# SilentView/EMCID

Measured on AMD Instinct MI355X. Metric: concept-edits/sec (1 000-concept batch, SD-v1.4), higher is better.
Workload: dtype f32 forward (2 x fp16 split MFMA, fp32 accumulate) + f64 solve

## Files before the change

emcid_amd/csrc/clip_layers.hip:

```cpp
#include "common.h"

#include <algorithm>

namespace emcid {

__global__ __launch_bounds__(256) void gather_rows16_kernel(const unsigned char* __restrict__ src, int64_t src_stride,
                                                             const int* __restrict__ idx, unsigned char* __restrict__ dst,
                                                             int64_t dst_stride, int row_bytes) {
    typedef unsigned int v4u __attribute__((ext_vector_type(4)));
    const int64_t r = blockIdx.x;
    const v4u* s = reinterpret_cast<const v4u*>(src + (int64_t)idx[r] * src_stride);
    v4u* d = reinterpret_cast<v4u*>(dst + r * dst_stride);
    for (int i = threadIdx.x; i < row_bytes / 16; i += 256) d[i] = s[i];
}

__global__ __launch_bounds__(256) void gather_f32_kernel(const float* __restrict__ src, const int* __restrict__ idx,
                                                          float* __restrict__ dst, int n) {
    const int i = blockIdx.x * 256 + threadIdx.x;
    if (i < n) dst[i] = src[idx[i]];
}

__device__ __forceinline__ unsigned long long fp_mix(unsigned long long x) {
    x ^= x >> 30; x *= 0xBF58476D1CE4E5B9ull; x ^= x >> 27; x *= 0x94D049BB133111EBull; x ^= x >> 31;
    return x;
}

__device__ __forceinline__ unsigned long long fingerprint_of(const unsigned char* data, long long bytes, unsigned long long* lds) {
    typedef unsigned long long v2u64 __attribute__((ext_vector_type(2)));
    const long long nvec = bytes / 16, ns = nvec < 4096 ? nvec : 4096;
    unsigned long long h = 0;
    v2u64 x[16];
#pragma unroll
    for (int u = 0; u < 16; ++u) {
        const long long i = threadIdx.x + 256 * u;
        const long long v = ns == nvec ? i : i * nvec / ns;
        x[u] = i < ns ? *reinterpret_cast<const v2u64*>(data + 16 * v) : (v2u64){0ull, 0ull};
    }
#pragma unroll
    for (int u = 0; u < 16; ++u) {
        const long long i = threadIdx.x + 256 * u;
        if (i < ns)
            h ^= fp_mix(x[u][0] + 0x9E3779B97F4A7C15ull * (unsigned long long)(2 * i + 1)) ^ fp_mix(x[u][1] + 0x9E3779B97F4A7C15ull * (unsigned long long)(2 * i + 2));
    }
#pragma unroll
    for (int o = 32; o > 0; o >>= 1) {
        const unsigned lo = __shfl_xor((unsigned)(h & 0xffffffffu), o, 64), hi = __shfl_xor((unsigned)(h >> 32), o, 64);
        h ^= ((unsigned long long)hi << 32) | lo;
    }
    if ((threadIdx.x & 63) == 0) lds[threadIdx.x >> 6] = h;
    __syncthreads();
    return lds[0] ^ lds[1] ^ lds[2] ^ lds[3];
}

struct FpBatch { const unsigned char* data[32]; long long bytes[32]; long long slot[32]; };

__global__ __launch_bounds__(256) void fingerprint_store_kernel(FpBatch b, long long* table) {
    __shared__ unsigned long long lds[4];
    const unsigned char* data = b.data[blockIdx.x];
    const long long bytes = b.bytes[blockIdx.x];
    const unsigned long long h = fingerprint_of(data, bytes, lds);
    if (threadIdx.x == 0) {
        long long* e = table + 4 * b.slot[blockIdx.x];
        e[0] = (long long)reinterpret_cast<uintptr_t>(data); e[1] = bytes; e[2] = (long long)h; e[3] = 0;
    }
}

__global__ __launch_bounds__(256) void fingerprint_content_kernel(FpBatch b, unsigned long long* out) {
    __shared__ unsigned long long lds[4];
    const unsigned long long h = fingerprint_of(b.data[blockIdx.x], b.bytes[blockIdx.x], lds);
    if (threadIdx.x == 0) out[b.slot[blockIdx.x]] = h;
}

struct FpSkip { unsigned long long m[4]; };

__global__ __launch_bounds__(256) void fingerprint_check_kernel(const long long* table, long long first_slot, FpSkip skip, int* flag) {
    __shared__ unsigned long long lds[4];
    if ((skip.m[blockIdx.x >> 6] >> (blockIdx.x & 63)) & 1ull) return;
    const long long* e = table + 4 * (first_slot + blockIdx.x);
    const long long bytes = e[1];
    if (bytes <= 0) return;
    const unsigned long long h = fingerprint_of(reinterpret_cast<const unsigned char*>((uintptr_t)e[0]), bytes, lds);
    if (threadIdx.x == 0 && h != (unsigned long long)e[2]) atomicOr(flag, 1);
}

struct ClipWs {
    float* qkv;
    float* mid;
    uint32_t* ctx_p;
    float* ctx_s;
    uint32_t* z_p;
    float* z_s;
    float* f_scale;
    uint32_t* f_p;
    uint32_t* xq_p;
    float* xq_s;
    float* hs_q;
};

inline int64_t clip_ws_bytes(int64_t rows, int64_t h, int64_t d) {
    const int64_t r = round_up(rows, 64);
    return 4 * (r * 3 * h + r * h + r * h + r + r * h + r + 2 * r + r * d + r * h + r + r * h) + 16 * 16;
}

inline bool clip_ws_carve(void* base, int64_t bytes, int64_t rows, int64_t h, int64_t d, ClipWs& w) {
    if (base == nullptr || !aligned16(base) || bytes < clip_ws_bytes(rows, h, d)) return false;
    const int64_t r = round_up(rows, 64);
    char* p = (char*)base;
    auto take = [&](int64_t n4) { char* q = p; p += round_up(4 * n4, 16); return q; };
    w.qkv = (float*)take(r * 3 * h);
    w.mid = (float*)take(r * h);
    w.ctx_p = (uint32_t*)take(r * h);
    w.ctx_s = (float*)take(r);
    w.z_p = (uint32_t*)take(r * h);
    w.z_s = (float*)take(r);
    w.f_scale = (float*)take(2 * r);
    w.f_p = (uint32_t*)take(r * d);
    w.xq_p = (uint32_t*)take(r * h);
    w.xq_s = (float*)take(r);
    w.hs_q = (float*)take(r * h);
    return true;
}

}

using namespace emcid;

extern "C" {

int emcid_fingerprint_store(int64_t n, const void* const* data, const int64_t* bytes, const int64_t* slots, void* table,
                            int64_t table_slots, void* stream) {
    EMCID_CHECK_ARG(n >= 0 && table && (n == 0 || (data && bytes && slots)));
    for (int64_t i0 = 0; i0 < n; i0 += 32) {
        FpBatch b{};
        const int cnt = (int)std::min<int64_t>(32, n - i0);
        for (int i = 0; i < cnt; ++i) {
            EMCID_CHECK_ARG(data[i0 + i] && bytes[i0 + i] > 0 && bytes[i0 + i] % 16 == 0 && aligned16(data[i0 + i]) &&
                            slots[i0 + i] >= 0 && slots[i0 + i] < table_slots);
            b.data[i] = (const unsigned char*)data[i0 + i]; b.bytes[i] = bytes[i0 + i]; b.slot[i] = slots[i0 + i];
        }
        hipLaunchKernelGGL(fingerprint_store_kernel, dim3((unsigned)cnt), dim3(256), 0, (hipStream_t)stream, b, (long long*)table);
    }
    EMCID_CHECK_LAUNCH();
    return EMCID_OK;
}

int emcid_fingerprint_check(const void* table, int64_t table_slots, int64_t first_slot, int64_t n_slots, const uint64_t* skip_mask,
                            int* flag, void* stream) {
    EMCID_CHECK_ARG(table && flag && first_slot >= 0 && n_slots >= 0 && first_slot + n_slots <= table_slots && n_slots <= 256);
    if (n_slots == 0) return EMCID_OK;
    FpSkip skip{};
    if (skip_mask != nullptr)
        for (int w = 0; w < 4; ++w) skip.m[w] = skip_mask[w];
    hipLaunchKernelGGL(fingerprint_check_kernel, dim3((unsigned)n_slots), dim3(256), 0, (hipStream_t)stream, (const long long*)table,
                       (long long)first_slot, skip, flag);
    EMCID_CHECK_LAUNCH();
    return EMCID_OK;
}

int emcid_fingerprint_content(int64_t n, const void* const* data, const int64_t* bytes, uint64_t* out_dev, void* stream) {
    EMCID_CHECK_ARG(n >= 0 && (n == 0 || (data && bytes && out_dev)));
    if (n == 0) return EMCID_OK;
    for (int64_t i = 0; i < n; ++i)
        EMCID_CHECK_ARG(data[i] && bytes[i] > 0 && bytes[i] % 16 == 0 && aligned16(data[i]));
    for (int64_t i0 = 0; i0 < n; i0 += 32) {
        FpBatch b{};
        const int cnt = (int)std::min<int64_t>(32, n - i0);
        for (int i = 0; i < cnt; ++i) {
            b.data[i] = (const unsigned char*)data[i0 + i]; b.bytes[i] = bytes[i0 + i]; b.slot[i] = i0 + i;
        }
        hipLaunchKernelGGL(fingerprint_content_kernel, dim3((unsigned)cnt), dim3(256), 0, (hipStream_t)stream, b,
                           (unsigned long long*)out_dev);
    }
    EMCID_CHECK_LAUNCH();
    return EMCID_OK;
}

int64_t emcid_clip_workspace_bytes(int64_t rows, int64_t h, int64_t d) { return clip_ws_bytes(rows, h, d); }

int emcid_clip_layer_head_sp16(const emcid_clip_layer_sp16* L, int64_t rows, int64_t h, int64_t d, int64_t heads, float attn_scale,
                               const int* anc, int64_t anc_ld, const int* depth, const int* rows_sel, int64_t n_sel,
                               const float* hs, const void* x_planes, const float* x_inv_scale, float* mid, void* f_planes,
                               float* f_scale, float* f_f32, void* workspace, int64_t workspace_bytes, void* stream) {
    EMCID_CHECK_ARG(L && rows > 0 && h > 0 && d > 0 && heads > 0 && h % heads == 0 && anc && depth && hs && x_planes && x_inv_scale);
    EMCID_CHECK_ARG(mid && f_planes && f_scale && n_sel > 0 && n_sel <= rows && (rows_sel != nullptr || n_sel == rows) && h % 32 == 0 && d % 32 == 0);
    ClipWs w;
    if (!clip_ws_carve(workspace, workspace_bytes, rows, h, d, w)) return fail(EMCID_ERR_BAD_ARG, __func__, "workspace too small or misaligned");
    hipStream_t st = (hipStream_t)stream;
    const int64_t D = h / heads;
    const float* q;
    int64_t ldq;
    const float* res;
    if (rows_sel == nullptr) {
        EMCID_TRY(emcid_linear_sp16_f32(x_planes, h, x_inv_scale, L->qkv_planes, h, L->qkv_inv_scale, L->qkv_bias, nullptr, 0, w.qkv,
                                        3 * h, nullptr, 0, nullptr, rows, 3 * h, h, 0, -1, stream));
        q = w.qkv, ldq = 3 * h, res = hs;
    } else {
        EMCID_TRY(emcid_linear_sp16_f32(x_planes, h, x_inv_scale, (const uint32_t*)L->qkv_planes + h * h, h, L->qkv_inv_scale + h,
                                        L->qkv_bias ? L->qkv_bias + h : nullptr, nullptr, 0, w.qkv + h, 3 * h, nullptr, 0, nullptr,
                                        rows, 2 * h, h, 0, -1, stream));
        {
            ScopedProf sp(KC_MISC, st);
            hipLaunchKernelGGL(gather_rows16_kernel, dim3((unsigned)n_sel), dim3(256), 0, st, (const unsigned char*)x_planes, 4 * h,
                               rows_sel, (unsigned char*)w.xq_p, 4 * h, (int)(4 * h));
            hipLaunchKernelGGL(gather_f32_kernel, dim3((unsigned)((n_sel + 255) / 256)), dim3(256), 0, st, x_inv_scale, rows_sel,
                               w.xq_s, (int)n_sel);
            hipLaunchKernelGGL(gather_rows16_kernel, dim3((unsigned)n_sel), dim3(256), 0, st, (const unsigned char*)hs, 4 * h,
                               rows_sel, (unsigned char*)w.hs_q, 4 * h, (int)(4 * h));
            EMCID_CHECK_LAUNCH();
        }
        EMCID_TRY(emcid_linear_sp16_f32(w.xq_p, h, w.xq_s, L->qkv_planes, h, L->qkv_inv_scale, L->qkv_bias, nullptr, 0, w.mid, h,
                                        nullptr, 0, nullptr, n_sel, h, h, 0, -1, stream));
        q = w.mid, ldq = h, res = w.hs_q;
    }
    EMCID_TRY(emcid_tree_attention_sp16(q, ldq, w.qkv + h, w.qkv + 2 * h, 3 * h, anc, anc_ld, depth, rows_sel, n_sel, heads, D,
                                        attn_scale, w.ctx_p, h, w.ctx_s, stream));
    EMCID_TRY(emcid_linear_sp16_f32(w.ctx_p, h, w.ctx_s, L->out_planes, h, L->out_inv_scale, L->out_bias, res, h, mid, h, nullptr,
                                    0, nullptr, n_sel, h, h, 0, -1, stream));
    EMCID_TRY(emcid_add_layernorm_sp16(mid, h, nullptr, 0, L->ln2_gamma, L->ln2_beta, L->ln2_eps, n_sel, h, nullptr, nullptr, w.z_p,
                                       h, w.z_s, L->fc1_bound, f_scale, stream));
    EMCID_TRY(emcid_linear_sp16_f32(w.z_p, h, w.z_s, L->fc1_planes, h, L->fc1_inv_scale, L->fc1_bias, nullptr, 0, f_f32, d,
                                    f_planes, d, f_scale, n_sel, d, h, L->act, -1, stream));
    return EMCID_OK;
}

int emcid_clip_layer_tail_sp16(const emcid_clip_layer_sp16* L, int64_t n, int64_t h, int64_t d, const void* f_planes,
                               const float* f_inv_scale, const float* mid, float* hs_out, const float* next_ln_gamma,
                               const float* next_ln_beta, float next_ln_eps, void* x_planes, float* x_inv_scale, void* stream) {
    EMCID_CHECK_ARG(L && n > 0 && h % 32 == 0 && d % 32 == 0 && f_planes && f_inv_scale && mid && hs_out);
    EMCID_TRY(emcid_linear_sp16_f32(f_planes, d, f_inv_scale, L->fc2_planes, d, L->fc2_inv_scale, L->fc2_bias, mid, h, hs_out, h,
                                    nullptr, 0, nullptr, n, h, d, 0, -1, stream));
    if (next_ln_gamma != nullptr) {
        EMCID_CHECK_ARG(next_ln_beta && x_planes && x_inv_scale);
        EMCID_TRY(emcid_add_layernorm_sp16(hs_out, h, nullptr, 0, next_ln_gamma, next_ln_beta, next_ln_eps, n, h, nullptr, nullptr,
                                           x_planes, h, x_inv_scale, nullptr, nullptr, stream));
    }
    return EMCID_OK;
}

int emcid_clip_edit_layer_tail_sp16(const emcid_clip_layer_sp16* L, int64_t n_rows, int64_t h, int64_t d, const float* f_f32,
                                    const void* f_planes, const float* f_inv_scale, const float* mid, const int64_t* lookup,
                                    const int64_t* seg, int64_t B, int64_t N, const float* zs_t, double edit_weight,
                                    int layers_left, double lam_ratio, const void* cov_factor_ws, int64_t n_layers,
                                    int64_t layer_index, int use_inverse, const float* W0, float* W, float* dW, float* K_out,
                                    float* Zc_out, void* k_planes, float* k_inv_scale, void* dual_ws, int64_t dual_ws_bytes,
                                    int* info_dev, void* linear_ws, int64_t linear_ws_bytes, float* hs_out,
                                    const float* next_ln_gamma, const float* next_ln_beta, float next_ln_eps, void* x_planes,
                                    float* x_inv_scale, void* stream) {
    EMCID_CHECK_ARG(L && n_rows > 0 && h % 32 == 0 && d % 32 == 0 && f_f32 && lookup && seg && B > 0 && N > 0 && zs_t);
    EMCID_CHECK_ARG(cov_factor_ws && W0 && W && K_out && Zc_out && dual_ws && info_dev && (hs_out == nullptr || (f_planes && f_inv_scale && mid)));
    EMCID_TRY(emcid_gather_mean_f32(f_f32, B, n_rows, d, 0, d, lookup, seg, N, K_out, d, stream));
    EMCID_CHECK_ARG((k_planes == nullptr) == (k_inv_scale == nullptr));
    if (k_planes != nullptr) {
        EMCID_TRY(emcid_split_rows_f16(K_out, d, N, d, k_planes, d, k_inv_scale, nullptr, stream));
        EMCID_TRY(emcid_linear_sp16_f32(k_planes, d, k_inv_scale, L->fc2_planes, d, L->fc2_inv_scale, L->fc2_bias, nullptr, 0, Zc_out, h,
                                        nullptr, 0, nullptr, N, h, d, 0, -1, stream));
    } else {
        EMCID_TRY(emcid_linear_ws_f32(K_out, d, W, d, L->fc2_bias, nullptr, 0, Zc_out, h, N, h, d, 0, -1, linear_ws, linear_ws_bytes, stream));
    }
    EMCID_TRY(emcid_edit_dual_apply_stage1_f64(K_out, Zc_out, zs_t, N, d, h, edit_weight, layers_left, lam_ratio, cov_factor_ws,
                                               n_layers, layer_index, 0, N, use_inverse, dual_ws, dual_ws_bytes, stream));
    EMCID_TRY(emcid_edit_dual_apply_stage2_f64(N, d, h, cov_factor_ws, n_layers, layer_index, use_inverse, 0, W0, W, dW, dual_ws,
                                               dual_ws_bytes, info_dev, stream));
    if (hs_out != nullptr) {
        EMCID_TRY(emcid_split_rows_f16(W, d, h, d, const_cast<void*>(L->fc2_planes), d, const_cast<float*>(L->fc2_inv_scale), nullptr,
                                       stream));
        EMCID_TRY(emcid_clip_layer_tail_sp16(L, n_rows, h, d, f_planes, f_inv_scale, mid, hs_out, next_ln_gamma, next_ln_beta,
                                             next_ln_eps, x_planes, x_inv_scale, stream));
    }
    return EMCID_OK;
}

int emcid_clip_layers_sp16(const emcid_clip_layer_sp16* layers, int64_t n_layers, int64_t rows, int64_t h, int64_t d, int64_t heads,
                           float attn_scale, const int* anc, int64_t anc_ld, const int* depth, float* hs, void* x_planes,
                           float* x_inv_scale, const float* next_ln_gamma, const float* next_ln_beta, float next_ln_eps,
                           void* workspace, int64_t workspace_bytes, void* stream) {
    EMCID_CHECK_ARG(layers && n_layers > 0 && hs && x_planes && x_inv_scale);
    ClipWs w;
    if (!clip_ws_carve(workspace, workspace_bytes, rows, h, d, w)) return fail(EMCID_ERR_BAD_ARG, __func__, "workspace too small or misaligned");
    for (int64_t i = 0; i < n_layers; ++i) {
        const emcid_clip_layer_sp16* L = layers + i;
        EMCID_TRY(emcid_clip_layer_head_sp16(L, rows, h, d, heads, attn_scale, anc, anc_ld, depth, nullptr, rows, hs, x_planes,
                                             x_inv_scale, w.mid, w.f_p, w.f_scale, nullptr, workspace, workspace_bytes, stream));
        const bool last = i + 1 == n_layers;
        const float* g = last ? next_ln_gamma : layers[i + 1].ln1_gamma;
        const float* b = last ? next_ln_beta : layers[i + 1].ln1_beta;
        const float eps = last ? next_ln_eps : layers[i + 1].ln1_eps;
        EMCID_TRY(emcid_clip_layer_tail_sp16(L, rows, h, d, w.f_p, w.f_scale + rows, w.mid, hs, g, b, eps, x_planes, x_inv_scale, stream));
    }
    return EMCID_OK;
}

}
```

emcid_amd/csrc/edit_solve.hip:

```cpp
#include "spd_solve.h"

namespace emcid {


__global__ __launch_bounds__(256) void prep_kr_kernel(const float* __restrict__ K, const float* __restrict__ Zc,
                                                       const float* __restrict__ zs_t, int N, int d, int h, double s,
                                                       double layers_left, double* __restrict__ Kt64, int Np, int dp,
                                                       double* __restrict__ Rt, int hp, double g = 1.0) {
    const int n = blockIdx.x;
    for (int j = threadIdx.x; j < dp; j += 256) {
        double v = 0.0;
        if (n < N && j < d) v = (double)K[(int64_t)n * d + j] * s * g;
        Kt64[(int64_t)n * dp + j] = v;
    }
    if (Rt) {
        for (int i = threadIdx.x; i < hp; i += 256) {
            double v = 0.0;
            if (n < N && i < h) {
                const float src = zs_t[(int64_t)n * h + i] - Zc[(int64_t)n * h + i];
                v = ((double)src * s) / layers_left * g;
            }
            Rt[(int64_t)n * hp + i] = v;
        }
    }
}

static void launch_prep_kr(const float* K, const float* Zc, const float* zs_t, int64_t N, int64_t d, int64_t h, double edit_weight,
                           int layers_left, double gain, double* Kt, int64_t Np, int64_t dp, double* R, int64_t hp, hipStream_t st) {
    ScopedProf sp(KC_PREP, st);
    hipLaunchKernelGGL(prep_kr_kernel, dim3((unsigned)Np), dim3(256), 0, st, K, Zc, zs_t, (int)N, (int)d, (int)h, sqrt(edit_weight / 0.5),
                       (double)layers_left, Kt, (int)Np, (int)dp, R, (int)hp, gain);
}

__global__ __launch_bounds__(256) void axpy_f32_kernel(float* __restrict__ W, const float* __restrict__ dW, int64_t n) {
    int64_t i = (int64_t)blockIdx.x * 256 + threadIdx.x;
    const int64_t stride = (int64_t)gridDim.x * 256;
    for (; i < n; i += stride) W[i] += dW[i];
}

__global__ __launch_bounds__(256) void apply_u_kernel(const double* __restrict__ U, const float* __restrict__ W0,
                                                       float* __restrict__ W, float* __restrict__ dW, int64_t n) {
    int64_t i = (int64_t)blockIdx.x * 256 + threadIdx.x;
    const int64_t stride = (int64_t)gridDim.x * 256;
    for (; i < n; i += stride) {
        const float f = (float)U[i];
        if (dW) dW[i] = f;
        if (W) W[i] = W0[i] + f;
    }
}

static int factor_and_solve(double* A, double* L, int64_t dp, int64_t lda, double* invw, int* info, double* B, double* Y,
                            int64_t rows, int64_t ldb, hipStream_t st) {
    return with_graph(make_key(GRAPH_FACTOR_SOLVE, {A, L, invw, info, B, Y}, {dp, lda, rows, ldb}), st, [&](hipStream_t s) {
        EMCID_TRY(cholesky_impl(A, L, dp, lda, invw, info, s));
        return cholesky_solve_impl(L, dp, lda, invw, B, Y, rows, ldb, s);
    });
}


struct CovPtrs { const float* c[32]; };
__global__ __launch_bounds__(256) void scale_cov_kernel(CovPtrs cov, int d, int dp, double lam, float cw, double* __restrict__ M,
                                                         int64_t s_mat) {
    const int l = blockIdx.y;
    const int i = blockIdx.x;
    const float* C = cov.c[l];
    double* row = M + l * s_mat + (int64_t)i * dp;
    for (int j = threadIdx.x; j <= i; j += 256) {
        double v;
        if (i < d) {
            const float c1 = C[(int64_t)i * d + j] * cw;
            v = lam * (double)(c1 / 0.5f);
        } else {
            v = (i == j) ? 1.0 : 0.0;
        }
        row[j] = v;
    }
}

static void assemble_dual_system(const double* P, const double* Q, int64_t dp, double* S, int Np, hipStream_t st,
                                 double* sk_work = nullptr) {
    ScopedProf sp(KC_ASSEMBLE, st);
    GemmShape g{P, dp, Q, dp, Np, Np, (int)dp, 1};
    if (Np >= 512 && sk_work && launch_gemm_f64_streamk2<true, true>(g, EpiAxpby{S, Np, 1.0, 0.0}, st, kStreamKWgs, sk_work, 1.0))
        return;
    hipLaunchKernelGGL(eye_f64_kernel, dim3((unsigned)Np), dim3(256), 0, st, S, Np);
    const int kt = (int)(dp / 16);
    g.ksplit = kt >= 64 ? 4 : kt >= 32 ? 2 : 1;
    launch_gemm_f64<true, true>(g, EpiAxpby{S, Np, 1.0, 1.0}, st, Np >= 512 ? 1 : 2);
}

__global__ __launch_bounds__(256) void transpose_f64_kernel(const double* __restrict__ src, int64_t lds_, double* __restrict__ dst,
                                                             int64_t ldd, int rows, int cols) {
    __shared__ double tile[32][33];
    const int bx = blockIdx.x * 32, by = blockIdx.y * 32;
    const int tx = threadIdx.x & 31, ty = threadIdx.x >> 5;
    for (int r = ty; r < 32; r += 8)
        tile[r][tx] = (by + r < rows && bx + tx < cols) ? src[(int64_t)(by + r) * lds_ + bx + tx] : 0.0;
    __syncthreads();
    for (int r = ty; r < 32; r += 8)
        if (bx + r < cols && by + tx < rows) dst[(int64_t)(bx + r) * ldd + by + tx] = tile[tx][r];
}

struct EditWorkspace {
    int64_t Np, dp, hp;
    int64_t off_A, off_L, off_inv, off_B, off_Y, off_R, total;
    EditWorkspace(int64_t N, int64_t d, int64_t h) {
        Np = round_up(N, NPAD);
        dp = round_up(d, NB);
        hp = round_up(h, 2);
        int64_t o = 0;
        off_A = o; o += dp * dp;
        off_L = o; o += dp * dp;
        off_inv = o; o += inv_doubles(dp);
        off_B = o; o += Np * dp;
        off_Y = o; o += Np * dp;
        off_R = o; o += Np * hp;
        total = o;
    }
};

int solve_schur_rhs(const double* R, int64_t hp, int64_t h, int64_t Np, const double* LS, const double* invS, const double* XT,
                    double* full_inv, double* RT, double* Y2, int64_t y2_doubles, hipStream_t st) {
    if (y2_doubles < hp * Np) return fail(EMCID_ERR_WORKSPACE, __func__, "RT / Y2 hold fewer than h rows of Np (h > d rounded up to 128)");
    const int form = schur_rhs_form(Np, XT != nullptr, full_inv != nullptr, y2_doubles);
    hipLaunchKernelGGL(transpose_f64_kernel, dim3((unsigned)((hp + 31) / 32), (unsigned)(Np / 32)), dim3(256), 0, st, R, hp, RT, Np,
                       (int)Np, (int)hp);
    if (form == EMCID_SCHUR_XROW) {
        ScopedProf sp(KC_TRSM_DIAG, st);
        GemmShape f{RT, Np, XT, Np, (int)h, (int)Np, (int)Np, 0};
        f.tri = 1; f.pair = 1;
        launch_gemm_f64<true, false>(f, EpiAxpby{Y2, Np, 1.0, 0.0}, st);
        GemmShape b{Y2, Np, XT, Np, (int)h, (int)Np, (int)Np, 0};
        b.tri = 2; b.pair = 1;
        launch_gemm_f64<true, true>(b, EpiAxpby{RT, Np, 1.0, 0.0}, st);
    } else if (form == EMCID_SCHUR_FULL_INVERSE) {
        EMCID_TRY(build_full_inverse(LS, Np, Np, invS, full_inv, Y2, y2_doubles, 1, 0, 0, st));
        ScopedProf sp(KC_TRSM_DIAG, st);
        GemmShape f{RT, Np, full_inv, Np, (int)h, (int)Np, (int)Np, 0};
        f.tri = 1; f.pair = 1;
        launch_gemm_f64<true, true>(f, EpiAxpby{Y2, Np, 1.0, 0.0}, st);
        GemmShape b{Y2, Np, full_inv, Np, (int)h, (int)Np, (int)Np, 0};
        b.tri = 2; b.pair = 1;
        launch_gemm_f64<true, false>(b, EpiAxpby{RT, Np, 1.0, 0.0}, st);
    } else {
        EMCID_TRY(cholesky_solve_impl(LS, Np, Np, invS, RT, Y2, h, Np, st));
    }
    return EMCID_OK;
}

}

using namespace emcid;

extern "C" {

int emcid_assemble_spd_f64(const float* C, int64_t ldc, const double* Kt64, int64_t Np, int64_t d, int64_t ldk, double lam,
                           float cw, double* A, int64_t lda, void* stream) {
    EMCID_CHECK_ARG(C && Kt64 && A && Np > 0 && d > 0);
    const int64_t dp = round_up(d, NB);
    EMCID_CHECK_ARG(lda >= dp && ldk >= dp && ldc >= d && (ldk % 2 == 0) && aligned16(Kt64));
    GemmShape p{Kt64, ldk, Kt64, ldk, (int)dp, (int)dp, (int)Np, 1};
    {
        ScopedProf sp(KC_ASSEMBLE, (hipStream_t)stream);
        launch_gemm_f64<false, false>(p, EpiAssemble{C, ldc, lam, cw, A, lda, (int)d}, (hipStream_t)stream);
    }
    EMCID_CHECK_LAUNCH();
    return EMCID_OK;
}

int emcid_delta_w_f64(const double* Rt, int64_t ldr, const double* Xt, int64_t ldx, int64_t Np, int64_t h, int64_t d,
                      const float* W0, float* W, int64_t ldw, float* dW, double* U, void* stream) {
    EMCID_CHECK_ARG(Rt && Xt && Np > 0 && h > 0 && d > 0 && ldr % 2 == 0 && ldx % 2 == 0 && aligned16(Rt) && aligned16(Xt));
    EMCID_CHECK_ARG((W == nullptr) || (W0 != nullptr));
    GemmShape p{Rt, ldr, Xt, ldx, (int)h, (int)d, (int)Np, 0};
    {
        ScopedProf sp(KC_DELTA_W, (hipStream_t)stream);
        launch_gemm_f64<false, false>(p, EpiDeltaW{W0, W, ldw, dW, d, U, d}, (hipStream_t)stream);
    }
    EMCID_CHECK_LAUNCH();
    return EMCID_OK;
}

int emcid_axpy_f32(float* W, const float* dW, int64_t n, void* stream) {
    EMCID_CHECK_ARG(W && dW && n > 0);
    int64_t blocks = (n + 255) / 256;
    if (blocks > 2048) blocks = 2048;
    hipLaunchKernelGGL(axpy_f32_kernel, dim3((unsigned)blocks), dim3(256), 0, (hipStream_t)stream, W, dW, n);
    EMCID_CHECK_LAUNCH();
    return EMCID_OK;
}

int64_t emcid_edit_workspace_bytes(int64_t N, int64_t d, int64_t h) {
    if (N <= 0 || d <= 0 || h <= 0) return 0;
    return EditWorkspace(N, d, h).total * (int64_t)sizeof(double);
}

static int edit_layer_impl(const float* K, const float* Zc, const float* zs_t, const float* C, int64_t N, int64_t d, int64_t h,
                           double lam, double edit_weight, int layers_left, int64_t n_lo, int64_t n_hi, const float* W0,
                           float* W, double* Xt_out, double* Rt_out, float* dW_out, double* U_out, void* workspace,
                           int64_t workspace_bytes, int* info_dev, void* stream) {
    EMCID_CHECK_ARG(K && Zc && zs_t && C && N > 0 && d > 0 && h > 0 && layers_left > 0 && workspace && info_dev);
    EMCID_CHECK_ARG(N < (1 << 24) && d <= 32768 && h <= 32768);
    EMCID_CHECK_ARG(0 <= n_lo && n_lo < n_hi && n_hi <= N);
    EMCID_CHECK_ARG((W == nullptr) || (W0 != nullptr));
    EMCID_CHECK_ARG(aligned16(workspace));
    EditWorkspace ws(N, d, h);
    EMCID_CHECK_WORKSPACE(workspace_bytes, ws.total * (int64_t)sizeof(double), " (see emcid_edit_workspace_bytes)");
    hipStream_t st = (hipStream_t)stream;
    double* base = (double*)workspace;
    double *A = base + ws.off_A, *L = base + ws.off_L, *inv = base + ws.off_inv;
    double *B = base + ws.off_B, *Y = base + ws.off_Y, *R = base + ws.off_R;
    const float cw = (float)(1.0 - edit_weight);
    const int64_t rows = n_hi - n_lo;

    launch_prep_kr(K, Zc, zs_t, N, d, h, edit_weight, layers_left, 1.0, B, ws.Np, ws.dp, R, ws.hp, st);
    EMCID_CHECK_LAUNCH();
    EMCID_TRY(emcid_assemble_spd_f64(C, d, B, ws.Np, d, ws.dp, lam, cw, A, ws.dp, stream));
    double* Bs = B + n_lo * ws.dp;
    EMCID_TRY(factor_and_solve(A, L, ws.dp, ws.dp, inv, info_dev, Bs, Y + n_lo * ws.dp, rows, ws.dp, st));
    if (W || dW_out || U_out)
        EMCID_TRY(emcid_delta_w_f64(R + n_lo * ws.hp, ws.hp, Bs, ws.dp, rows, h, d, W0, W, d, dW_out, U_out, stream));
    if (Xt_out)
        hipLaunchKernelGGL(copy2d_f64_kernel, dim3((unsigned)rows), dim3(256), 0, st, Bs, ws.dp, Xt_out, d, (int)rows, (int)d);
    if (Rt_out)
        hipLaunchKernelGGL(copy2d_f64_kernel, dim3((unsigned)rows), dim3(256), 0, st, R + n_lo * ws.hp, ws.hp, Rt_out, h,
                           (int)rows, (int)h);
    EMCID_CHECK_LAUNCH();
    return EMCID_OK;
}

int emcid_edit_layer_f64(const float* K, const float* Zc, const float* zs_t, const float* C, int64_t N, int64_t d, int64_t h,
                         double lam, double edit_weight, int layers_left, const float* W0, float* W, double* Xt_out,
                         double* Rt_out, float* dW_out, void* workspace, int64_t workspace_bytes, int* info_dev,
                         void* stream) {
    return edit_layer_impl(K, Zc, zs_t, C, N, d, h, lam, edit_weight, layers_left, 0, N, W0, W, Xt_out, Rt_out, dW_out,
                           nullptr, workspace, workspace_bytes, info_dev, stream);
}

int emcid_edit_layer_shard_f64(const float* K, const float* Zc, const float* zs_t, const float* C, int64_t N, int64_t d,
                               int64_t h, double lam, double edit_weight, int layers_left, int64_t n_lo, int64_t n_hi,
                               double* U_partial, double* Xt_out, double* Rt_out, void* workspace, int64_t workspace_bytes,
                               int* info_dev, void* stream) {
    EMCID_CHECK_ARG(U_partial != nullptr);
    return edit_layer_impl(K, Zc, zs_t, C, N, d, h, lam, edit_weight, layers_left, n_lo, n_hi, nullptr, nullptr, Xt_out,
                           Rt_out, nullptr, U_partial, workspace, workspace_bytes, info_dev, stream);
}

int emcid_apply_update_f32(const double* U, const float* W0, float* W, float* dW, int64_t n, void* stream) {
    EMCID_CHECK_ARG(U && n > 0 && (W || dW) && ((W == nullptr) || (W0 != nullptr)));
    int64_t blocks = (n + 255) / 256;
    if (blocks > 2048) blocks = 2048;
    hipLaunchKernelGGL(apply_u_kernel, dim3((unsigned)blocks), dim3(256), 0, (hipStream_t)stream, U, W0, W, dW, n);
    EMCID_CHECK_LAUNCH();
    return EMCID_OK;
}


int64_t emcid_cov_factor_workspace_bytes(int64_t n_layers, int64_t d) {
    if (n_layers <= 0 || d <= 0) return 0;
    return CovFactorLayout(n_layers, d).total * (int64_t)sizeof(double);
}

int emcid_factor_cov_f64(const float* const* C_host_list, int64_t n_layers, int64_t d, double lam, double edit_weight,
                         void* workspace, int64_t workspace_bytes, int* info_dev, void* stream) {
    EMCID_CHECK_ARG(C_host_list && n_layers > 0 && n_layers <= 32 && d > 0 && d <= 32768 && workspace && info_dev);
    EMCID_CHECK_ARG(aligned16(workspace));
    const CovFactorLayout cov(n_layers, d);
    EMCID_CHECK_WORKSPACE(workspace_bytes, cov.total * (int64_t)sizeof(double), " (see emcid_cov_factor_workspace_bytes)");
    const int64_t dp = cov.dp, s_mat = cov.s_mat, s_inv = cov.s_inv;
    double *Mb = cov.M(workspace, 0), *Lb = cov.L(workspace, 0), *Ib = cov.I(workspace, 0);
    CovPtrs cp;
    for (int i = 0; i < 32; ++i) cp.c[i] = i < n_layers ? C_host_list[i] : nullptr;
    for (int i = 0; i < n_layers; ++i) EMCID_CHECK_ARG(cp.c[i] != nullptr);
    const float cw = (float)(1.0 - edit_weight);
    hipStream_t st = (hipStream_t)stream;
    GraphKey key = make_key(GRAPH_FACTOR_COV, {Mb, info_dev}, {n_layers, d, 0, 0, 0});
    memcpy(&key.num[2], &lam, sizeof(double));
    memcpy(&key.num[3], &cw, sizeof(float));
    for (int i = 0; i < n_layers; ++i)
        if (i < 6) key.ptr[2 + i] = cp.c[i]; else key.num[4] = key.num[4] * 1000003 + (int64_t)(uintptr_t)cp.c[i];
    return with_graph(key, st, [&](hipStream_t s) {
        hipLaunchKernelGGL(scale_cov_kernel, dim3((unsigned)dp, (unsigned)n_layers), dim3(256), 0, s, cp, (int)d, (int)dp, lam, cw,
                           Mb, s_mat);
        return cholesky_serial(Mb, Lb, dp, dp, Ib, info_dev, s, (int)n_layers, s_mat, s_inv);
    });
}

int emcid_cov_inverse_f64(void* cov_factor_ws, int64_t n_layers, int64_t d, int64_t first_layer, int64_t count, void* stream) {
    EMCID_CHECK_ARG(cov_factor_ws && n_layers > 0 && n_layers <= 32 && d > 0 && d <= 32768 && aligned16(cov_factor_ws));
    EMCID_CHECK_ARG(0 <= first_layer && count > 0 && first_layer + count <= n_layers);
    const CovFactorLayout cov(n_layers, d);
    const int64_t dp = cov.dp;
    double* Mb = cov.M(cov_factor_ws, first_layer);
    const double *Lb = cov.L(cov_factor_ws, first_layer), *Ib = cov.I(cov_factor_ws, first_layer);
    double* Xb = cov.X(cov_factor_ws, first_layer);
    return with_graph(make_key(GRAPH_COV_INVERSE, {Mb, Lb, Ib, Xb}, {dp, count}), (hipStream_t)stream, [&](hipStream_t s) {
        return build_full_inverse(Lb, dp, dp, Ib, Xb, Mb, cov.s_mat, (int)count, cov.s_mat, cov.s_inv, s);
    });
}

__global__ __launch_bounds__(256) void cov_factor_rescale_kernel(const double* src, double* dst, int64_t off_L, int64_t off_I,
                                                                 int64_t off_X, int64_t s_mat, int64_t s_inv, int dp, int n_tri,
                                                                 double gain_L, double gain_inv, int with_inverse) {
    const int64_t layer = blockIdx.y;
    const int region = blockIdx.z;
    if (region == 1) {
        const double2* s = reinterpret_cast<const double2*>(src + off_I + layer * s_inv);
        double2* o = reinterpret_cast<double2*>(dst + off_I + layer * s_inv);
        for (int64_t i = (int64_t)blockIdx.x * 256 + threadIdx.x; i < s_inv / 2; i += (int64_t)gridDim.x * 256) {
            double2 v = s[i];
            v.x *= gain_inv;
            v.y *= gain_inv;
            o[i] = v;
        }
        return;
    }
    if (region == 2 && !with_inverse) return;
    const int t = blockIdx.x;
    if (t >= n_tri) return;
    int I = (int)((sqrtf(8.0f * (float)t + 1.0f) - 1.0f) * 0.5f);
    while ((I + 1) * (I + 2) / 2 <= t) ++I;
    while (I * (I + 1) / 2 > t) --I;
    const int J = t - I * (I + 1) / 2;
    const int64_t base = (region == 0 ? off_L : off_X) + layer * s_mat + (int64_t)I * NB * dp + (int64_t)J * NB;
    const double g = region == 0 ? gain_L : gain_inv;
    for (int e = threadIdx.x; e < NB * (NB / 2); e += 256) {
        const int r = e / (NB / 2), c2 = e % (NB / 2);
        const int64_t at = base + (int64_t)r * dp + 2 * c2;
        double2 v = *reinterpret_cast<const double2*>(src + at);
        v.x *= g;
        v.y *= g;
        *reinterpret_cast<double2*>(dst + at) = v;
    }
}

int emcid_cov_factor_rescale_f64(const void* src_ws, void* dst_ws, int64_t workspace_bytes, int64_t n_layers, int64_t d, double a,
                                 int with_inverse, void* stream) {
    EMCID_CHECK_ARG(src_ws && dst_ws && n_layers > 0 && n_layers <= 32 && d > 0 && d <= 32768);
    EMCID_CHECK_ARG(aligned16(src_ws) && aligned16(dst_ws) && a > 0.0 && a < 1e300);
    const CovFactorLayout cov(n_layers, d);
    EMCID_CHECK_WORKSPACE(workspace_bytes, cov.total * (int64_t)sizeof(double), " (see emcid_cov_factor_workspace_bytes)");
    const int64_t dp = cov.dp, s_inv = cov.s_inv, nt = dp / NB;
    EMCID_CHECK_ARG(s_inv % 2 == 0);
    const double* src = (const double*)src_ws;
    const int n_tri = (int)(nt * (nt + 1) / 2);
    const double root = sqrt(a);
    hipLaunchKernelGGL(cov_factor_rescale_kernel, dim3((unsigned)n_tri, (unsigned)n_layers, 3), dim3(256), 0, (hipStream_t)stream,
                       src, (double*)dst_ws, (int64_t)(cov.L(src, 0) - src), (int64_t)(cov.I(src, 0) - src), (int64_t)(cov.X(src, 0) - src),
                       cov.s_mat, s_inv, (int)dp, n_tri, root, 1.0 / root, with_inverse);
    EMCID_CHECK_LAUNCH();
    return EMCID_OK;
}

static double* dual_block(void* workspace, int64_t N, int64_t d, int64_t h, int64_t DualWorkspace::*off) {
    if (!workspace || N <= 0 || d <= 0 || h <= 0) return nullptr;
    return (double*)workspace + DualWorkspace(N, d, h).*off;
}

int64_t emcid_edit_dual_workspace_bytes(int64_t N, int64_t d, int64_t h) {
    if (N <= 0 || d <= 0 || h <= 0) return 0;
    return DualWorkspace(N, d, h).total * (int64_t)sizeof(double);
}

double* emcid_edit_dual_block(void* workspace, int64_t N, int64_t d, int64_t h, int which, int64_t* doubles_out) {
    if (doubles_out) *doubles_out = -1;
    int64_t off = 0, n = 0;
    if (!workspace || N <= 0 || d <= 0 || h <= 0 || !DualWorkspace(N, d, h).block(which, &off, &n)) return nullptr;
    if (doubles_out) *doubles_out = n;
    return (double*)workspace + off;
}

int emcid_edit_dual_schur_form(int64_t N, int64_t d, int64_t h) {
    if (N <= 0 || d <= 0 || h <= 0) return -1;
    const DualWorkspace ws(N, d, h);
    return schur_rhs_form(ws.Np, cholesky_takes_shadow(ws.Np), true, ws.y2_doubles());
}

#define EMCID_CHECK_DUAL_STAGE1_ARGS()                                                                            \
    EMCID_CHECK_ARG(K && Zc && zs_t && N > 0 && d > 0 && h > 0 && layers_left > 0 && cov_factor_ws && workspace); \
    EMCID_CHECK_ARG(0 <= layer_index && layer_index < n_layers && 0 <= n_lo && n_lo < n_hi && n_hi <= N);         \
    EMCID_CHECK_ARG(lam_ratio > 0.0 && lam_ratio < 1e300)

int emcid_edit_dual_stage1_f64(const float* K, const float* Zc, const float* zs_t, int64_t N, int64_t d, int64_t h,
                               double edit_weight, int layers_left, double lam_ratio, const void* cov_factor_ws, int64_t n_layers,
                               int64_t layer_index, int64_t n_lo, int64_t n_hi, int use_inverse, void* workspace,
                               int64_t workspace_bytes, void* stream) {
    EMCID_CHECK_DUAL_STAGE1_ARGS();
    DualWorkspace ws(N, d, h);
    EMCID_CHECK_WORKSPACE(workspace_bytes, ws.total * (int64_t)sizeof(double), "");
    hipStream_t st = (hipStream_t)stream;
    double* base = (double*)workspace;
    double *Kt = base + ws.off_K, *Pt = base + ws.off_P, *Y = base + ws.off_Y, *R = base + ws.off_R;
    const int64_t dp = ws.dp;
    const CovFactorLayout cov(n_layers, d);
    const double *Lb = cov.L(cov_factor_ws, layer_index), *Ib = cov.I(cov_factor_ws, layer_index);
    launch_prep_kr(K, Zc, zs_t, N, d, h, edit_weight, layers_left, 1.0 / sqrt(lam_ratio), Kt, ws.Np, dp, R, ws.hp, st);
    const int64_t rows = n_hi - n_lo;
    if (use_inverse) {
        const double* Xb = cov.X(cov_factor_ws, layer_index);
        apply_inverse_forward(Xb, dp, Kt + n_lo * dp, Y + n_lo * dp, (int)rows, st, base + ws.off_SK);
        apply_inverse_backward(Xb, dp, Y + n_lo * dp, (int)rows, (int)dp, Pt + n_lo * dp, dp, st, base + ws.off_SK);
        EMCID_CHECK_LAUNCH();
        return EMCID_OK;
    }
    if (hipMemcpyAsync(Pt + n_lo * dp, Kt + n_lo * dp, rows * dp * sizeof(double), hipMemcpyDeviceToDevice, st) != hipSuccess)
        return fail(EMCID_ERR_HIP, __func__, "hipMemcpyAsync");
    return with_graph(make_key(GRAPH_DUAL_STAGE1, {Lb, Ib, Pt + n_lo * dp, Y + n_lo * dp}, {dp, rows}), st, [&](hipStream_t q) {
        return cholesky_solve_impl(Lb, dp, dp, Ib, Pt + n_lo * dp, Y + n_lo * dp, rows, dp, q);
    });
}

double* emcid_edit_dual_pt(void* workspace, int64_t N, int64_t d, int64_t h) { return dual_block(workspace, N, d, h, &DualWorkspace::off_P); }

int emcid_edit_dual_stage2_f64(int64_t N, int64_t d, int64_t h, double lam_ratio, const float* W0, float* W, double* adjk_out, double* Rt_out,
                               float* dW_out, void* workspace, int64_t workspace_bytes, int* info_dev, void* stream) {
    EMCID_CHECK_ARG(N > 0 && d > 0 && h > 0 && workspace && info_dev && ((W == nullptr) || (W0 != nullptr)));
    EMCID_CHECK_ARG(lam_ratio > 0.0 && lam_ratio < 1e300);
    DualWorkspace ws(N, d, h);
    EMCID_CHECK_WORKSPACE(workspace_bytes, ws.total * (int64_t)sizeof(double), "");
    hipStream_t st = (hipStream_t)stream;
    double* base = (double*)workspace;
    double *Kt = base + ws.off_K, *Pt = base + ws.off_P, *R = base + ws.off_R, *S = base + ws.off_S, *LS = base + ws.off_LS;
    double *invS = base + ws.off_invS, *PT = base + ws.off_PT, *Y2 = base + ws.off_Y2;
    const int64_t dp = ws.dp, Np = ws.Np;
    EMCID_TRY(with_graph(make_key(GRAPH_DUAL_STAGE2,{Kt, Pt, S, LS, invS, PT, Y2, info_dev}, {dp, Np, N}), st, [&](hipStream_t q) {
        if (Np > N)
            hipLaunchKernelGGL(zero_f64_kernel, dim3(256), dim3(256), 0, q, Pt + N * dp, (Np - N) * dp);
        assemble_dual_system(Pt, Kt, dp, S, (int)Np, q, base + ws.off_SK);
        EMCID_TRY(cholesky_impl(S, LS, Np, Np, invS, info_dev, q));
        hipLaunchKernelGGL(transpose_f64_kernel, dim3((unsigned)(dp / 32), (unsigned)(Np / 32)), dim3(256), 0, q, Pt, dp, PT, Np,
                           (int)Np, (int)dp);
        return cholesky_solve_impl(LS, Np, Np, invS, PT, Y2, dp, Np, q);
    }));
    if (W || dW_out) {
        ScopedProf sp(KC_DELTA_W, st);
        GemmShape g{R, ws.hp, PT, Np, (int)h, (int)d, (int)Np, 0};
        launch_gemm_f64<false, true>(g, EpiDeltaW{W0, W, d, dW_out, d, nullptr, d}, st);
    }
    const double root = sqrt(lam_ratio);
    if (adjk_out)
        hipLaunchKernelGGL(copy2d_f64_kernel, dim3((unsigned)d), dim3(256), 0, st, PT, Np, adjk_out, N, (int)d, (int)N, 1.0 / root);
    if (Rt_out) hipLaunchKernelGGL(copy2d_f64_kernel, dim3((unsigned)N), dim3(256), 0, st, R, ws.hp, Rt_out, h, (int)N, (int)h, root);
    EMCID_CHECK_LAUNCH();
    return EMCID_OK;
}

int emcid_edit_dual_apply_stage1_f64(const float* K, const float* Zc, const float* zs_t, int64_t N, int64_t d, int64_t h,
                                     double edit_weight, int layers_left, double lam_ratio, const void* cov_factor_ws, int64_t n_layers,
                                     int64_t layer_index, int64_t n_lo, int64_t n_hi, int use_inverse, void* workspace,
                                     int64_t workspace_bytes, void* stream) {
    EMCID_CHECK_DUAL_STAGE1_ARGS();
    DualWorkspace ws(N, d, h);
    EMCID_CHECK_WORKSPACE(workspace_bytes, ws.total * (int64_t)sizeof(double), "");
    hipStream_t st = (hipStream_t)stream;
    double* base = (double*)workspace;
    double *Kt = base + ws.off_K, *Bs = base + ws.off_P, *Yt = base + ws.off_Y, *R = base + ws.off_R;
    const int64_t dp = ws.dp;
    const CovFactorLayout cov(n_layers, d);
    const double *Lb = cov.L(cov_factor_ws, layer_index), *Ib = cov.I(cov_factor_ws, layer_index);
    launch_prep_kr(K, Zc, zs_t, N, d, h, edit_weight, layers_left, 1.0 / sqrt(lam_ratio), Kt, ws.Np, dp, R, ws.hp, st);
    const int64_t rows = n_hi - n_lo;
    if (use_inverse) {
        const int64_t gemm_rows = (n_lo == 0 && n_hi == N) ? ws.Np : rows;
        apply_inverse_forward(cov.X(cov_factor_ws, layer_index), dp, Kt + n_lo * dp, Yt + n_lo * dp, (int)gemm_rows, st,
                              base + ws.off_SK);
        if (gemm_rows != ws.Np && ws.Np > N)
            hipLaunchKernelGGL(zero_f64_kernel, dim3(256), dim3(256), 0, st, Yt + N * dp, (ws.Np - N) * dp);
        EMCID_CHECK_LAUNCH();
        return EMCID_OK;
    }
    if (ws.Np > N) hipLaunchKernelGGL(zero_f64_kernel, dim3(256), dim3(256), 0, st, Yt + N * dp, (ws.Np - N) * dp);
    if (hipMemcpyAsync(Bs + n_lo * dp, Kt + n_lo * dp, rows * dp * sizeof(double), hipMemcpyDeviceToDevice, st) != hipSuccess)
        return fail(EMCID_ERR_HIP, __func__, "hipMemcpyAsync");
    return with_graph(make_key(GRAPH_APPLY_STAGE1,{Lb, Ib, Bs + n_lo * dp, Yt + n_lo * dp}, {dp, rows}), st, [&](hipStream_t q) {
        trsm_forward(Lb, dp, dp, OB, Ib, Bs + n_lo * dp, dp, Yt + n_lo * dp, dp, (int)rows, q);
        return check_launch("emcid_edit_dual_apply_stage1_f64");
    });
}

double* emcid_edit_dual_yt(void* workspace, int64_t N, int64_t d, int64_t h) { return dual_block(workspace, N, d, h, &DualWorkspace::off_Y); }

int emcid_edit_dual_apply_assemble_f64(int64_t N, int64_t d, int64_t h, void* workspace, int64_t workspace_bytes, void* stream) {
    EMCID_CHECK_ARG(N > 0 && d > 0 && h > 0 && workspace);
    DualWorkspace ws(N, d, h);
    EMCID_CHECK_WORKSPACE(workspace_bytes, ws.total * (int64_t)sizeof(double), "");
    hipStream_t st = (hipStream_t)stream;
    double* base = (double*)workspace;
    double *Yt = base + ws.off_Y, *S = base + ws.off_S;
    const int64_t dp = ws.dp, Np = ws.Np;
    assemble_dual_system(Yt, Yt, dp, S, (int)Np, st, base + ws.off_SK);
    EMCID_CHECK_LAUNCH();
    return EMCID_OK;
}

int emcid_edit_dual_apply_stage2_f64(int64_t N, int64_t d, int64_t h, const void* cov_factor_ws, int64_t n_layers,
                                     int64_t layer_index, int use_inverse, int assembled, const float* W0, float* W,
                                     float* dW_out, void* workspace, int64_t workspace_bytes, int* info_dev, void* stream) {
    EMCID_CHECK_ARG(N > 0 && d > 0 && h > 0 && workspace && info_dev && cov_factor_ws && ((W == nullptr) || (W0 != nullptr)));
    EMCID_CHECK_ARG(0 <= layer_index && layer_index < n_layers && (W || dW_out));
    DualWorkspace ws(N, d, h);
    EMCID_CHECK_WORKSPACE(workspace_bytes, ws.total * (int64_t)sizeof(double), "");
    hipStream_t st = (hipStream_t)stream;
    double* base = (double*)workspace;
    double *Yt = base + ws.off_Y, *R = base + ws.off_R, *S = base + ws.off_S, *LS = base + ws.off_LS, *invS = base + ws.off_invS;
    double *RT = base + ws.off_PT, *Y2 = base + ws.off_Y2, *V = base + ws.off_V, *U = base + ws.off_U;
    const int64_t dp = ws.dp, Np = ws.Np, hp = ws.hp;
    const CovFactorLayout cov(n_layers, d);
    const double *Lb = cov.L(cov_factor_ws, layer_index), *Ib = cov.I(cov_factor_ws, layer_index);
    static const int shadow_env = env_flag("EMCID_SHADOW_P", 1);
    bool shadow = shadow_env && use_inverse && cholesky_takes_shadow(Np);
    if (shadow && shadow_env == 1) {
        const int64_t ntl = (dp + SH_BN - 1) / SH_BN, nb = Np / NB;
        const int64_t steps = ((ntl + 1) * (SH_BN / 16) + nb - 1) / nb;
        const int64_t wgs = ((Np + SH_BM - 1) / SH_BM) * ((ntl + 1) / 2), rounds = (wgs + 239) / 240;
        shadow = rounds * (9.0 + 1.5 * (double)steps) <= 50.0;
    }
    double* P = base + ws.off_P;
    const double* X = use_inverse ? cov.X(cov_factor_ws, layer_index) : nullptr;
    const bool p_first = !shadow && use_inverse && Np < h;
    const bool xrow = cholesky_takes_shadow(Np);
    double *XT = base + ws.off_XT, *TT = base + ws.off_TT;
    EMCID_TRY(with_graph(make_key(GRAPH_APPLY_STAGE2, {Yt, R, S, LS, RT, V, U, info_dev},
                                  {dp, Np, N, hp, (int64_t)(uintptr_t)Lb,
                                   use_inverse + 2 * (assembled != 0) + 4 * (int)shadow + 8 * h + ((int64_t)p_first << 31) + ((int64_t)xrow << 30) + (d << 32)}),
                         st,
                         [&](hipStream_t q) {
        if (!assembled) {
            assemble_dual_system(Yt, Yt, dp, S, (int)Np, q, base + ws.off_SK);
        }
        if (p_first) apply_inverse_backward(X, dp, Yt, (int)Np, (int)dp, P, dp, q, base + ws.off_SK);
        ShadowJob job{Yt, dp, X, dp, P, dp, (int)Np, (int)dp, (int)dp, 0, nullptr, 0, 0, 0};
        job.wgs = (int)((Np + SH_BM - 1) / SH_BM) * (int)(((dp + SH_BN - 1) / SH_BN + 1) / 2);
        const XrowJob xj{XT, Np, TT};
        EMCID_TRY(cholesky_impl(S, LS, Np, Np, invS, info_dev, q, shadow ? &job : nullptr, xrow ? &xj : nullptr));
        EMCID_TRY(solve_schur_rhs(R, hp, h, Np, LS, invS, xrow ? XT : nullptr, S, RT, Y2, ws.y2_doubles(), q));
        if (!shadow && !p_first) {
            ScopedProf sp(KC_DELTA_W, q);
            GemmShape g{RT, Np, Yt, dp, (int)h, (int)dp, (int)Np, 0};
            launch_gemm_f64<true, false>(g, EpiAxpby{V, dp, 1.0, 0.0}, q);
        }
        if (!use_inverse) trsm_backward(Lb, dp, dp, OB, Ib, V, dp, U, dp, (int)h, q);
        return check_launch("emcid_edit_dual_apply_stage2_f64");
    }));
    if (shadow || p_first) {
        ScopedProf sp(KC_DELTA_W, st);
        GemmShape g{RT, Np, P, dp, (int)h, (int)d, (int)Np, 0};
        launch_gemm_f64<true, false>(g, EpiDeltaW{W0, W, d, dW_out, d, nullptr, 0}, st, -1);
        EMCID_CHECK_LAUNCH();
        return EMCID_OK;
    }
    if (use_inverse)
        apply_inverse_backward(X, dp, V, (int)h, (int)dp, U, dp, st, base + ws.off_SK);
    hipLaunchKernelGGL(apply_u2d_kernel, dim3((unsigned)h), dim3(256), 0, st, U, dp, W0, W, dW_out, (int)d);
    EMCID_CHECK_LAUNCH();
    return EMCID_OK;
}

__global__ __launch_bounds__(256) void add_identity_f64_kernel(double* __restrict__ S, int n) {
    const int i = blockIdx.x * 256 + threadIdx.x;
    if (i < n) S[(int64_t)i * n + i] += 1.0;
}

static int check_tiles(const int* tiles, int n_tiles, int64_t dp) {
    if (!tiles || n_tiles <= 0 || n_tiles > 256) return 0;
    for (int i = 0; i < n_tiles; ++i)
        if (tiles[i] < 0 || (int64_t)tiles[i] * NB >= dp || (i > 0 && tiles[i] <= tiles[i - 1])) return 0;
    return 1;
}

int emcid_edit_dual_cols_stage1_f64(const float* K, const float* Zc, const float* zs_t, int64_t N, int64_t d, int64_t h,
                                    double edit_weight, int layers_left, double lam_ratio, const void* cov_factor_ws, int64_t n_layers,
                                    int64_t layer_index, const int* tiles_host, int n_tiles, void* workspace,
                                    int64_t workspace_bytes, void* stream) {
    EMCID_CHECK_ARG(K && Zc && zs_t && N > 0 && d > 0 && h > 0 && layers_left > 0 && cov_factor_ws && workspace);
    EMCID_CHECK_ARG(0 <= layer_index && layer_index < n_layers && lam_ratio > 0.0 && lam_ratio < 1e300);
    DualWorkspace ws(N, d, h);
    EMCID_CHECK_ARG(check_tiles(tiles_host, n_tiles, ws.dp));
    EMCID_CHECK_WORKSPACE(workspace_bytes, ws.total * (int64_t)sizeof(double), "");
    hipStream_t st = (hipStream_t)stream;
    double* base = (double*)workspace;
    double *Kt = base + ws.off_K, *Yc = base + ws.off_Y, *R = base + ws.off_R, *S = base + ws.off_S, *sk = base + ws.off_SK;
    const int64_t dp = ws.dp, Np = ws.Np;
    const double* X = CovFactorLayout(n_layers, d).X(cov_factor_ws, layer_index);
    launch_prep_kr(K, Zc, zs_t, N, d, h, edit_weight, layers_left, 1.0 / sqrt(lam_ratio), Kt, Np, dp, R, ws.hp, st);
    for (int i = 0; i < n_tiles; ++i) {
        const int64_t t = tiles_host[i], kd = (t + 1) * NB;
        ScopedProf sp(KC_INV_APPLY, st);
        GemmShape g{Kt, dp, X + t * NB * dp, dp, (int)Np, NB, (int)kd, 0};
        if (!launch_gemm_f64_streamk2<true, true>(g, EpiAxpby{Yc + (int64_t)i * NB, dp, 1.0, 0.0}, st, kStreamKWgs, sk))
            return fail(EMCID_ERR_BAD_ARG, __func__, "more output tiles than stream-K ticket counters");
    }
    {
        ScopedProf sp(KC_ASSEMBLE, st);
        GemmShape g{Yc, dp, Yc, dp, (int)Np, (int)Np, n_tiles * NB, 1};
        if (!launch_gemm_f64_streamk2<true, true>(g, EpiAxpby{S, Np, 1.0, 0.0}, st, kStreamKWgs, sk, 0.0))
            return fail(EMCID_ERR_BAD_ARG, __func__, "more output tiles than stream-K ticket counters");
    }
    EMCID_CHECK_LAUNCH();
    return EMCID_OK;
}

double* emcid_edit_dual_s(void* workspace, int64_t N, int64_t d, int64_t h) { return dual_block(workspace, N, d, h, &DualWorkspace::off_S); }

double* emcid_edit_dual_u(void* workspace, int64_t N, int64_t d, int64_t h) { return dual_block(workspace, N, d, h, &DualWorkspace::off_U); }

int emcid_edit_dual_cols_stage2_f64(int64_t N, int64_t d, int64_t h, const void* cov_factor_ws, int64_t n_layers,
                                    int64_t layer_index, const int* tiles_host, int n_tiles, void* workspace,
                                    int64_t workspace_bytes, int* info_dev, void* stream) {
    EMCID_CHECK_ARG(N > 0 && d > 0 && h > 0 && workspace && info_dev && cov_factor_ws);
    EMCID_CHECK_ARG(0 <= layer_index && layer_index < n_layers);
    DualWorkspace ws(N, d, h);
    EMCID_CHECK_ARG(check_tiles(tiles_host, n_tiles, ws.dp));
    EMCID_CHECK_WORKSPACE(workspace_bytes, ws.total * (int64_t)sizeof(double), "");
    hipStream_t st = (hipStream_t)stream;
    double* base = (double*)workspace;
    double *Yc = base + ws.off_Y, *R = base + ws.off_R, *S = base + ws.off_S, *LS = base + ws.off_LS, *invS = base + ws.off_invS;
    double *RT = base + ws.off_PT, *Y2 = base + ws.off_Y2, *V = base + ws.off_V, *U = base + ws.off_U;
    const int64_t dp = ws.dp, Np = ws.Np, hp = ws.hp;
    if (ws.y2_doubles() < hp * Np) return fail(EMCID_ERR_WORKSPACE, __func__, "RT / Y2 hold fewer than h rows of Np (h > d rounded up to 128)");
    const double* X = CovFactorLayout(n_layers, d).X(cov_factor_ws, layer_index);
    const int w = n_tiles * NB;
    const bool xrow = cholesky_takes_shadow(Np);
    EMCID_TRY(with_graph(make_key(GRAPH_COLS_STAGE2,{Yc, R, S, LS, RT, V, U, info_dev}, {dp, Np, N, hp, (int64_t)w + ((int64_t)xrow << 40)}), st, [&](hipStream_t q) {
        hipLaunchKernelGGL(add_identity_f64_kernel, dim3((unsigned)((Np + 255) / 256)), dim3(256), 0, q, S, (int)Np);
        const XrowJob xj{base + ws.off_XT, Np, base + ws.off_TT};
        EMCID_TRY(cholesky_impl(S, LS, Np, Np, invS, info_dev, q, nullptr, xrow ? &xj : nullptr));
        EMCID_TRY(solve_schur_rhs(R, hp, h, Np, LS, invS, xrow ? xj.Xt : nullptr, nullptr, RT, Y2, ws.y2_doubles(), q));
        {
            ScopedProf sp(KC_DELTA_W, q);
            GemmShape g{RT, Np, Yc, dp, (int)h, w, (int)Np, 0};
            launch_gemm_f64<true, false>(g, EpiAxpby{V, dp, 1.0, 0.0}, q);
        }
        hipLaunchKernelGGL(zero2d_f64_kernel, dim3((unsigned)h, 1u), dim3(256), 0, q, U, dp, (int64_t)0, (int)dp);
        return check_launch("emcid_edit_dual_cols_stage2_f64");
    }));
    for (int i = 0; i < n_tiles; ++i) {
        const int64_t t = tiles_host[i], kd = (t + 1) * NB;
        ScopedProf sp(KC_INV_APPLY, st);
        GemmShape g{V + (int64_t)i * NB, dp, X + t * NB * dp, dp, (int)h, (int)kd, NB, 0};
        launch_gemm_f64<true, false>(g, EpiAxpby{U, dp, 1.0, 1.0}, st);
    }
    EMCID_CHECK_LAUNCH();
    return EMCID_OK;
}

int emcid_apply_update2d_f32(const double* U, int64_t ldu, const float* W0, float* W, float* dW, int64_t h, int64_t d, void* stream) {
    EMCID_CHECK_ARG(U && h > 0 && d > 0 && ldu >= d && (W || dW) && ((W == nullptr) || (W0 != nullptr)));
    hipLaunchKernelGGL(apply_u2d_kernel, dim3((unsigned)h), dim3(256), 0, (hipStream_t)stream, U, ldu, W0, W, dW, (int)d);
    EMCID_CHECK_LAUNCH();
    return EMCID_OK;
}

}
```

emcid_amd/csrc/spd_solve.h:

```cpp
#pragma once
#include "common.h"
#include "gemm_f64.h"

namespace emcid {


#define EMCID_GEMM_F64_INSTANCES(X)                                                                        \
    X void launch_gemm_f64<true, false, EpiAxpby>(GemmShape, EpiAxpby, hipStream_t, int);                     \
    X void launch_gemm_f64<true, true, EpiAxpby>(GemmShape, EpiAxpby, hipStream_t, int);                      \
    X bool launch_gemm_f64_streamk2<true, true>(GemmShape, EpiAxpby, hipStream_t, int, double*, double);      \
    X bool launch_gemm_f64_streamk2<true, false>(GemmShape, EpiAxpby, hipStream_t, int, double*, double);     \
    X void launch_gemm_f64<false, true, EpiAxpby>(GemmShape, EpiAxpby, hipStream_t, int);                     \
    X void launch_gemm_f64<false, false, EpiAxpby>(GemmShape, EpiAxpby, hipStream_t, int);                    \
    X void launch_gemm_f64<false, false, EpiAssemble>(GemmShape, EpiAssemble, hipStream_t, int);              \
    X void launch_gemm_f64<false, false, EpiDeltaW>(GemmShape, EpiDeltaW, hipStream_t, int);                  \
    X void launch_gemm_f64<false, true, EpiDeltaW>(GemmShape, EpiDeltaW, hipStream_t, int);                   \
    X void launch_gemm_f64<true, false, EpiDeltaW>(GemmShape, EpiDeltaW, hipStream_t, int);
EMCID_GEMM_F64_INSTANCES(extern template)

struct ShadowJob {
    const double* A; int64_t lda;
    const double* B; int64_t ldb;
    double* C; int64_t ldc;
    int M, N, K;
    int wgs;
    long long* stamps;
    int xcd_gx;
    int nofast;
    int fuse_pair;
};

struct XrowJob {
    double* Xt; int64_t ldx;
    double* Tt;
};
constexpr int SH_BM = 64, SH_BN = 128;

inline bool cholesky_takes_shadow(int64_t dp) {
    return dp <= 2048 && dp >= 2 * NB;
}
int cholesky_serial(double* A, double* L, int64_t dp, int64_t lda, double* invw, int* info, hipStream_t st, int nbatch = 1,
                    int64_t s_mat = 0, int64_t s_inv = 0);
int cholesky_impl(double* A, double* L, int64_t dp, int64_t lda, double* invw, int* info, hipStream_t st,
                  const ShadowJob* shadow = nullptr, const XrowJob* xrow = nullptr);
void trsm_forward(const double* L, int64_t ldl, int64_t n, int blk, const double* inv, double* B, int64_t ldb, double* Out,
                  int64_t ldo, int rows, hipStream_t st);
void trsm_backward(const double* L, int64_t ldl, int64_t n, int blk, const double* inv, double* B, int64_t ldb, double* Out,
                   int64_t ldo, int rows, hipStream_t st);
int cholesky_solve_impl(const double* L, int64_t dp, int64_t lda, const double* invw, double* Bt, double* Yt, int64_t Mrows,
                        int64_t ldb, hipStream_t st);
int64_t full_inverse_scratch_doubles(int64_t dp, int64_t lda);
int build_full_inverse(const double* L, int64_t dp, int64_t lda, const double* invw, double* X, double* T, int64_t t_doubles,
                       int nbatch, int64_t s_mat, int64_t s_inv, hipStream_t st);
constexpr int kStreamKWgs = 256;
void apply_inverse_forward(const double* X, int64_t dp, const double* Kt, double* Yt, int rows, hipStream_t st,
                           double* sk_work = nullptr);
void apply_inverse_backward(const double* X, int64_t dp, const double* V, int rows, int ncols, double* C, int64_t ldc,
                            hipStream_t st, double* sk_work = nullptr);
void assemble_schur_system(const double* Yk, int64_t ldy, int64_t dp, const double* Lkp, int64_t ldl, int64_t M, double* S, int N,
                           int Np, hipStream_t st);


struct CovFactorLayout {
    int64_t n_layers, dp, s_mat, s_inv, total;
    CovFactorLayout(int64_t n_layers_, int64_t d)
        : n_layers(n_layers_), dp(round_up(d, NB)), s_mat(dp * dp), s_inv(inv_doubles(dp)), total(n_layers * (3 * s_mat + s_inv)) {}
    double* M(const void* ws, int64_t l) const { return (double*)ws + l * s_mat; }
    double* L(const void* ws, int64_t l) const { return (double*)ws + n_layers * s_mat + l * s_mat; }
    double* I(const void* ws, int64_t l) const { return (double*)ws + 2 * n_layers * s_mat + l * s_inv; }
    double* X(const void* ws, int64_t l) const { return (double*)ws + n_layers * (2 * s_mat + s_inv) + l * s_mat; }
};

struct DualWorkspace {
    int64_t Np, dp, hp;
    int64_t off_K, off_P, off_Y, off_R, off_S, off_LS, off_invS, off_PT, off_Y2, off_V, off_U, off_SK, off_XT, off_TT, total;
    DualWorkspace(int64_t N, int64_t d, int64_t h) {
        Np = round_up(N, NB);
        dp = round_up(d, NB);
        hp = round_up(h, 2);
        int64_t o = 0;
        off_K = o; o += Np * dp;
        off_P = o; o += Np * dp;
        off_Y = o; o += Np * dp;
        off_R = o; o += Np * hp;
        off_S = o; o += Np * Np;
        off_LS = o; o += Np * Np;
        off_invS = o; o += inv_doubles(Np);
        off_PT = o; o += dp * Np;
        off_Y2 = o; o += dp * Np;
        off_V = o; o += hp * dp;
        off_U = o; o += hp * dp;
        off_SK = o; o += streamk_workspace_doubles(kStreamKWgs);
        off_XT = o; o += Np * Np;
        off_TT = o; o += Np * NB;
        total = o;
    }
    int64_t y2_doubles() const { return dp * Np; }
    bool block(int which, int64_t* off, int64_t* doubles) const {
        const int64_t offs[] = {off_K, off_P, off_Y, off_R, off_S, off_LS, off_invS, off_PT, off_Y2, off_V, off_U, off_SK, off_XT, off_TT, total};
        if (which == EMCID_DUAL_SK_COUNTERS) {
            *off = off_XT - 8192;
            *doubles = 8192;
            return true;
        }
        if (which < 0 || which > EMCID_DUAL_TT) return false;
        *off = offs[which];
        *doubles = offs[which + 1] - offs[which];
        return true;
    }
};

inline int schur_rhs_form(int64_t Np, bool have_xt, bool have_full_inv, int64_t scratch_doubles) {
    if (have_xt) return EMCID_SCHUR_XROW;
    if (have_full_inv && Np <= 4096 && full_inverse_scratch_doubles(Np, Np) <= scratch_doubles) return EMCID_SCHUR_FULL_INVERSE;
    return EMCID_SCHUR_SUBSTITUTION;
}

int solve_schur_rhs(const double* R, int64_t hp, int64_t h, int64_t Np, const double* LS, const double* invS, const double* XT,
                    double* full_inv, double* RT, double* Y2, int64_t y2_doubles, hipStream_t st);


static __global__ __launch_bounds__(256) void copy2d_f64_kernel(const double* __restrict__ src, int64_t lds_, double* __restrict__ dst,
                                                                 int64_t ldd, int rows, int cols, double scale = 1.0) {
    const int r = blockIdx.x;
    for (int c = threadIdx.x; c < cols; c += 256) dst[(int64_t)r * ldd + c] = src[(int64_t)r * lds_ + c] * scale;
}

static __global__ __launch_bounds__(256) void zero_f64_kernel(double* __restrict__ p, int64_t n) {
    int64_t i = (int64_t)blockIdx.x * 256 + threadIdx.x;
    const int64_t stride = (int64_t)gridDim.x * 256;
    for (; i < n; i += stride) p[i] = 0.0;
}

static __global__ __launch_bounds__(256) void zero2d_f64_kernel(double* __restrict__ p, int64_t ld, int64_t s_batch, int cols) {
    double* row = p + blockIdx.y * s_batch + (int64_t)blockIdx.x * ld;
    for (int j = threadIdx.x; j < cols; j += 256) row[j] = 0.0;
}

static __global__ __launch_bounds__(256) void eye_f64_kernel(double* __restrict__ S, int n) {
    const int i = blockIdx.x;
    for (int j = threadIdx.x; j < n; j += 256) S[(int64_t)i * n + j] = (i == j) ? 1.0 : 0.0;
}

static __global__ __launch_bounds__(256) void apply_u2d_kernel(const double* __restrict__ U, int64_t ldu, const float* __restrict__ W0,
                                                                float* __restrict__ W, float* __restrict__ dW, int d) {
    const int i = blockIdx.x;
    for (int j = threadIdx.x; j < d; j += 256) {
        const float f = (float)U[(int64_t)i * ldu + j];
        if (dW) dW[(int64_t)i * d + j] = f;
        if (W) W[(int64_t)i * d + j] = W0[(int64_t)i * d + j] + f;
    }
}

}
```

emcid_amd/hip.py:

```python
from __future__ import annotations

import ctypes as C
import math
import os
import threading
from pathlib import Path
from typing import Optional

import torch

_LIB_PATH = Path(__file__).resolve().parent / "csrc" / "libemcid_hip.so"
_lib = None

EXPORTS = [
    "emcid_abi_version", "emcid_last_error", "emcid_gram_accumulate_f32", "emcid_symmetrize_lower_f32",
    "emcid_gather_mean_f32", "emcid_edit_workspace_bytes", "emcid_edit_layer_f64", "emcid_assemble_spd_f64",
    "emcid_cholesky_f64", "emcid_cholesky_solve_f64", "emcid_delta_w_f64", "emcid_dgemm_f64", "emcid_dgemm_ex_f64", "emcid_dgemm_batched_f64", "emcid_streamk_workspace_bytes", "emcid_dgemm_streamk_f64", "emcid_debug_streamk_stamps", "emcid_debug_step_stamps", "emcid_debug_linear_sp16_stamps", "emcid_fingerprint_store", "emcid_fingerprint_check", "emcid_fingerprint_content", "emcid_axpy_f32",
    "emcid_profile_enable", "emcid_profile_collect", "emcid_attention_f32", "emcid_edit_layer_shard_f64",
    "emcid_apply_update_f32", "emcid_inverse_workspace_doubles", "emcid_quick_gelu_f32", "emcid_add_layernorm_f32", "emcid_embed_layernorm_f32", "emcid_tree_attention_f32", "emcid_debug_leaf_stamps",
    "emcid_cov_factor_workspace_bytes", "emcid_factor_cov_f64", "emcid_cov_inverse_f64", "emcid_cov_factor_rescale_f64",
    "emcid_edit_dual_workspace_bytes",
    "emcid_edit_dual_stage1_f64", "emcid_edit_dual_pt", "emcid_edit_dual_stage2_f64",
    "emcid_edit_dual_apply_stage1_f64", "emcid_edit_dual_yt", "emcid_edit_dual_apply_stage2_f64",
    "emcid_edit_dual_apply_assemble_f64",
    "emcid_edit_dual_preserve_workspace_bytes", "emcid_edit_layer_dual_preserve_f64",
    "emcid_session_retain_workspace_bytes", "emcid_session_retain_f64", "emcid_session_step_norms_f64",
    "emcid_session_release_workspace_bytes", "emcid_session_release_f64", "emcid_session_rescale_f64",
    "emcid_cov_factor_fold_workspace_bytes", "emcid_cov_factor_fold_f64",
    "emcid_session_refold_update_f64", "emcid_cov_factor_refactor_f64",
    "emcid_score_rows_f32", "emcid_score_chains_f64", "emcid_score_chains_pair_f64", "emcid_score_pooled_f32",
    "emcid_score_chains_pair_grid_f64",
    "emcid_edit_lu_workspace_bytes", "emcid_edit_layer_lu_f64", "emcid_lu_solve_f64",
    "emcid_edit_dual_cols_stage1_f64", "emcid_edit_dual_s", "emcid_edit_dual_u", "emcid_edit_dual_cols_stage2_f64",
    "emcid_apply_update2d_f32", "emcid_linear_f32", "emcid_linear_ws_f32", "emcid_linear_workspace_bytes",
    "emcid_split_rows_f16", "emcid_linear_sp16_f32", "emcid_gram_sp16_workspace_bytes", "emcid_gram_sp16_workspace_bytes_for", "emcid_gram_accumulate_sp16_f32", "emcid_add_layernorm_sp16", "emcid_embed_layernorm_sp16",
    "emcid_tree_attention_sp16", "emcid_tree_attention_sp16_supported", "emcid_clip_workspace_bytes",
    "emcid_clip_layer_head_sp16", "emcid_clip_layer_tail_sp16", "emcid_clip_layers_sp16", "emcid_clip_edit_layer_tail_sp16",
    "emcid_edit_dual_block", "emcid_edit_dual_schur_form", "emcid_full_inverse_scratch_doubles", "emcid_full_inverse_f64",
]
DUAL_BLOCKS = ["K", "P", "Y", "R", "S", "LS", "INVS", "PT", "Y2", "V", "U", "SK", "XT", "TT", "SK_COUNTERS"]
SCHUR_FORMS = ["xrow", "full_inverse", "substitution"]
PROF_CLASSES = ["prep", "assemble", "chol_leaf", "chol_panel", "chol_trail", "trsm_diag", "trsm_update", "delta_w",
                "gram", "gather", "dgemm", "misc", "inv_build", "chol_inner", "inv_apply", "inv_block", "linear"]

ABI_VERSION = 16
NB = 128
NPAD = 64


class EmcidHipError(RuntimeError):
    pass


def lib_path() -> Path:
    return _LIB_PATH


def load():
    global _lib
    if _lib is not None:
        return _lib
    if not _LIB_PATH.exists():
        raise EmcidHipError(
            f"{_LIB_PATH} is missing: build it with `python -c 'import __graft_entry__ as g; g.build()'` "
            f"or `make -C {_LIB_PATH.parent}`. The MI355X path has no CPU fallback.")
    lib = C.CDLL(str(_LIB_PATH))
    p, i64, i32, f64, f32 = C.c_void_p, C.c_int64, C.c_int, C.c_double, C.c_float
    sig = {
        "emcid_abi_version": (i32, []),
        "emcid_last_error": (C.c_char_p, []),
        "emcid_gram_accumulate_f32": (i32, [p, i64, i64, i64, p, i64, i32, p]),
        "emcid_symmetrize_lower_f32": (i32, [p, i64, i64, p]),
        "emcid_gather_mean_f32": (i32, [p, i64, i64, i64, i64, i64, p, p, i64, p, i64, p]),
        "emcid_edit_workspace_bytes": (i64, [i64, i64, i64]),
        "emcid_edit_layer_f64": (i32, [p, p, p, p, i64, i64, i64, f64, f64, i32, p, p, p, p, p, p, i64, p, p]),
        "emcid_edit_layer_shard_f64": (i32, [p, p, p, p, i64, i64, i64, f64, f64, i32, i64, i64, p, p, p, p, i64, p, p]),
        "emcid_apply_update_f32": (i32, [p, p, p, p, i64, p]),
        "emcid_assemble_spd_f64": (i32, [p, i64, p, i64, i64, i64, f64, f32, p, i64, p]),
        "emcid_cholesky_f64": (i32, [p, p, i64, i64, p, p, p]),
        "emcid_inverse_workspace_doubles": (i64, [i64]),
        "emcid_debug_leaf_stamps": (i32, [p, p, p, p, p, p]),
        "emcid_cov_factor_workspace_bytes": (i64, [i64, i64]),
        "emcid_factor_cov_f64": (i32, [p, i64, i64, f64, f64, p, i64, p, p]),
        "emcid_cov_inverse_f64": (i32, [p, i64, i64, i64, i64, p]),
        "emcid_cov_factor_rescale_f64": (i32, [p, p, i64, i64, i64, f64, i32, p]),
        "emcid_edit_dual_workspace_bytes": (i64, [i64, i64, i64]),
        "emcid_edit_dual_stage1_f64": (i32, [p, p, p, i64, i64, i64, f64, i32, f64, p, i64, i64, i64, i64, i32, p, i64, p]),
        "emcid_edit_dual_pt": (p, [p, i64, i64, i64]),
        "emcid_edit_dual_block": (p, [p, i64, i64, i64, i32, C.POINTER(i64)]),
        "emcid_edit_dual_schur_form": (i32, [i64, i64, i64]),
        "emcid_full_inverse_scratch_doubles": (i64, [i64, i64]),
        "emcid_full_inverse_f64": (i32, [p, i64, i64, p, p, p, i64, p]),
        "emcid_edit_dual_stage2_f64": (i32, [i64, i64, i64, f64, p, p, p, p, p, p, i64, p, p]),
        "emcid_edit_dual_apply_stage1_f64": (i32, [p, p, p, i64, i64, i64, f64, i32, f64, p, i64, i64, i64, i64, i32, p, i64, p]),
        "emcid_edit_dual_yt": (p, [p, i64, i64, i64]),
        "emcid_edit_dual_apply_stage2_f64": (i32, [i64, i64, i64, p, i64, i64, i32, i32, p, p, p, p, i64, p, p]),
        "emcid_edit_dual_apply_assemble_f64": (i32, [i64, i64, i64, p, i64, p]),
        "emcid_edit_dual_preserve_workspace_bytes": (i64, [i64, i64, i64, i64]),
        "emcid_edit_layer_dual_preserve_f64": (i32, [p, p, p, i64, i64, i64, f64, i32, f64, p, i64, i64, p, i64, p, i64, p, i64, i64,
                                                     p, p, p, p, p, i64, p, p]),
        "emcid_session_retain_workspace_bytes": (i64, [i64, i64, i64]),
        "emcid_session_retain_f64": (i32, [p, i64, i64, f64, f64, p, i64, i64, p, i64, p, i64, p, i64, i64, p, i64, p, p]),
        "emcid_session_step_norms_f64": (i32, [p, i64, i64, i64, i64, i64, i64, p, p, p, p]),
        "emcid_session_release_workspace_bytes": (i64, [i64, i64, i64]),
        "emcid_session_release_f64": (i32, [p, i64, i64, i64, p, i64, p, i64, p, i64, i64, p, i64, p, p]),
        "emcid_session_rescale_f64": (i32, [p, p, i64, i64, i64, p, i64, p, i64, p, i64, i64, p, i64, p, p]),
        "emcid_cov_factor_fold_workspace_bytes": (i64, [i64, i64]),
        "emcid_cov_factor_fold_f64": (i32, [p, f64, p, i64, i64, i64, p, f64, f64, i32, p, i64, i64, i64, p, p, i64, p, p]),
        "emcid_session_refold_update_f64": (i32, [p, i64, i64, i64, p, i64, i64, i64, p, i64, i64, p, i64, p, p]),
        "emcid_cov_factor_refactor_f64": (i32, [p, i64, i64, i64, p, p]),
        "emcid_score_rows_f32": (i32, [p, i64, p, i64, p, i64, p, p, f32, i64, i64, p, p]),
        "emcid_score_chains_f64": (i32, [p, i64, p, i64, p, p, i64, p, p]),
        "emcid_score_chains_pair_f64": (i32, [p, i64, p, i64, p, p, p, i64, p, i64, p, p, i64, p, p]),
        "emcid_score_chains_pair_grid_f64": (i32, [p, i64, i64, p, i64, p, p, p, i64, i64, p, i64, p, p, i64, p, i64, p, p]),
        "emcid_score_pooled_f32": (i32, [p, i64, p, i64, p, p, f32, p, i64, i64, i64, i64, p, p]),
        "emcid_cholesky_solve_f64": (i32, [p, i64, i64, p, p, p, i64, i64, p]),
        "emcid_edit_dual_cols_stage1_f64": (i32, [p, p, p, i64, i64, i64, f64, i32, f64, p, i64, i64, p, i32, p, i64, p]),
        "emcid_edit_dual_s": (p, [p, i64, i64, i64]),
        "emcid_edit_dual_u": (p, [p, i64, i64, i64]),
        "emcid_edit_dual_cols_stage2_f64": (i32, [i64, i64, i64, p, i64, i64, p, i32, p, i64, p, p]),
        "emcid_apply_update2d_f32": (i32, [p, i64, p, p, p, i64, i64, p]),
        "emcid_edit_lu_workspace_bytes": (i64, [i64, i64, i64]),
        "emcid_edit_layer_lu_f64": (i32, [p, p, p, p, i64, i64, i64, f64, f64, i32, p, p, p, p, p, p, i64, p, p]),
        "emcid_lu_solve_f64": (i32, [p, i64, i64, p, i64, i64, p, p, p]),
        "emcid_delta_w_f64": (i32, [p, i64, p, i64, i64, i64, i64, p, p, i64, p, p, p]),
        "emcid_dgemm_f64": (i32, [i32, i32, i64, i64, i64, f64, p, i64, p, i64, f64, p, i64, p]),
        "emcid_dgemm_ex_f64": (i32, [i32, i32, i64, i64, i64, f64, p, i64, p, i64, f64, p, i64, i32, i32, i32, p]),
        "emcid_dgemm_batched_f64": (i32, [i32, i32, i64, i64, i64, f64, p, i64, i64, p, i64, i64, f64, p, i64, i64, i64, p]),
        "emcid_streamk_workspace_bytes": (i64, [i32]),
        "emcid_debug_streamk_stamps": (i32, [p]),
        "emcid_debug_linear_sp16_stamps": (i32, [p]),
        "emcid_fingerprint_store": (i32, [i64, p, p, p, p, i64, p]),
        "emcid_fingerprint_check": (i32, [p, i64, i64, i64, p, p, p]),
        "emcid_fingerprint_content": (i32, [i64, p, p, p, p]),
        "emcid_debug_step_stamps": (i32, [p]),
        "emcid_dgemm_streamk_f64": (i32, [i32, i64, i64, i64, f64, p, i64, p, i64, p, i64, i32, i32, f64, p, i64, p]),
        "emcid_axpy_f32": (i32, [p, p, i64, p]),
        "emcid_quick_gelu_f32": (i32, [p, p, i64, p]),
        "emcid_linear_f32": (i32, [p, i64, p, i64, p, p, i64, p, i64, i64, i64, i64, i32, i32, p]),
        "emcid_linear_ws_f32": (i32, [p, i64, p, i64, p, p, i64, p, i64, i64, i64, i64, i32, i32, p, i64, p]),
        "emcid_linear_workspace_bytes": (i64, []),
        "emcid_split_rows_f16": (i32, [p, i64, i64, i64, p, i64, p, p, p]),
        "emcid_gram_sp16_workspace_bytes": (i64, [i64]),
        "emcid_gram_sp16_workspace_bytes_for": (i64, [i64, i64]),
        "emcid_gram_accumulate_sp16_f32": (i32, [p, p, i64, i64, i64, p, i64, p, i64, p]),
        "emcid_add_layernorm_sp16": (i32, [p, i64, p, i64, p, p, C.c_float, i64, i64, p, p, p, i64, p, p, p, p]),
        "emcid_embed_layernorm_sp16": (i32, [p, i64, i64, p, i64, i64, p, p, p, p, C.c_float, i64, i64, p, p, p, i64, p, p]),
        "emcid_tree_attention_sp16_supported": (i32, [i64, i64, i64]),
        "emcid_clip_workspace_bytes": (i64, [i64, i64, i64]),
        "emcid_clip_layer_head_sp16": (i32, [p, i64, i64, i64, i64, f32, p, i64, p, p, i64, p, p, p, p, p, p, p, p, i64, p]),
        "emcid_clip_layer_tail_sp16": (i32, [p, i64, i64, i64, p, p, p, p, p, p, f32, p, p, p]),
        "emcid_clip_layers_sp16": (i32, [p, i64, i64, i64, i64, i64, f32, p, i64, p, p, p, p, p, p, f32, p, i64, p]),
        "emcid_clip_edit_layer_tail_sp16": (i32, [p, i64, i64, i64, p, p, p, p, p, p, i64, i64, p, f64, i32, f64, p, i64, i64, i32,
                                                 p, p, p, p, p, p, p, p, i64, p, p, i64, p, p, p, f32, p, p, p]),
        "emcid_tree_attention_sp16": (i32, [p, i64, p, p, i64, p, i64, p, p, i64, i64, i64, f32, p, i64, p, p]),
        "emcid_linear_sp16_f32": (i32, [p, i64, p, p, i64, p, p, p, i64, p, i64, p, i64, p, i64, i64, i64, i32, i32, p]),
        "emcid_add_layernorm_f32": (i32, [p, i64, p, i64, p, p, C.c_float, i64, i64, p, p, p]),
        "emcid_embed_layernorm_f32": (i32, [p, i64, i64, p, i64, i64, p, p, p, p, C.c_float, i64, i64, p, p, p]),
        "emcid_tree_attention_f32": (i32, [p, i64, p, p, i64, p, i64, p, p, i64, i64, i64, f32, p, i64, p]),
        "emcid_profile_enable": (i32, [C.c_uint]),
        "emcid_profile_collect": (i32, [p, p, i32]),
        "emcid_attention_f32": (i32, [p, p, p, i64, i64, i64, p, i32, i64, i64, i32, f32, i64, i64, i64, i64, p, p]),
    }
    for name, (res, args) in sig.items():
        fn = getattr(lib, name)
        fn.restype, fn.argtypes = res, args
    if lib.emcid_abi_version() != ABI_VERSION:
        raise EmcidHipError(f"ABI mismatch: library {lib.emcid_abi_version()} vs binding {ABI_VERSION}; rebuild csrc/")
    _lib = lib
    return lib


_tls = threading.local()


def _check(rc: int, what: str):
    restore = getattr(_tls, "restore", None)
    if restore:
        torch.cuda.set_device(restore.pop())
    if rc != 0:
        raise EmcidHipError(f"{what} failed (rc={rc}): {load().emcid_last_error().decode()}")


def _ptr(t: Optional[torch.Tensor], dtype=None, what="tensor"):
    if t is None:
        return None
    if not t.is_cuda:
        raise EmcidHipError(f"{what} must live in HBM (got device {t.device}); there is no CPU path")
    if dtype is not None and t.dtype != dtype:
        raise EmcidHipError(f"{what} must be {dtype}, got {t.dtype}")
    return C.c_void_p(t.data_ptr())


def _stream(t: torch.Tensor):
    idx = t.device.index
    cur = torch.cuda.current_device()
    if idx is not None and idx != cur:
        if getattr(_tls, "restore", None) is None:
            _tls.restore = []
        _tls.restore.append(cur)
        torch.cuda.set_device(idx)
    return C.c_void_p(torch.cuda.current_stream(t.device).cuda_stream)


def pinned_copy(t: torch.Tensor) -> torch.Tensor:
    out = torch.empty(t.shape, dtype=t.dtype, pin_memory=True)
    out.copy_(t.detach(), non_blocking=True)
    return out



GRAM_SPLIT = os.environ.get("EMCID_GRAM_SPLIT", "1") != "0"
_GRAM_WS = {}


def gram_takes_row_weight(X: torch.Tensor, ksplit: int = 0) -> bool:
    d = X.shape[1]
    return bool(GRAM_SPLIT and ksplit != 1 and X.shape[0] >= 2048 and d % 4 == 0 and d >= 256 and X.stride(0) % 4 == 0
                and X.stride(1) == 1 and X.data_ptr() % 16 == 0 and X.dtype == torch.float32)


def gram_accumulate_(G: torch.Tensor, X: torch.Tensor, ksplit: int = 0, row_weight: Optional[torch.Tensor] = None):
    assert X.dim() == 2 and G.dim() == 2 and G.shape[0] == G.shape[1] == X.shape[1]
    assert X.stride(1) == 1 and G.stride(1) == 1
    if X.shape[0] == 0:
        return G
    d = X.shape[1]
    if row_weight is not None:
        assert row_weight.shape == (X.shape[0],) and row_weight.dtype == torch.float32 and row_weight.is_contiguous()
        if not (gram_takes_row_weight(X, ksplit) and G.dtype == torch.float32):
            X, row_weight = X * row_weight.unsqueeze(1), None
    if GRAM_SPLIT and ksplit != 1 and X.shape[0] >= 2048 and d % 4 == 0 and d >= 256 and X.stride(0) % 4 == 0 \
            and X.data_ptr() % 16 == 0 and X.dtype == torch.float32 and G.dtype == torch.float32:
        key = (X.device.index if X.device.index is not None else torch.cuda.current_device(),
               torch.cuda.current_stream(X.device).cuda_stream, d)
        need = int(load().emcid_gram_sp16_workspace_bytes_for(d, X.shape[0]))
        ws = _GRAM_WS.get(key)
        if ws is None or ws.numel() < need:
            if ws is None and len(_GRAM_WS) >= 8:
                _GRAM_WS.clear()
            ws = _GRAM_WS[key] = torch.empty(need, dtype=torch.uint8, device=X.device)
        _check(load().emcid_gram_accumulate_sp16_f32(_ptr(X, torch.float32, "X"),
                                                     _ptr(row_weight, torch.float32, "row_weight") if row_weight is not None else None,
                                                     X.shape[0], d, X.stride(0),
                                                     _ptr(G, torch.float32, "G"), G.stride(0), C.c_void_p(ws.data_ptr()),
                                                     ws.numel(), _stream(G)), "emcid_gram_accumulate_sp16_f32")
        return G
    _check(load().emcid_gram_accumulate_f32(_ptr(X, torch.float32, "X"), X.shape[0], X.shape[1], X.stride(0),
                                            _ptr(G, torch.float32, "G"), G.stride(0), ksplit, _stream(G)),
           "emcid_gram_accumulate_f32")
    return G


def symmetrize_lower_(G: torch.Tensor):
    _check(load().emcid_symmetrize_lower_f32(_ptr(G, torch.float32, "G"), G.shape[0], G.stride(0), _stream(G)),
           "emcid_symmetrize_lower_f32")
    return G



def gather_mean(act: torch.Tensor, idx: torch.Tensor, seg: torch.Tensor, out: Optional[torch.Tensor] = None):
    assert act.dim() == 3 and act.stride(2) == 1
    B, S, c = act.shape
    N = seg.numel() - 1
    assert idx.numel() == B
    if out is None:
        out = torch.empty(N, c, dtype=torch.float32, device=act.device)
    _check(load().emcid_gather_mean_f32(_ptr(act, torch.float32, "act"), B, S, c, act.stride(0), act.stride(1),
                                        _ptr(idx, torch.int64, "idx"), _ptr(seg, torch.int64, "seg"), N,
                                        _ptr(out, torch.float32, "out"), out.stride(0), _stream(act)),
           "emcid_gather_mean_f32")
    return out



def edit_workspace_bytes(N: int, d: int, h: int) -> int:
    return int(load().emcid_edit_workspace_bytes(N, d, h))


class EditWorkspace:

    def __init__(self, N: int, d: int, h: int, device, lu: bool = False):
        self.key = (N, d, h)
        self.lu = lu
        self.nbytes = int(load().emcid_edit_lu_workspace_bytes(N, d, h)) if lu else edit_workspace_bytes(N, d, h)
        self.buf = torch.zeros(self.nbytes // 8, dtype=torch.float64, device=device)
        self.info = torch.zeros(1, dtype=torch.int32, device=device)


def edit_layer(K, Zc, zs_t, Cov, lam: float, edit_weight: float, layers_left: int, W0=None, W=None,
               want_factors: bool = False, want_dw: bool = True, ws: Optional[EditWorkspace] = None):
    N, d = K.shape
    h = Zc.shape[1]
    assert Cov.shape == (d, d) and zs_t.shape == (N, h) and Zc.shape == (N, h)
    for t, nm in ((K, "K"), (Zc, "Zc"), (zs_t, "zs_t"), (Cov, "C")):
        assert t.is_contiguous(), nm
    if ws is None or ws.key != (N, d, h) or ws.lu:
        ws = EditWorkspace(N, d, h, K.device)
    dev = K.device
    Xt = torch.empty(N, d, dtype=torch.float64, device=dev) if want_factors else None
    Rt = torch.empty(N, h, dtype=torch.float64, device=dev) if want_factors else None
    dW = torch.empty(h, d, dtype=torch.float32, device=dev) if want_dw else None
    if W is not None:
        assert W.is_contiguous() and W.shape == (h, d) and W0 is not None and W0.is_contiguous()
    _check(load().emcid_edit_layer_f64(
        _ptr(K, torch.float32, "K"), _ptr(Zc, torch.float32, "Zc"), _ptr(zs_t, torch.float32, "zs_t"),
        _ptr(Cov, torch.float32, "C"), N, d, h, float(lam), float(edit_weight), int(layers_left),
        _ptr(W0, torch.float32, "W0"), _ptr(W, torch.float32, "W"), _ptr(Xt), _ptr(Rt), _ptr(dW),
        _ptr(ws.buf), ws.nbytes, _ptr(ws.info, torch.int32, "info"), _stream(K)), "emcid_edit_layer_f64")
    return {"Xt": Xt, "Rt": Rt, "dW": dW, "ws": ws}


def edit_layer_lu(K, Zc, zs_t, Cov, lam: float, edit_weight: float, layers_left: int, W0=None, W=None,
                  want_factors: bool = False, want_dw: bool = True, ws: Optional[EditWorkspace] = None):
    N, d = K.shape
    h = Zc.shape[1]
    assert Cov.shape == (d, d) and zs_t.shape == (N, h) and Zc.shape == (N, h)
    for t, nm in ((K, "K"), (Zc, "Zc"), (zs_t, "zs_t"), (Cov, "C")):
        assert t.is_contiguous(), nm
    if ws is None or ws.key != (N, d, h) or not ws.lu:
        ws = EditWorkspace(N, d, h, K.device, lu=True)
    dev = K.device
    adj_k = torch.empty(d, N, dtype=torch.float64, device=dev) if want_factors else None
    Rt = torch.empty(N, h, dtype=torch.float64, device=dev) if want_factors else None
    dW = torch.empty(h, d, dtype=torch.float32, device=dev) if want_dw else None
    if W is not None:
        assert W.is_contiguous() and W.shape == (h, d) and W0 is not None and W0.is_contiguous()
    _check(load().emcid_edit_layer_lu_f64(
        _ptr(K, torch.float32, "K"), _ptr(Zc, torch.float32, "Zc"), _ptr(zs_t, torch.float32, "zs_t"),
        _ptr(Cov, torch.float32, "C"), N, d, h, float(lam), float(edit_weight), int(layers_left),
        _ptr(W0, torch.float32, "W0"), _ptr(W, torch.float32, "W"), _ptr(adj_k), _ptr(Rt), _ptr(dW),
        _ptr(ws.buf), ws.nbytes, _ptr(ws.info, torch.int32, "info"), _stream(K)), "emcid_edit_layer_lu_f64")
    return {"adj_k": adj_k, "Rt": Rt, "dW": dW, "ws": ws}


def lu_solve_(A: torch.Tensor, B: torch.Tensor):
    n = A.shape[0]
    piv = torch.zeros(n, dtype=torch.int32, device=A.device)
    info = torch.zeros(1, dtype=torch.int32, device=A.device)
    _check(load().emcid_lu_solve_f64(_ptr(A, torch.float64, "A"), A.stride(0), n, _ptr(B, torch.float64, "B"), B.stride(0),
                                     B.shape[1], _ptr(piv), _ptr(info), _stream(A)), "emcid_lu_solve_f64")
    return piv, info


def edit_layer_shard(K, Zc, zs_t, Cov, lam: float, edit_weight: float, layers_left: int, rows, want_factors=False,
                     ws: Optional[EditWorkspace] = None):
    N, d = K.shape
    h = Zc.shape[1]
    lo, hi = rows
    assert Cov.shape == (d, d) and zs_t.shape == (N, h) and Zc.shape == (N, h) and 0 <= lo < hi <= N
    for t, nm in ((K, "K"), (Zc, "Zc"), (zs_t, "zs_t"), (Cov, "C")):
        assert t.is_contiguous(), nm
    if ws is None or ws.key != (N, d, h) or ws.lu:
        ws = EditWorkspace(N, d, h, K.device)
    dev = K.device
    U = torch.empty(h, d, dtype=torch.float64, device=dev)
    Xt = torch.empty(hi - lo, d, dtype=torch.float64, device=dev) if want_factors else None
    Rt = torch.empty(hi - lo, h, dtype=torch.float64, device=dev) if want_factors else None
    _check(load().emcid_edit_layer_shard_f64(
        _ptr(K, torch.float32, "K"), _ptr(Zc, torch.float32, "Zc"), _ptr(zs_t, torch.float32, "zs_t"),
        _ptr(Cov, torch.float32, "C"), N, d, h, float(lam), float(edit_weight), int(layers_left), lo, hi,
        _ptr(U), _ptr(Xt), _ptr(Rt), _ptr(ws.buf), ws.nbytes, _ptr(ws.info, torch.int32, "info"), _stream(K)),
        "emcid_edit_layer_shard_f64")
    return {"U": U, "Xt": Xt, "Rt": Rt, "ws": ws}


def apply_update_(U, W0, W, want_dw=True):
    assert U.is_contiguous() and W.is_contiguous() and W0.is_contiguous() and U.shape == W.shape
    dW = torch.empty_like(W) if want_dw else None
    _check(load().emcid_apply_update_f32(_ptr(U, torch.float64, "U"), _ptr(W0, torch.float32, "W0"),
                                         _ptr(W, torch.float32, "W"), _ptr(dW), W.numel(), _stream(W)),
           "emcid_apply_update_f32")
    return dW


def dgemm(ta: int, tb: int, A, B, Cm, alpha=1.0, beta=0.0, M=None, N=None, K=None):
    M = M if M is not None else (A.shape[0] if ta == 0 else A.shape[1])
    K = K if K is not None else (A.shape[1] if ta == 0 else A.shape[0])
    N = N if N is not None else (B.shape[0] if tb == 0 else B.shape[1])
    _check(load().emcid_dgemm_f64(ta, tb, M, N, K, float(alpha), _ptr(A, torch.float64), A.stride(0),
                                  _ptr(B, torch.float64), B.stride(0), float(beta), _ptr(Cm, torch.float64),
                                  Cm.stride(0), _stream(Cm)), "emcid_dgemm_f64")
    return Cm


def dgemm_ex(ta: int, tb: int, A, B, Cm, alpha=1.0, beta=0.0, flags=0, cfg=-1, ksplit=0):
    M = A.shape[0] if ta == 0 else A.shape[1]
    K = A.shape[1] if ta == 0 else A.shape[0]
    N = B.shape[0] if tb == 0 else B.shape[1]
    _check(load().emcid_dgemm_ex_f64(ta, tb, M, N, K, float(alpha), _ptr(A, torch.float64), A.stride(0),
                                     _ptr(B, torch.float64), B.stride(0), float(beta), _ptr(Cm, torch.float64),
                                     Cm.stride(0), int(flags), int(cfg), int(ksplit), _stream(Cm)), "emcid_dgemm_ex_f64")
    return Cm


_streamk_ws = {}


def dgemm_streamk(tb: int, A, B, Cm, alpha=1.0, flags=1, wgs=256, diag_add=0.0):
    M, K = A.shape
# ... 246 lines not shown
        h = self.planes.contiguous().view(torch.float16).view(r, k // 8, 2, 8).float()
        return ((h[:, :, 0] + h[:, :, 1]).reshape(r, k)) * self.inv_scale[:, None]


def split_supported(x: torch.Tensor) -> bool:
    return (x.is_cuda and x.dtype == torch.float32 and x.dim() == 2 and x.shape[1] % 32 == 0 and x.stride(1) == 1
            and x.stride(0) % 4 == 0 and x.data_ptr() % 16 == 0 and x.shape[0] > 0)


def split_rows(x: torch.Tensor, bias: Optional[torch.Tensor] = None, want_bound: bool = False) -> SplitRows:
    if not split_supported(x):
        raise EmcidHipError("split_rows: fp32 HBM rows with K contiguous, K % 32 == 0 and 16-byte aligned rows")
    rows, K = x.shape
    planes = torch.empty(rows, K, dtype=torch.int32, device=x.device)
    inv = torch.empty(rows, dtype=torch.float32, device=x.device)
    bound = None
    if want_bound:
        bound = torch.zeros(2, dtype=torch.float32, device=x.device)
        if bias is not None:
            bound[1:2] = bias.detach().abs().max()
    _check(load().emcid_split_rows_f16(_ptr(x, torch.float32, "x"), x.stride(0), rows, K, _ptr(planes), planes.stride(0), _ptr(inv),
                                       _ptr(bound), _stream(x)), "emcid_split_rows_f16")
    return SplitRows(planes, inv, None, bound)


def linear_sp(x: SplitRows, w: SplitRows, bias: Optional[torch.Tensor] = None, act: int = ACT_NONE,
              residual: Optional[torch.Tensor] = None, out: Optional[torch.Tensor] = None, want_f32: bool = True,
              planes_scale: Optional[torch.Tensor] = None, cfg: int = -1):
    M, K = x.planes.shape
    N = w.planes.shape[0]
    if w.planes.shape[1] != K or K % 32:
        raise EmcidHipError("linear_sp: operands (M, K) and (N, K) with K % 32 == 0")
    for t in (x.planes, w.planes):
        if t.stride(1) != 1 or t.stride(0) % 4 or t.data_ptr() % 16 or t.dtype != torch.int32:
            raise EmcidHipError("linear_sp: planes must be int32 row views with 16-byte aligned rows")
    dev = x.planes.device
    y = None
    if want_f32 or planes_scale is None:
        y = out if out is not None else torch.empty(M, N, dtype=torch.float32, device=dev)
        if y.shape != (M, N) or y.stride(1) != 1 or y.dtype != torch.float32:
            raise EmcidHipError("linear_sp: out must be an (M, N) fp32 row view")
    yp = None
    if planes_scale is not None:
        if N % 32 or planes_scale.shape != (2, M) or not planes_scale.is_contiguous():
            raise EmcidHipError("linear_sp: planes output needs N % 32 == 0 and a contiguous (2, M) scale / inverse scale")
        yp = torch.empty(M, N, dtype=torch.int32, device=dev)
    if bias is not None and (bias.shape != (N,) or not bias.is_contiguous()):
        raise EmcidHipError("linear_sp: bias must be a contiguous (N,) vector")
    if residual is not None and (residual.shape != (M, N) or residual.stride(1) != 1):
        raise EmcidHipError("linear_sp: residual must be an (M, N) row view")
    if LINEAR_FLOPS["count"]:
        LINEAR_FLOPS["flops"] += 2.0 * M * N * K
        LINEAR_FLOPS["launches"] += 1
    _check(load().emcid_linear_sp16_f32(
        _ptr(x.planes), x.planes.stride(0), _ptr(x.inv_scale, torch.float32, "x scale"), _ptr(w.planes), w.planes.stride(0),
        _ptr(w.inv_scale, torch.float32, "w scale"), _ptr(bias, torch.float32, "bias"), _ptr(residual, torch.float32, "residual"),
        residual.stride(0) if residual is not None else 0, _ptr(y), y.stride(0) if y is not None else 0, _ptr(yp),
        yp.stride(0) if yp is not None else 0, _ptr(planes_scale, torch.float32, "planes scale"), M, N, K, int(act), int(cfg),
        _stream(x.planes)), "emcid_linear_sp16_f32")
    if planes_scale is None:
        return y
    return SplitRows(yp, planes_scale[1], y)


def add_layernorm(a: torch.Tensor, b: Optional[torch.Tensor], ln: torch.nn.LayerNorm, want_sum: bool = True):
    rows, cols = a.shape
    if a.stride(1) != 1 or (b is not None and (b.stride(1) != 1 or b.shape != a.shape)):
        raise EmcidHipError("add_layernorm: (rows, cols) operands with unit column stride")
    if ln.weight is None or ln.bias is None or tuple(ln.normalized_shape) != (cols,):
        raise EmcidHipError("add_layernorm: LayerNorm over the last dimension with affine parameters")
    y = torch.empty(rows, cols, dtype=torch.float32, device=a.device) if (b is not None and want_sum) else None
    z = torch.empty(rows, cols, dtype=torch.float32, device=a.device)
    _check(load().emcid_add_layernorm_f32(_ptr(a, torch.float32, "a"), a.stride(0), _ptr(b, torch.float32, "b"),
                                          b.stride(0) if b is not None else 0,
                                          _ptr(ln.weight, torch.float32, "gamma"), _ptr(ln.bias, torch.float32, "beta"),
                                          float(ln.eps), rows, cols, _ptr(y), _ptr(z), _stream(a)), "emcid_add_layernorm_f32")
    return (a if b is None else y), z


def add_layernorm_sp(a: torch.Tensor, b: Optional[torch.Tensor], ln: torch.nn.LayerNorm, want_sum: bool = True,
                     want_f32: bool = False, bound: Optional[torch.Tensor] = None):
    rows, cols = a.shape
    if a.stride(1) != 1 or (b is not None and (b.stride(1) != 1 or b.shape != a.shape)):
        raise EmcidHipError("add_layernorm_sp: (rows, cols) operands with unit column stride")
    if ln.weight is None or ln.bias is None or tuple(ln.normalized_shape) != (cols,) or cols % 32 or cols > 2048:
        raise EmcidHipError("add_layernorm_sp: LayerNorm over the last dimension with affine parameters, cols % 32 == 0, <= 2048")
    dev = a.device
    y = torch.empty(rows, cols, dtype=torch.float32, device=dev) if (b is not None and want_sum) else None
    z = torch.empty(rows, cols, dtype=torch.float32, device=dev) if want_f32 else None
    planes = torch.empty(rows, cols, dtype=torch.int32, device=dev)
    inv = torch.empty(rows, dtype=torch.float32, device=dev)
    out_scale = torch.empty(2, rows, dtype=torch.float32, device=dev) if bound is not None else None
    _check(load().emcid_add_layernorm_sp16(_ptr(a, torch.float32, "a"), a.stride(0), _ptr(b, torch.float32, "b"),
                                           b.stride(0) if b is not None else 0,
                                           _ptr(ln.weight, torch.float32, "gamma"), _ptr(ln.bias, torch.float32, "beta"),
                                           float(ln.eps), rows, cols, _ptr(y), _ptr(z), _ptr(planes), planes.stride(0), _ptr(inv),
                                           _ptr(bound, torch.float32, "bound"), _ptr(out_scale), _stream(a)),
           "emcid_add_layernorm_sp16")
    return (a if b is None else y), SplitRows(planes, inv, z, None, out_scale)


def embed_layernorm_sp(tok_emb: torch.Tensor, pos_emb: torch.Tensor, token: torch.Tensor, position: torch.Tensor,
                       ln: torch.nn.LayerNorm):
    rows, cols = token.numel(), tok_emb.shape[1]
    if tok_emb.stride(1) != 1 or pos_emb.stride(1) != 1 or pos_emb.shape[1] != cols or position.numel() != rows:
        raise EmcidHipError("embed_layernorm_sp: embedding tables with unit column stride and one index pair per row")
    if ln.weight is None or ln.bias is None or tuple(ln.normalized_shape) != (cols,) or cols % 32 or cols > 2048:
        raise EmcidHipError("embed_layernorm_sp: LayerNorm over the last dimension with affine parameters, cols % 32 == 0, <= 2048")
    y = torch.empty(rows, cols, dtype=torch.float32, device=tok_emb.device)
    planes = torch.empty(rows, cols, dtype=torch.int32, device=tok_emb.device)
    inv = torch.empty(rows, dtype=torch.float32, device=tok_emb.device)
    _check(load().emcid_embed_layernorm_sp16(_ptr(tok_emb, torch.float32, "tok_emb"), tok_emb.stride(0), tok_emb.shape[0],
                                             _ptr(pos_emb, torch.float32, "pos_emb"), pos_emb.stride(0), pos_emb.shape[0],
                                             _ptr(token, torch.int64, "token"), _ptr(position, torch.int32, "position"),
                                             _ptr(ln.weight, torch.float32, "gamma"), _ptr(ln.bias, torch.float32, "beta"),
                                             float(ln.eps), rows, cols, _ptr(y), None, _ptr(planes), planes.stride(0), _ptr(inv),
                                             _stream(tok_emb)), "emcid_embed_layernorm_sp16")
    return y, SplitRows(planes, inv)


def tree_attention_sp_supported(anc: torch.Tensor, H: int, D: int) -> bool:
    return bool(load().emcid_tree_attention_sp16_supported(anc.shape[1], H, D)) and (H * D) % 32 == 0


def tree_attention_sp(q, k, v, anc, depth, H: int, scale=None, rows=None) -> SplitRows:
    U, HD = k.shape
    D = HD // H
    for t in (q, k, v):
        if t.stride(1) != 1 or t.shape[1] != HD:
            raise EmcidHipError("tree_attention_sp: q/k/v must be row-major")
    if k.stride(0) != v.stride(0):
        raise EmcidHipError("tree_attention_sp: k and v must share a leading dimension")
    n = U if rows is None else rows.numel()
    if q.shape[0] != n:
        raise EmcidHipError(f"tree_attention_sp: {q.shape[0]} query rows for {n} query nodes")
    planes = torch.empty(n, HD, dtype=torch.int32, device=q.device)
    inv = torch.empty(n, dtype=torch.float32, device=q.device)
    scale = float(D ** -0.5 if scale is None else scale)
    _check(load().emcid_tree_attention_sp16(
        _ptr(q, torch.float32, "q"), q.stride(0), _ptr(k, torch.float32, "k"), _ptr(v, torch.float32, "v"), k.stride(0),
        _ptr(anc, torch.int32, "anc"), anc.stride(0), _ptr(depth, torch.int32, "depth"),
        _ptr(rows, torch.int32, "rows") if rows is not None else None, n, H, D, scale, _ptr(planes), planes.stride(0), _ptr(inv),
        _stream(q)), "emcid_tree_attention_sp16")
    return SplitRows(planes, inv)


def embed_layernorm(tok_emb: torch.Tensor, pos_emb: torch.Tensor, token: torch.Tensor, position: torch.Tensor,
                    ln: torch.nn.LayerNorm):
    rows, cols = token.numel(), tok_emb.shape[1]
    if tok_emb.stride(1) != 1 or pos_emb.stride(1) != 1 or pos_emb.shape[1] != cols or position.numel() != rows:
        raise EmcidHipError("embed_layernorm: embedding tables with unit column stride and one index pair per row")
    if ln.weight is None or ln.bias is None or tuple(ln.normalized_shape) != (cols,):
        raise EmcidHipError("embed_layernorm: LayerNorm over the last dimension with affine parameters")
    y = torch.empty(rows, cols, dtype=torch.float32, device=tok_emb.device)
    z = torch.empty_like(y)
    _check(load().emcid_embed_layernorm_f32(_ptr(tok_emb, torch.float32, "tok_emb"), tok_emb.stride(0), tok_emb.shape[0],
                                            _ptr(pos_emb, torch.float32, "pos_emb"), pos_emb.stride(0), pos_emb.shape[0],
                                            _ptr(token, torch.int64, "token"), _ptr(position, torch.int32, "position"),
                                            _ptr(ln.weight, torch.float32, "gamma"), _ptr(ln.bias, torch.float32, "beta"),
                                            float(ln.eps), rows, cols, _ptr(y), _ptr(z), _stream(tok_emb)),
           "emcid_embed_layernorm_f32")
    return y, z


def tree_attention(q, k, v, anc, depth, H: int, scale=None, rows=None):
    U, HD = k.shape
    D = HD // H
    for t in (q, k, v):
        if t.stride(1) != 1 or t.shape[1] != HD:
            raise EmcidHipError("tree_attention: q/k/v must be row-major")
    if k.stride(0) != v.stride(0):
        raise EmcidHipError("tree_attention: k and v must share a leading dimension")
    n = U if rows is None else rows.numel()
    if q.shape[0] != n:
        raise EmcidHipError(f"tree_attention: {q.shape[0]} query rows for {n} query nodes")
    out = torch.empty(n, HD, dtype=torch.float32, device=q.device)
    scale = float(D ** -0.5 if scale is None else scale)
    _check(load().emcid_tree_attention_f32(
        _ptr(q, torch.float32, "q"), q.stride(0), _ptr(k, torch.float32, "k"), _ptr(v, torch.float32, "v"), k.stride(0),
        _ptr(anc, torch.int32, "anc"), anc.stride(0), _ptr(depth, torch.int32, "depth"),
        _ptr(rows, torch.int32, "rows") if rows is not None else None, n, H, D, scale, _ptr(out), out.stride(0),
        _stream(q)), "emcid_tree_attention_f32")
    return out



class ClipLayerSp16(C.Structure):
    _fields_ = [(n, C.c_void_p) for n in (
        "ln1_gamma", "ln1_beta", "ln2_gamma", "ln2_beta", "qkv_planes", "qkv_inv_scale", "qkv_bias", "out_planes",
        "out_inv_scale", "out_bias", "fc1_planes", "fc1_inv_scale", "fc1_bias", "fc1_bound", "fc2_planes", "fc2_inv_scale",
        "fc2_bias")] + [("ln1_eps", C.c_float), ("ln2_eps", C.c_float), ("act", C.c_int32), ("reserved", C.c_int32)]


_CLIP_WS = {}


def clip_workspace(dev: torch.device, rows: int, h: int, d: int) -> torch.Tensor:
    key = (dev.index if dev.index is not None else torch.cuda.current_device(), torch.cuda.current_stream(dev).cuda_stream,
           rows, h, d)
    ws = _CLIP_WS.get(key)
    if ws is None:
        if len(_CLIP_WS) >= 16:
            _CLIP_WS.clear()
        ws = _CLIP_WS[key] = torch.empty(int(load().emcid_clip_workspace_bytes(rows, h, d)), dtype=torch.uint8, device=dev)
    return ws


def clip_layers(layer_array, first: int, count: int, rows: int, h: int, d: int, heads: int, scale: float, anc: torch.Tensor,
                depth: torch.Tensor, hs: torch.Tensor, x: "SplitRows", next_ln: Optional[torch.nn.LayerNorm]):
    ws = clip_workspace(hs.device, rows, h, d)
    if LINEAR_FLOPS["count"]:
        LINEAR_FLOPS["flops"] += count * 2.0 * rows * h * (4 * h + 2 * d)
        LINEAR_FLOPS["launches"] += 4 * count
    base = C.addressof(layer_array) + first * C.sizeof(ClipLayerSp16)
    g = _ptr(next_ln.weight, torch.float32, "gamma") if next_ln is not None else None
    b = _ptr(next_ln.bias, torch.float32, "beta") if next_ln is not None else None
    _check(load().emcid_clip_layers_sp16(C.c_void_p(base), count, rows, h, d, heads, float(scale), _ptr(anc, torch.int32, "anc"),
                                         anc.stride(0), _ptr(depth, torch.int32, "depth"), _ptr(hs, torch.float32, "hs"),
                                         _ptr(x.planes), _ptr(x.inv_scale), g, b, float(next_ln.eps) if next_ln is not None else 0.0,
                                         C.c_void_p(ws.data_ptr()), ws.numel(), _stream(hs)), "emcid_clip_layers_sp16")


def clip_layer_head(layer_array, index: int, rows: int, h: int, d: int, heads: int, scale: float, anc: torch.Tensor,
                    depth: torch.Tensor, rows_sel: Optional[torch.Tensor], hs: torch.Tensor, x: "SplitRows", want_f32: bool):
    dev = hs.device
    n = rows if rows_sel is None else rows_sel.numel()
    ws = clip_workspace(dev, rows, h, d)
    mid = torch.empty(n, h, dtype=torch.float32, device=dev)
    f_planes = torch.empty(n, d, dtype=torch.int32, device=dev)
    f_scale = torch.empty(2, n, dtype=torch.float32, device=dev)
    f_f32 = torch.empty(n, d, dtype=torch.float32, device=dev) if want_f32 else None
    if LINEAR_FLOPS["count"]:
        LINEAR_FLOPS["flops"] += 2.0 * h * (rows * (3 * h if rows_sel is None else 2 * h) + n * (h if rows_sel is not None else 0)
                                            + n * h + n * d)
        LINEAR_FLOPS["launches"] += 3 if rows_sel is None else 4
    base = C.addressof(layer_array) + index * C.sizeof(ClipLayerSp16)
    _check(load().emcid_clip_layer_head_sp16(
        C.c_void_p(base), rows, h, d, heads, float(scale), _ptr(anc, torch.int32, "anc"), anc.stride(0),
        _ptr(depth, torch.int32, "depth"), _ptr(rows_sel, torch.int32, "rows") if rows_sel is not None else None, n,
        _ptr(hs, torch.float32, "hs"), _ptr(x.planes), _ptr(x.inv_scale), _ptr(mid), _ptr(f_planes), _ptr(f_scale), _ptr(f_f32),
        C.c_void_p(ws.data_ptr()), ws.numel(), _stream(hs)), "emcid_clip_layer_head_sp16")
    return mid, SplitRows(f_planes, f_scale[1], f_f32)


def clip_layer_tail(layer_array, index: int, h: int, d: int, f: "SplitRows", mid: torch.Tensor,
                    next_ln: Optional[torch.nn.LayerNorm]):
    dev = mid.device
    n = mid.shape[0]
    hs = torch.empty(n, h, dtype=torch.float32, device=dev)
    x = None
    if next_ln is not None:
        x = SplitRows(torch.empty(n, h, dtype=torch.int32, device=dev), torch.empty(n, dtype=torch.float32, device=dev))
    if LINEAR_FLOPS["count"]:
        LINEAR_FLOPS["flops"] += 2.0 * n * h * d
        LINEAR_FLOPS["launches"] += 1
    base = C.addressof(layer_array) + index * C.sizeof(ClipLayerSp16)
    _check(load().emcid_clip_layer_tail_sp16(
        C.c_void_p(base), n, h, d, _ptr(f.planes), _ptr(f.inv_scale), _ptr(mid, torch.float32, "mid"), _ptr(hs),
        _ptr(next_ln.weight, torch.float32, "gamma") if next_ln is not None else None,
        _ptr(next_ln.bias, torch.float32, "beta") if next_ln is not None else None,
        float(next_ln.eps) if next_ln is not None else 0.0, _ptr(x.planes) if x is not None else None,
        _ptr(x.inv_scale) if x is not None else None, _stream(mid)), "emcid_clip_layer_tail_sp16")
    return hs, x


def clip_edit_layer_tail(layer_array, index: int, h: int, d: int, f: "SplitRows", mid: torch.Tensor, lookup: torch.Tensor,
                         seg: torch.Tensor, zs_t: torch.Tensor, factors: "CovFactors", layer_index: int, edit_weight: float,
                         layers_left: int, W0: torch.Tensor, W: torch.Tensor, ws: "DualWorkspace", lam: Optional[float],
                         next_ln: Optional[torch.nn.LayerNorm], last: bool, want_dw: bool = True, zc_split: bool = True):
    dev = mid.device
    n = f.f32.shape[0]
    N = seg.numel() - 1
    K = torch.empty(N, d, dtype=torch.float32, device=dev)
    Zc = torch.empty(N, h, dtype=torch.float32, device=dev)
    dW = torch.empty(h, d, dtype=torch.float32, device=dev) if want_dw else None
    kp = torch.empty(N, d, dtype=torch.int32, device=dev) if zc_split else None
    ks = torch.empty(N, dtype=torch.float32, device=dev) if zc_split else None
    hs = x = None
    if not last:
        hs = torch.empty(n, h, dtype=torch.float32, device=dev)
        if next_ln is not None:
            x = SplitRows(torch.empty(n, h, dtype=torch.int32, device=dev), torch.empty(n, dtype=torch.float32, device=dev))
    lws = _linear_workspace(dev) if (d >= 2048 and -(-N // 128) * -(-h // 128) <= 128
                                     and not torch.cuda.is_current_stream_capturing()) else None
    if LINEAR_FLOPS["count"]:
        LINEAR_FLOPS["flops"] += 2.0 * N * h * d + (0.0 if last else 2.0 * n * h * d)
        LINEAR_FLOPS["launches"] += 1 if last else 2
    base = C.addressof(layer_array) + index * C.sizeof(ClipLayerSp16)
    use_inverse = layer_index in factors.have_inverse
    _check(load().emcid_clip_edit_layer_tail_sp16(
        C.c_void_p(base), n, h, d, _ptr(f.f32, torch.float32, "fc2 input"), _ptr(f.planes), _ptr(f.inv_scale),
        _ptr(mid, torch.float32, "mid"), _ptr(lookup, torch.int64, "lookup"), _ptr(seg, torch.int64, "seg"), lookup.numel(), N,
        _ptr(zs_t, torch.float32, "zs_t"), float(edit_weight), int(layers_left), factors.lam_ratio(lam), _ptr(factors.buf),
        factors.n_layers, int(layer_index), int(bool(use_inverse)), _ptr(W0, torch.float32, "W0"), _ptr(W, torch.float32, "W"),
        _ptr(dW), _ptr(K), _ptr(Zc), _ptr(kp), _ptr(ks), _ptr(ws.buf), ws.nbytes, _ptr(ws.info, torch.int32),
        C.c_void_p(lws.data_ptr()) if lws is not None else None, lws.numel() if lws is not None else 0, _ptr(hs),
        _ptr(next_ln.weight, torch.float32, "gamma") if (next_ln is not None and not last) else None,
        _ptr(next_ln.bias, torch.float32, "beta") if (next_ln is not None and not last) else None,
        float(next_ln.eps) if (next_ln is not None and not last) else 0.0, _ptr(x.planes) if x is not None else None,
        _ptr(x.inv_scale) if x is not None else None, _stream(mid)), "emcid_clip_edit_layer_tail_sp16")
    return {"K": K, "Zc": Zc, "dW": dW, "hs": hs, "x": x}



class CovFactors:

    def __init__(self, n_layers: int, d: int, device):
        self.n_layers, self.d = n_layers, d
        self.nbytes = int(load().emcid_cov_factor_workspace_bytes(n_layers, d))
        self.buf = torch.zeros(self.nbytes // 8, dtype=torch.float64, device=device)
        self.info = torch.zeros(1, dtype=torch.int32, device=device)
        self.dp = (d + NB - 1) // NB * NB
        self._inv = ((self.dp + 511) // 512) * (512 * 512 + 256 * 256)
        self.have_inverse = set()
        self.ready = None
        self.cached = False
        self.lam = None
        self.edit_weight = None

    def lam_ratio(self, lam: Optional[float]) -> float:
        if lam is None or self.lam is None or float(lam) == self.lam:
            return 1.0
        if not (lam > 0.0 and self.lam > 0.0):
            raise EmcidHipError(f"mom2_update_weight must be positive for the Cholesky path (got {lam})")
        return float(lam) / float(self.lam)

    def L(self, layer: int) -> torch.Tensor:
        o = (self.n_layers + layer) * self.dp * self.dp
        return self.buf[o:o + self.dp * self.dp].view(self.dp, self.dp)

    def X(self, layer: int) -> torch.Tensor:
        o = self.n_layers * (2 * self.dp * self.dp + self._inv) + layer * self.dp * self.dp
        return self.buf[o:o + self.dp * self.dp].view(self.dp, self.dp)


def cov_inverse(factors: "CovFactors", first: int = 0, count: Optional[int] = None):
    count = factors.n_layers - first if count is None else count
    _check(load().emcid_cov_inverse_f64(_ptr(factors.buf), factors.n_layers, factors.d, int(first), int(count),
                                        _stream(factors.buf)), "emcid_cov_inverse_f64")
    factors.have_inverse.update(range(first, first + count))


def factor_cov(covs, lam: float, edit_weight: float, factors: Optional[CovFactors] = None, inverse: bool = True) -> CovFactors:
    d = covs[0].shape[0]
    for c in covs:
        assert c.shape == (d, d) and c.is_contiguous()
    if factors is None or factors.n_layers != len(covs) or factors.d != d:
        factors = CovFactors(len(covs), d, covs[0].device)
    arr = (C.c_void_p * len(covs))(*[_ptr(c, torch.float32, "C").value for c in covs])
    _check(load().emcid_factor_cov_f64(arr, len(covs), d, float(lam), float(edit_weight), _ptr(factors.buf), factors.nbytes,
                                       _ptr(factors.info, torch.int32), _stream(covs[0])), "emcid_factor_cov_f64")
    factors.have_inverse = set()
    factors.lam, factors.edit_weight = float(lam), float(edit_weight)
    if inverse:
        cov_inverse(factors)
    return factors


def cov_factor_rescale(src: CovFactors, a: float, dst: Optional[CovFactors] = None, lam: Optional[float] = None,
                       edit_weight: Optional[float] = None) -> CovFactors:
    if not (a > 0.0 and a < 1e300):
        raise EmcidHipError(f"the scale of a factored workspace must be positive and finite (got {a})")
    with_inverse = len(src.have_inverse) == src.n_layers
    if dst is None or dst.n_layers != src.n_layers or dst.d != src.d or dst.buf.device != src.buf.device:
        dst = CovFactors(src.n_layers, src.d, src.buf.device)
    if dst is not src:
        dst.info.zero_()
    _check(load().emcid_cov_factor_rescale_f64(_ptr(src.buf), _ptr(dst.buf), dst.nbytes, src.n_layers, src.d, float(a),
                                               int(with_inverse), _stream(src.buf)), "emcid_cov_factor_rescale_f64")
    dst.have_inverse = set(range(src.n_layers)) if with_inverse else set()
    dst.lam = float(lam) if lam is not None else (src.lam * float(a) if src.lam is not None else None)
    dst.edit_weight = float(edit_weight) if edit_weight is not None else src.edit_weight
    return dst


class DualWorkspace:
    def __init__(self, N: int, d: int, h: int, device):
        self.key = (N, d, h)
        self.nbytes = int(load().emcid_edit_dual_workspace_bytes(N, d, h))
        self.buf = torch.zeros(self.nbytes // 8, dtype=torch.float64, device=device)
        self.info = torch.zeros(1, dtype=torch.int32, device=device)
        self.Np, self.dp = (N + NB - 1) // NB * NB, (d + NB - 1) // NB * NB
        pt = load().emcid_edit_dual_pt(_ptr(self.buf), N, d, h)
        off = (pt - self.buf.data_ptr()) // 8
        self.Pt = self.buf[off:off + self.Np * self.dp].view(self.Np, self.dp)
        hp = h + (h % 2)
        off = (load().emcid_edit_dual_s(_ptr(self.buf), N, d, h) - self.buf.data_ptr()) // 8
        self.S = self.buf[off:off + self.Np * self.Np].view(self.Np, self.Np)
        off = (load().emcid_edit_dual_u(_ptr(self.buf), N, d, h) - self.buf.data_ptr()) // 8
        self.U = self.buf[off:off + hp * self.dp].view(hp, self.dp)[:h]
        self.hp = hp
        Np, dp = self.Np, self.dp
        self.Kt, self.Yt = self.block("K").view(Np, dp), self.block("Y").view(Np, dp)
        self.Rt = self.block("R").view(Np, hp)
        self.LS, self.XT = self.block("LS").view(Np, Np), self.block("XT").view(Np, Np)
        self.RT = self.block("PT").view(dp, Np)
        self.V = self.block("V").view(hp, dp)[:h]
        self.sk_counters = self.block("SK_COUNTERS")

    def block(self, name: str) -> torch.Tensor:
        n = C.c_int64(0)
        at = load().emcid_edit_dual_block(_ptr(self.buf), *self.key, DUAL_BLOCKS.index(name), C.byref(n))
        if not at or n.value < 0:
            raise EmcidHipError(f"no block {name!r} in a dual workspace")
        off = (at - self.buf.data_ptr()) // 8
        return self.buf[off:off + n.value]

    def schur_form(self) -> str:
        return SCHUR_FORMS[load().emcid_edit_dual_schur_form(*self.key)]


def full_inverse(L: torch.Tensor, inv: torch.Tensor, scratch: torch.Tensor):
    X = torch.zeros_like(L)
    _check(load().emcid_full_inverse_f64(_ptr(L, torch.float64), L.shape[0], L.stride(0), _ptr(inv), _ptr(X), _ptr(scratch),
                                         scratch.numel(), _stream(L)), "emcid_full_inverse_f64")
    return X


def edit_layer_dual(K, Zc, zs_t, factors: CovFactors, layer_index: int, edit_weight: float, layers_left: int,
                    W0=None, W=None, want_factors: bool = False, want_dw: bool = True, ws: Optional[DualWorkspace] = None,
                    rows=None, gather_pt=None, use_inverse: Optional[bool] = None, lam: Optional[float] = None):
    if use_inverse is None:
        use_inverse = layer_index in factors.have_inverse
    N, d = K.shape
    h = Zc.shape[1]
    for t, nm in ((K, "K"), (Zc, "Zc"), (zs_t, "zs_t")):
        assert t.is_contiguous(), nm
    assert zs_t.shape == (N, h) and factors.d == d
    if ws is None or ws.key != (N, d, h):
        ws = DualWorkspace(N, d, h, K.device)
    lo, hi = rows if rows is not None else (0, N)
    lib = load()
    _check(lib.emcid_edit_dual_stage1_f64(
        _ptr(K, torch.float32, "K"), _ptr(Zc, torch.float32, "Zc"), _ptr(zs_t, torch.float32, "zs_t"), N, d, h,
        float(edit_weight), int(layers_left), factors.lam_ratio(lam), _ptr(factors.buf), factors.n_layers, int(layer_index), lo, hi,
        int(bool(use_inverse)), _ptr(ws.buf), ws.nbytes, _stream(K)), "emcid_edit_dual_stage1_f64")
    if gather_pt is not None:
        ws.Pt[:N].copy_(gather_pt(ws.Pt[lo:hi]))
    dev = K.device
    adj_k = torch.empty(d, N, dtype=torch.float64, device=dev) if want_factors else None
    Rt = torch.empty(N, h, dtype=torch.float64, device=dev) if want_factors else None
    dW = torch.empty(h, d, dtype=torch.float32, device=dev) if want_dw else None
    if W is not None:
        assert W.is_contiguous() and W.shape == (h, d) and W0 is not None and W0.is_contiguous()
    _check(lib.emcid_edit_dual_stage2_f64(N, d, h, factors.lam_ratio(lam), _ptr(W0, torch.float32, "W0"), _ptr(W, torch.float32, "W"), _ptr(adj_k),
                                          _ptr(Rt), _ptr(dW), _ptr(ws.buf), ws.nbytes, _ptr(ws.info, torch.int32),
                                          _stream(K)), "emcid_edit_dual_stage2_f64")
    return {"adj_k": adj_k, "Rt": Rt, "dW": dW, "ws": ws}


def column_tiles(rank: int, world: int, n_tiles: int):
    load_ = [0] * world
    owner = {}
    for t in range(n_tiles - 1, -1, -1):
        r = min(range(world), key=lambda i: (load_[i], i))
        owner[t] = r
        load_[r] += t + 1
    return [t for t in range(n_tiles) if owner[t] == rank]


class _HipColsBackend:

    def __init__(self, K, Zc, zs_t, factors, layer_index, edit_weight, layers_left, ws, lam=None):
        self.a = (K, Zc, zs_t, factors, layer_index, edit_weight, layers_left, ws)
        self.lam_ratio = factors.lam_ratio(lam)

    def stage1(self, tiles):
        K, Zc, zs_t, factors, layer_index, edit_weight, layers_left, ws = self.a
        N, d = K.shape
        arr = (C.c_int * len(tiles))(*tiles)
        _check(load().emcid_edit_dual_cols_stage1_f64(
            _ptr(K, torch.float32, "K"), _ptr(Zc, torch.float32, "Zc"), _ptr(zs_t, torch.float32, "zs_t"), N, d, Zc.shape[1],
            float(edit_weight), int(layers_left), self.lam_ratio, _ptr(factors.buf), factors.n_layers, int(layer_index), arr,
            len(tiles), _ptr(ws.buf), ws.nbytes, _stream(K)), "emcid_edit_dual_cols_stage1_f64")
        return ws.S

    def stage2(self, tiles):
        K, Zc, zs_t, factors, layer_index, edit_weight, layers_left, ws = self.a
        N, d = K.shape
        arr = (C.c_int * len(tiles))(*tiles)
        _check(load().emcid_edit_dual_cols_stage2_f64(N, d, Zc.shape[1], _ptr(factors.buf), factors.n_layers, int(layer_index), arr,
                                                      len(tiles), _ptr(ws.buf), ws.nbytes, _ptr(ws.info, torch.int32), _stream(K)),
               "emcid_edit_dual_cols_stage2_f64")
        return ws.U

    def apply(self, U, W0, W, want_dw):
        K, Zc = self.a[0], self.a[1]
        h, d = Zc.shape[1], K.shape[1]
        dW = torch.empty(h, d, dtype=torch.float32, device=K.device) if want_dw else None
        _check(load().emcid_apply_update2d_f32(_ptr(U), U.stride(0), _ptr(W0, torch.float32, "W0"), _ptr(W, torch.float32, "W"),
                                               _ptr(dW), h, d, _stream(K)), "emcid_apply_update2d_f32")
        return dW


def edit_layer_dual_cols(K, Zc, zs_t, factors, layer_index: int, edit_weight: float, layers_left: int, W0, W,
                         tiles, all_reduce, want_dw: bool = True, ws: Optional["DualWorkspace"] = None, backend=None,
                         lam: Optional[float] = None):
    N, d = K.shape
    h = Zc.shape[1]
    tiles = sorted(int(t) for t in tiles)
    if not tiles:
        raise EmcidHipError("a rank without a column tile: world size exceeds d / 128")
    if backend is None:
        for t, nm in ((K, "K"), (Zc, "Zc"), (zs_t, "zs_t"), (W, "W"), (W0, "W0")):
            assert t.is_contiguous(), nm
        assert zs_t.shape == (N, h) and factors.d == d and W.shape == (h, d)
        if layer_index not in factors.have_inverse:
            raise EmcidHipError("edit_layer_dual_cols needs the explicit inverse factor of the layer (cov_inverse)")
        if ws is None or ws.key != (N, d, h):
            ws = DualWorkspace(N, d, h, K.device)
        backend = _HipColsBackend(K, Zc, zs_t, factors, layer_index, edit_weight, layers_left, ws, lam)
    S = backend.stage1(tiles)
    all_reduce(S)
    U = backend.stage2(tiles)
    all_reduce(U)
    dW = backend.apply(U, W0, W, want_dw)
    return {"dW": dW, "ws": ws}


def edit_layer_dual_apply(K, Zc, zs_t, factors: CovFactors, layer_index: int, edit_weight: float, layers_left: int,
                          W0, W, want_dw: bool = True, ws: Optional[DualWorkspace] = None,
                          use_inverse: Optional[bool] = None, on_factor_start=None, lam: Optional[float] = None):
    if use_inverse is None:
        use_inverse = layer_index in factors.have_inverse
    N, d = K.shape
    h = Zc.shape[1]
    for t, nm in ((K, "K"), (Zc, "Zc"), (zs_t, "zs_t"), (W, "W"), (W0, "W0")):
        assert t.is_contiguous(), nm
    assert zs_t.shape == (N, h) and factors.d == d and W.shape == (h, d)
    if ws is None or ws.key != (N, d, h):
        ws = DualWorkspace(N, d, h, K.device)
    lib = load()
    _check(lib.emcid_edit_dual_apply_stage1_f64(
        _ptr(K, torch.float32, "K"), _ptr(Zc, torch.float32, "Zc"), _ptr(zs_t, torch.float32, "zs_t"), N, d, h,
        float(edit_weight), int(layers_left), factors.lam_ratio(lam), _ptr(factors.buf), factors.n_layers, int(layer_index), 0, N,
        int(bool(use_inverse)), _ptr(ws.buf), ws.nbytes, _stream(K)), "emcid_edit_dual_apply_stage1_f64")
    dW = torch.empty(h, d, dtype=torch.float32, device=K.device) if want_dw else None
    if on_factor_start is not None:
        _check(lib.emcid_edit_dual_apply_assemble_f64(N, d, h, _ptr(ws.buf), ws.nbytes, _stream(K)),
               "emcid_edit_dual_apply_assemble_f64")
        on_factor_start()
    _check(lib.emcid_edit_dual_apply_stage2_f64(N, d, h, _ptr(factors.buf), factors.n_layers, int(layer_index),
                                                int(bool(use_inverse)), int(on_factor_start is not None),
                                                _ptr(W0, torch.float32, "W0"), _ptr(W, torch.float32, "W"), _ptr(dW),
                                                _ptr(ws.buf), ws.nbytes, _ptr(ws.info, torch.int32), _stream(K)),
           "emcid_edit_dual_apply_stage2_f64")
    return {"dW": dW, "ws": ws}


def check_preserved_state(sd, n_layers: int, d: int, capacity: int) -> int:
    def bad(what):
        return EmcidHipError(f"preserved key state: {what}")

    if not isinstance(sd, dict):
        raise bad(f"a dict is expected (got {type(sd).__name__})")
    missing = [k for k in ("M", "d", "n_layers", "Yp", "Lp", "tile_inv", "row_scale") if k not in sd]
    if missing:
        raise bad(f"no entry {missing}")
    M = sd["M"]
    if isinstance(M, bool) or not isinstance(M, int) or M < 0:
        raise bad(f"M must be a non-negative integer (got {M!r})")
    if sd["d"] != d:
        raise bad(f"its rows are of width d = {sd['d']}, this state's of d = {d}")
    if sd["n_layers"] != n_layers:
        raise bad(f"it holds {sd['n_layers']} layers, this state {n_layers}")
    if M > capacity:
        raise bad(f"its M = {M} committed rows exceed this state's capacity {capacity}")
    tiles = (M + NB - 1) // NB
    for name, shape in (("Yp", (M, d)), ("Lp", (M, M)), ("tile_inv", (tiles, NB, NB))):
        ts = sd[name]
        if not isinstance(ts, (list, tuple)) or len(ts) != n_layers:
            raise bad(f"{name} must be a list of {n_layers} tensors")
        for i, t in enumerate(ts):
            if not isinstance(t, torch.Tensor) or t.dtype != torch.float64 or tuple(t.shape) != shape:
                got = (tuple(t.shape), t.dtype) if isinstance(t, torch.Tensor) else type(t).__name__
                raise bad(f"{name}[{i}] must be an f64 tensor of {shape} for M = {M}, d = {d} (got {got})")
    rs = sd["row_scale"]
    if not isinstance(rs, torch.Tensor) or rs.dtype != torch.float64 or tuple(rs.shape) != (M,):
        raise bad(f"row_scale must be an f64 tensor of ({M},)")
    return M


class PreservedKeys:

    def __init__(self, n_layers: int, d: int, capacity: int, device):
        if capacity < 1:
            raise EmcidHipError(f"the capacity of a preserved key set must be positive (got {capacity})")
        self.n_layers, self.d, self.capacity, self.M = int(n_layers), int(d), int(capacity), 0
        self.dp = (d + NB - 1) // NB * NB
        self.ldl = self.capacity + (self.capacity % 2)
        tiles = (self.capacity + NB - 1) // NB
        self.Yp = [torch.zeros(self.capacity, self.dp, dtype=torch.float64, device=device) for _ in range(n_layers)]
        self.Lp = [torch.zeros(self.capacity, self.ldl, dtype=torch.float64, device=device) for _ in range(n_layers)]
        self.tile_inv = [torch.zeros(tiles, NB, NB, dtype=torch.float64, device=device) for _ in range(n_layers)]
        self.row_scale = torch.ones(self.capacity, dtype=torch.float64)

    def commit(self, N: int, scale: float = 1.0):
        assert self.M + N <= self.capacity
        self.row_scale[self.M:self.M + int(N)] = float(scale)
        self.M += int(N)

    def release_commit(self, keep):
        keep = check_keep(keep, self.M)[0]
        self.row_scale[:len(keep)] = self.row_scale[torch.as_tensor(keep, dtype=torch.long)]
        self.M = len(keep)

    def rescale_commit(self, factors):
        f = check_factors(factors, self.M)
        self.row_scale[:self.M] *= f

    def reset(self):
        self.M = 0

    def snapshot(self, first: int, end: int) -> "KeySnapshot":
        return KeySnapshot(self, first, end)

    def state_dict(self, sync: bool = True) -> dict:
        M, d, tiles = self.M, self.d, (self.M + NB - 1) // NB
        w = M - NB * (tiles - 1)

        def host(t: torch.Tensor) -> torch.Tensor:
            return pinned_copy(t) if t.is_cuda else t.clone()

        def tile_part(ti: torch.Tensor) -> torch.Tensor:
            ti = ti[:tiles].clone()
            if tiles and w < NB:
                ti[-1, w:, :] = 0
                ti[-1, :, w:] = 0
            return ti

        sd = {"M": M, "d": d, "n_layers": self.n_layers,
              "Yp": [host(y[:M, :d].contiguous()) for y in self.Yp],
              "Lp": [host(l[:M, :M].contiguous()) for l in self.Lp],
              "tile_inv": [host(tile_part(t)) for t in self.tile_inv],
              "row_scale": self.row_scale[:M].clone()}
        if sync and self.Yp[0].is_cuda:
            torch.cuda.current_stream(self.Yp[0].device).synchronize()
        return sd

    def load_state_dict(self, sd: dict):
        M = check_preserved_state(sd, self.n_layers, self.d, self.capacity)
        tiles = (M + NB - 1) // NB
        for i in range(self.n_layers):
            self.Yp[i][:M, :self.d].copy_(sd["Yp"][i])
            self.Yp[i][:M, self.d:].zero_()
            self.Lp[i][:M, :M].copy_(sd["Lp"][i])
            self.tile_inv[i][:tiles].copy_(sd["tile_inv"][i])
        self.row_scale[:M] = sd["row_scale"]
        self.M = M

    def check_layer(self, layer_index: int):
        if not 0 <= layer_index < self.n_layers:
            raise EmcidHipError(f"layer index {layer_index} outside the session state's {self.n_layers} layers")

    def layer_args(self, layer_index: int):
        self.check_layer(layer_index)
        Yp, Lp, Ti = self.Yp[layer_index], self.Lp[layer_index], self.tile_inv[layer_index]
        for t, nm in ((Yp, "Yp"), (Lp, "Lp"), (Ti, "tile_inv")):
            assert t.stride(-1) == 1 and (t.dim() < 3 or t.is_contiguous()), nm
        return (_ptr(Yp, torch.float64, "Yp"), Yp.stride(0), _ptr(Lp, torch.float64, "Lp"), Lp.stride(0),
                _ptr(Ti, torch.float64, "tile_inv"), self.capacity, self.M)

    @property
    def nbytes(self) -> int:
        return sum(t.numel() * 8 for ts in (self.Yp, self.Lp, self.tile_inv) for t in ts)


class KeySnapshot:

    def __init__(self, state: PreservedKeys, first: int, end: int):
        self.state, self.rows = state, slice(first, end)
        self.tiles = slice(first // NB, (end + NB - 1) // NB if end > first else first // NB)
        self.Yp = [t[self.rows].clone() for t in state.Yp]
        self.Lp = [t[self.rows].clone() for t in state.Lp]
        self.tile_inv = [t[self.tiles].clone() for t in state.tile_inv]
        self.row_scale = state.row_scale[:state.M if end > first else 0].clone()

    def restore(self):
        s = self.state
        for kept, live, part in ((self.Yp, s.Yp, self.rows), (self.Lp, s.Lp, self.rows), (self.tile_inv, s.tile_inv, self.tiles)):
            for k, t in zip(kept, live):
                t[part].copy_(k)
        s.row_scale[:self.row_scale.numel()] = self.row_scale


class _SessionWorkspace:

    @classmethod
    def fitting(cls, ws, device, *dims):
        return ws if ws is not None and ws.key == dims else cls(*dims, device)

    def __init__(self, what: str, size_fn, dims: dict, device):
        self.key = tuple(dims.values())
        self.nbytes = int(size_fn(*self.key))
        if self.nbytes <= 0:
            raise EmcidHipError(f"no {what} workspace for " + ", ".join(f"{k}={v}" for k, v in dims.items()))
        self.buf = torch.zeros(self.nbytes // 8, dtype=torch.float64, device=device)
        self.info = torch.zeros(1, dtype=torch.int32, device=device)


class PreserveWorkspace(_SessionWorkspace):

    def __init__(self, N: int, d: int, h: int, capacity: int, device):
        super().__init__("preserve", load().emcid_edit_dual_preserve_workspace_bytes, dict(N=N, d=d, h=h, capacity=capacity), device)


class RetainWorkspace(_SessionWorkspace):

    def __init__(self, N: int, d: int, capacity: int, device):
        super().__init__("retain", load().emcid_session_retain_workspace_bytes, dict(N=N, d=d, capacity=capacity), device)


class ReleaseWorkspace(_SessionWorkspace):

    def __init__(self, n_rebuilt: int, d: int, capacity: int, device):
        super().__init__("release", load().emcid_session_release_workspace_bytes, dict(n_rebuilt=n_rebuilt, d=d, capacity=capacity),
                         device)


def edit_layer_dual_preserve(K, Zc, zs_t, factors: CovFactors, layer_index: int, edit_weight: float, layers_left: int,
                             W0, W, state: PreservedKeys, want_dw: bool = True, want_u: bool = False,
                             ws: Optional[PreserveWorkspace] = None, lam: Optional[float] = None):
    N, d = K.shape
    h = Zc.shape[1]
    for t, nm in ((K, "K"), (Zc, "Zc"), (zs_t, "zs_t")) + (((W, "W"), (W0, "W0")) if W is not None else ()):
        assert t.is_contiguous(), nm
    assert zs_t.shape == (N, h) and factors.d == d == state.d and (W is None or W.shape == (h, d))
    state.check_layer(layer_index)
    if layer_index not in factors.have_inverse:
        raise EmcidHipError("edit_layer_dual_preserve needs the explicit inverse factor of the layer (cov_inverse)")
    if state.M + N > state.capacity:
        raise EmcidHipError(f"{state.M} preserved + {N} new rows exceed the state's capacity {state.capacity}")
    ws = PreserveWorkspace.fitting(ws, K.device, N, d, h, state.capacity)
    dW = torch.empty(h, d, dtype=torch.float32, device=K.device) if want_dw else None
    U = torch.empty(h, d, dtype=torch.float64, device=K.device) if want_u else None
    _check(load().emcid_edit_layer_dual_preserve_f64(
        _ptr(K, torch.float32, "K"), _ptr(Zc, torch.float32, "Zc"), _ptr(zs_t, torch.float32, "zs_t"), N, d, h,
        float(edit_weight), int(layers_left), factors.lam_ratio(lam), _ptr(factors.buf), factors.n_layers, int(layer_index),
        *state.layer_args(layer_index), _ptr(W0, torch.float32, "W0"), _ptr(W, torch.float32, "W"), _ptr(dW), _ptr(U),
        _ptr(ws.buf), ws.nbytes, _ptr(ws.info, torch.int32), _stream(K)), "emcid_edit_layer_dual_preserve_f64")
    return {"dW": dW, "U": U, "ws": ws}


def row_scale_of(edit_weight: float, factors: CovFactors, lam: Optional[float] = None, weight: float = 1.0) -> float:
    return math.sqrt(float(weight) * float(edit_weight) / 0.5) / math.sqrt(factors.lam_ratio(lam))


def session_retain(K, factors: CovFactors, layer_index: int, row_scale: float, state: PreservedKeys,
                   ws: Optional[RetainWorkspace] = None, lam: Optional[float] = None):
    N, d = K.shape
    assert K.is_contiguous(), "K"
    assert factors.d == d == state.d
    state.check_layer(layer_index)
    if layer_index not in factors.have_inverse:
        raise EmcidHipError("session_retain needs the explicit inverse factor of the layer (cov_inverse)")
    if state.M + N > state.capacity:
        raise EmcidHipError(f"{state.M} preserved + {N} retained rows exceed the state's capacity {state.capacity}")
    row_scale = float(row_scale)
    if not (row_scale > 0.0 and row_scale < float("inf")):
        raise EmcidHipError(f"row_scale must be positive and finite (got {row_scale})")
    ws = RetainWorkspace.fitting(ws, K.device, N, d, state.capacity)
    _check(load().emcid_session_retain_f64(
        _ptr(K, torch.float32, "K"), N, d, row_scale, factors.lam_ratio(lam), _ptr(factors.buf), factors.n_layers, int(layer_index),
        *state.layer_args(layer_index), _ptr(ws.buf), ws.nbytes, _ptr(ws.info, torch.int32), _stream(K)), "emcid_session_retain_f64")
    return {"ws": ws}


def check_keep(keep, M: int):
    keep = [int(i) for i in keep]
    if any(i < 0 or i >= M for i in keep) or any(b <= a for a, b in zip(keep, keep[1:])):
        raise EmcidHipError(f"keep must be strictly ascending row indices inside [0, {M})")
    first = next((j for j, i in enumerate(keep) if i != j), len(keep))
    return keep, first


def session_release(state: PreservedKeys, layer_index: int, keep, first: Optional[int] = None, ws: Optional[ReleaseWorkspace] = None):
    state.check_layer(layer_index)
    Yp = state.Yp[layer_index]
    if isinstance(keep, torch.Tensor) and keep.is_cuda:
        if first is None:
            raise EmcidHipError("session_release: a device tensor of kept rows needs `first`")
        keep_dev, n_keep, first = keep, int(keep.numel()), int(first)
        if keep_dev.dtype != torch.int32 or not keep_dev.is_contiguous() or keep_dev.device != Yp.device:
            raise EmcidHipError(f"session_release: keep must be a contiguous int32 tensor on {Yp.device}")
    else:
        rows, f = check_keep(keep.tolist() if isinstance(keep, torch.Tensor) else keep, state.M)
        if first is not None and int(first) != f:
            raise EmcidHipError(f"session_release: first = {first}, but the smallest released row of keep is {f}")
        keep_dev, n_keep, first = None, len(rows), f
    if not 0 <= first <= n_keep <= state.M:
        raise EmcidHipError(f"session_release: first = {first}, {n_keep} kept rows, {state.M} committed")
    if n_keep == state.M or first == n_keep:
        return {"ws": None, "launched": False, "first": first}
    if keep_dev is None:
        keep_dev = torch.tensor(rows, dtype=torch.int32, device=Yp.device)
    ws = ReleaseWorkspace.fitting(ws, Yp.device, n_keep - first, state.d, state.capacity)
    _check(load().emcid_session_release_f64(
        _ptr(keep_dev, torch.int32, "keep"), n_keep, first, state.d, *state.layer_args(layer_index),
        _ptr(ws.buf), ws.nbytes, _ptr(ws.info, torch.int32), _stream(Yp)), "emcid_session_release_f64")
    return {"ws": ws, "launched": True, "first": first}


def check_factors(factors, M: int) -> torch.Tensor:
    try:
        f = torch.as_tensor(factors, dtype=torch.float64, device="cpu").detach()
    except (TypeError, ValueError, RuntimeError) as e:
        raise EmcidHipError(f"row factors must be numbers: {e}") from e
    if f.dim() == 0:
        f = f.repeat(M)
    if f.dim() != 1 or f.numel() != M:
        raise EmcidHipError(f"{tuple(f.shape)} row factors for {M} committed rows")
    if not bool((torch.isfinite(f) & (f > 0.0)).all()):
        raise EmcidHipError("row factors must be positive and finite")
    return f.contiguous()


class RescaleWorkspace(_SessionWorkspace):

    def __init__(self, n_rebuilt: int, d: int, capacity: int, device):
        super().__init__("rescale", load().emcid_session_retain_workspace_bytes, dict(n_rebuilt=n_rebuilt, d=d, capacity=capacity),
                         device)


def session_rescale(state: PreservedKeys, layer_index: int, factors, first: Optional[int] = None, src: Optional[torch.Tensor] = None,
                    ws: Optional[RescaleWorkspace] = None):
    state.check_layer(layer_index)
    Yp, M = state.Yp[layer_index], state.M
    if isinstance(factors, torch.Tensor) and factors.is_cuda:
        if first is None:
            raise EmcidHipError("session_rescale: a device tensor of factors needs `first`")
        if factors.dtype != torch.float64 or not factors.is_contiguous() or factors.numel() != M or factors.device != Yp.device:
            raise EmcidHipError(f"session_rescale: factors must be a contiguous f64 tensor of {M} elements on {Yp.device}")
        f_dev, first = factors, int(first)
    else:
        f = check_factors(factors, M)
        changed = torch.nonzero(f != 1.0).flatten()
        lowest = int(changed[0]) if changed.numel() else M
        if first is None:
            first = 0 if src is not None else lowest
        first = int(first)
        if not 0 <= first <= M:
            raise EmcidHipError(f"session_rescale: first = {first}, {M} committed")
        if first > lowest:
            raise EmcidHipError(f"session_rescale: first = {first}, but row {lowest} has the factor {float(f[lowest])}")
        f_dev = None
    if not 0 <= first <= M:
        raise EmcidHipError(f"session_rescale: first = {first}, {M} committed")
    if first == M:
        return {"ws": None, "launched": False, "first": first}
    if not Yp.is_cuda:
# ... 246 lines not shown
```

include/emcid_hip.h:

```cpp
#ifndef EMCID_HIP_H
#define EMCID_HIP_H

#include <stdint.h>

#ifdef __cplusplus
extern "C" {
#endif

#define EMCID_OK 0
#define EMCID_ERR_BAD_ARG (-1)
#define EMCID_ERR_HIP (-2)
#define EMCID_ERR_WORKSPACE (-3)

#define EMCID_ABI_VERSION 16

int emcid_abi_version(void);
const char* emcid_last_error(void);

#define EMCID_PROF_CLASSES 16
int emcid_profile_enable(unsigned class_mask);
int emcid_profile_collect(double* ms_per_class_host, int64_t* launches_per_class_host, int n_classes);

int emcid_gram_accumulate_f32(const float* X, int64_t t, int64_t d, int64_t ldx,
                              float* G, int64_t ldg, int ksplit, void* stream);
int emcid_symmetrize_lower_f32(float* G, int64_t d, int64_t ldg, void* stream);

int emcid_gather_mean_f32(const float* act, int64_t B, int64_t S, int64_t c, int64_t ldb, int64_t lds_,
                          const int64_t* idx, const int64_t* seg, int64_t N,
                          float* out, int64_t ldo, void* stream);

int emcid_attention_f32(const float* q, const float* k, const float* v, int64_t sb, int64_t sh, int64_t ss,
                        const void* mask, int mask_kind, int64_t mb, int64_t mi, int causal, float scale,
                        int64_t B, int64_t H, int64_t S, int64_t D, float* out, void* stream);

int emcid_tree_attention_f32(const float* q, int64_t ldq, const float* k, const float* v, int64_t ld, const int* anc, int64_t anc_ld,
                             const int* depth, const int* rows, int64_t n_rows, int64_t H, int64_t D, float scale,
                             float* out, int64_t ldo, void* stream);

int emcid_quick_gelu_f32(const float* x, float* y, int64_t n, void* stream);

int emcid_linear_f32(const float* X, int64_t ldx, const float* W, int64_t ldw, const float* bias, const float* residual,
                     int64_t ldr, float* Y, int64_t ldy, int64_t M, int64_t N, int64_t K, int act, int cfg, void* stream);

int64_t emcid_linear_workspace_bytes(void);
int emcid_linear_ws_f32(const float* X, int64_t ldx, const float* W, int64_t ldw, const float* bias, const float* residual,
                        int64_t ldr, float* Y, int64_t ldy, int64_t M, int64_t N, int64_t K, int act, int cfg, void* workspace,
                        int64_t workspace_bytes, void* stream);

int emcid_split_rows_f16(const float* X, int64_t ldx, int64_t rows, int64_t K, void* planes, int64_t ldp, float* inv_scale,
                         float* max_row_norm, void* stream);

int emcid_linear_sp16_f32(const void* Xp, int64_t ldx, const float* x_inv_scale, const void* Wp, int64_t ldw,
                          const float* w_inv_scale, const float* bias, const float* residual, int64_t ldr, float* Y, int64_t ldy,
                          void* Yp, int64_t ldp, const float* y_scale, int64_t M, int64_t N, int64_t K, int act, int cfg,
                          void* stream);

int emcid_debug_linear_sp16_stamps(long long* stamps_dev);
int64_t emcid_gram_sp16_workspace_bytes(int64_t d);
int64_t emcid_gram_sp16_workspace_bytes_for(int64_t d, int64_t t);
int emcid_gram_accumulate_sp16_f32(const float* X, const float* row_weight, int64_t t, int64_t d, int64_t ldx, float* G, int64_t ldg,
                                   void* workspace, int64_t workspace_bytes, void* stream);

int emcid_add_layernorm_sp16(const float* a, int64_t lda, const float* b, int64_t ldb, const float* gamma, const float* beta,
                             float eps, int64_t rows, int64_t cols, float* y, float* z, void* planes, int64_t ldp,
                             float* inv_scale, const float* bound, float* out_scale, void* stream);
int emcid_embed_layernorm_sp16(const float* tok, int64_t ld_tok, int64_t n_tok, const float* pos, int64_t ld_pos, int64_t n_pos,
                               const int64_t* token, const int* position, const float* gamma, const float* beta, float eps,
                               int64_t rows, int64_t cols, float* y, float* z, void* planes, int64_t ldp, float* inv_scale,
                               void* stream);
int emcid_tree_attention_sp16_supported(int64_t anc_ld, int64_t H, int64_t D);
int emcid_tree_attention_sp16(const float* q, int64_t ldq, const float* k, const float* v, int64_t ld, const int* anc,
                              int64_t anc_ld, const int* depth, const int* rows, int64_t n_rows, int64_t H, int64_t D, float scale,
                              void* planes, int64_t ldp, float* inv_scale, void* stream);

int emcid_fingerprint_store(int64_t n, const void* const* data, const int64_t* bytes, const int64_t* slots, void* table,
                            int64_t table_slots, void* stream);
int emcid_fingerprint_check(const void* table, int64_t table_slots, int64_t first_slot, int64_t n_slots, const uint64_t* skip_mask,
                            int* flag, void* stream);

int emcid_fingerprint_content(int64_t n, const void* const* data, const int64_t* bytes, uint64_t* out_dev, void* stream);

typedef struct emcid_clip_layer_sp16 {
    const float* ln1_gamma; const float* ln1_beta;
    const float* ln2_gamma; const float* ln2_beta;
    const void* qkv_planes; const float* qkv_inv_scale; const float* qkv_bias;
    const void* out_planes; const float* out_inv_scale; const float* out_bias;
    const void* fc1_planes; const float* fc1_inv_scale; const float* fc1_bias; const float* fc1_bound;
    const void* fc2_planes; const float* fc2_inv_scale; const float* fc2_bias;
    float ln1_eps, ln2_eps;
    int32_t act, reserved;
} emcid_clip_layer_sp16;

int64_t emcid_clip_workspace_bytes(int64_t rows, int64_t h, int64_t d);

int emcid_clip_layer_head_sp16(const emcid_clip_layer_sp16* L, int64_t rows, int64_t h, int64_t d, int64_t heads, float attn_scale,
                               const int* anc, int64_t anc_ld, const int* depth, const int* rows_sel, int64_t n_sel,
                               const float* hs, const void* x_planes, const float* x_inv_scale, float* mid, void* f_planes,
                               float* f_scale, float* f_f32, void* workspace, int64_t workspace_bytes, void* stream);

int emcid_clip_layer_tail_sp16(const emcid_clip_layer_sp16* L, int64_t n, int64_t h, int64_t d, const void* f_planes,
                               const float* f_inv_scale, const float* mid, float* hs_out, const float* next_ln_gamma,
                               const float* next_ln_beta, float next_ln_eps, void* x_planes, float* x_inv_scale, void* stream);

int emcid_clip_edit_layer_tail_sp16(const emcid_clip_layer_sp16* L, int64_t n_rows, int64_t h, int64_t d, const float* f_f32,
                                    const void* f_planes, const float* f_inv_scale, const float* mid, const int64_t* lookup,
                                    const int64_t* seg, int64_t B, int64_t N, const float* zs_t, double edit_weight,
                                    int layers_left, double lam_ratio, const void* cov_factor_ws, int64_t n_layers,
                                    int64_t layer_index, int use_inverse, const float* W0, float* W, float* dW, float* K_out,
                                    float* Zc_out, void* k_planes, float* k_inv_scale, void* dual_ws, int64_t dual_ws_bytes,
                                    int* info_dev, void* linear_ws, int64_t linear_ws_bytes, float* hs_out,
                                    const float* next_ln_gamma, const float* next_ln_beta, float next_ln_eps, void* x_planes,
                                    float* x_inv_scale, void* stream);

int emcid_clip_layers_sp16(const emcid_clip_layer_sp16* layers, int64_t n_layers, int64_t rows, int64_t h, int64_t d, int64_t heads,
                           float attn_scale, const int* anc, int64_t anc_ld, const int* depth, float* hs, void* x_planes,
                           float* x_inv_scale, const float* next_ln_gamma, const float* next_ln_beta, float next_ln_eps,
                           void* workspace, int64_t workspace_bytes, void* stream);

int emcid_add_layernorm_f32(const float* a, int64_t lda, const float* b, int64_t ldb, const float* gamma, const float* beta,
                            float eps, int64_t rows, int64_t cols, float* y, float* z, void* stream);

int emcid_embed_layernorm_f32(const float* tok, int64_t ld_tok, int64_t n_tok, const float* pos, int64_t ld_pos, int64_t n_pos,
                              const int64_t* token, const int* position, const float* gamma, const float* beta, float eps,
                              int64_t rows, int64_t cols, float* y, float* z, void* stream);

int64_t emcid_edit_workspace_bytes(int64_t N, int64_t d, int64_t h);

int emcid_edit_layer_f64(const float* K, const float* Zc, const float* zs_t, const float* C,
                         int64_t N, int64_t d, int64_t h,
                         double lam, double edit_weight, int layers_left,
                         const float* W0, float* W,
                         double* Xt_out, double* Rt_out, float* dW_out,
                         void* workspace, int64_t workspace_bytes, int* info_dev, void* stream);
int emcid_cov_inverse_f64(void* cov_factor_ws, int64_t n_layers, int64_t d, int64_t first_layer, int64_t count, void* stream);

int emcid_edit_layer_shard_f64(const float* K, const float* Zc, const float* zs_t, const float* C,
                               int64_t N, int64_t d, int64_t h, double lam, double edit_weight, int layers_left,
                               int64_t n_lo, int64_t n_hi, double* U_partial, double* Xt_out, double* Rt_out,
                               void* workspace, int64_t workspace_bytes, int* info_dev, void* stream);
int emcid_apply_update_f32(const double* U, const float* W0, float* W, float* dW, int64_t n, void* stream);

int64_t emcid_cov_factor_workspace_bytes(int64_t n_layers, int64_t d);
int emcid_factor_cov_f64(const float* const* C_host_list, int64_t n_layers, int64_t d, double lam, double edit_weight,
                         void* workspace, int64_t workspace_bytes, int* info_dev, void* stream);
int emcid_cov_factor_rescale_f64(const void* src_ws, void* dst_ws, int64_t workspace_bytes, int64_t n_layers, int64_t d, double a,
                                 int with_inverse, void* stream);
int64_t emcid_edit_dual_workspace_bytes(int64_t N, int64_t d, int64_t h);
enum {
    EMCID_DUAL_K = 0, EMCID_DUAL_P = 1, EMCID_DUAL_Y = 2, EMCID_DUAL_R = 3, EMCID_DUAL_S = 4, EMCID_DUAL_LS = 5,
    EMCID_DUAL_INVS = 6, EMCID_DUAL_PT = 7, EMCID_DUAL_Y2 = 8, EMCID_DUAL_V = 9, EMCID_DUAL_U = 10, EMCID_DUAL_SK = 11,
    EMCID_DUAL_XT = 12, EMCID_DUAL_TT = 13, EMCID_DUAL_SK_COUNTERS = 14
};
double* emcid_edit_dual_block(void* workspace, int64_t N, int64_t d, int64_t h, int which, int64_t* doubles_out);
enum { EMCID_SCHUR_XROW = 0, EMCID_SCHUR_FULL_INVERSE = 1, EMCID_SCHUR_SUBSTITUTION = 2 };
int emcid_edit_dual_schur_form(int64_t N, int64_t d, int64_t h);
int emcid_edit_dual_stage1_f64(const float* K, const float* Zc, const float* zs_t, int64_t N, int64_t d, int64_t h,
                               double edit_weight, int layers_left, double lam_ratio, const void* cov_factor_ws, int64_t n_layers,
                               int64_t layer_index, int64_t n_lo, int64_t n_hi, int use_inverse, void* workspace,
                               int64_t workspace_bytes, void* stream);
double* emcid_edit_dual_pt(void* workspace, int64_t N, int64_t d, int64_t h);
int emcid_edit_dual_stage2_f64(int64_t N, int64_t d, int64_t h, double lam_ratio, const float* W0, float* W, double* adjk_out, double* Rt_out,
                               float* dW_out, void* workspace, int64_t workspace_bytes, int* info_dev, void* stream);

int emcid_edit_dual_apply_stage1_f64(const float* K, const float* Zc, const float* zs_t, int64_t N, int64_t d, int64_t h,
                                     double edit_weight, int layers_left, double lam_ratio, const void* cov_factor_ws, int64_t n_layers,
                                     int64_t layer_index, int64_t n_lo, int64_t n_hi, int use_inverse, void* workspace,
                                     int64_t workspace_bytes, void* stream);
double* emcid_edit_dual_yt(void* workspace, int64_t N, int64_t d, int64_t h);
int emcid_edit_dual_apply_stage2_f64(int64_t N, int64_t d, int64_t h, const void* cov_factor_ws, int64_t n_layers,
                                     int64_t layer_index, int use_inverse, int assembled, const float* W0, float* W,
                                     float* dW_out, void* workspace, int64_t workspace_bytes, int* info_dev, void* stream);
int emcid_edit_dual_apply_assemble_f64(int64_t N, int64_t d, int64_t h, void* workspace, int64_t workspace_bytes, void* stream);

int64_t emcid_edit_dual_preserve_workspace_bytes(int64_t N, int64_t d, int64_t h, int64_t capacity);
int emcid_edit_layer_dual_preserve_f64(const float* K, const float* Zc, const float* zs_t, int64_t N, int64_t d, int64_t h,
                                       double edit_weight, int layers_left, double lam_ratio, const void* cov_factor_ws,
                                       int64_t n_layers, int64_t layer_index, double* Yp, int64_t ldy, double* Lp, int64_t ldl,
                                       double* tile_inv, int64_t capacity, int64_t M, const float* W0, float* W, float* dW_out,
                                       double* U_out, void* workspace, int64_t workspace_bytes, int* info_dev, void* stream);

int64_t emcid_session_retain_workspace_bytes(int64_t N, int64_t d, int64_t capacity);
int emcid_session_retain_f64(const float* K, int64_t N, int64_t d, double row_scale, double lam_ratio, const void* cov_factor_ws,
                             int64_t n_layers, int64_t layer_index, double* Yp, int64_t ldy, double* Lp, int64_t ldl,
                             double* tile_inv, int64_t capacity, int64_t M, void* workspace, int64_t workspace_bytes, int* info_dev,
                             void* stream);

int64_t emcid_session_release_workspace_bytes(int64_t n_rebuilt, int64_t d, int64_t capacity);
int emcid_session_release_f64(const int32_t* keep_dev, int64_t n_keep, int64_t first, int64_t d, double* Yp, int64_t ldy, double* Lp,
                              int64_t ldl, double* tile_inv, int64_t capacity, int64_t M, void* workspace, int64_t workspace_bytes,
                              int* info_dev, void* stream);

int emcid_session_rescale_f64(const double* factors_dev, const double* src_Yp, int64_t lds, int64_t first, int64_t d, double* Yp,
                              int64_t ldy, double* Lp, int64_t ldl, double* tile_inv, int64_t capacity, int64_t M, void* workspace,
                              int64_t workspace_bytes, int* info_dev, void* stream);

int emcid_session_step_norms_f64(const void* workspace, int64_t workspace_bytes, int64_t N, int64_t d, int64_t h, int64_t capacity,
                                 int64_t M, double* drift_out, double* left_out, double* resid_out, void* stream);

int64_t emcid_cov_factor_fold_workspace_bytes(int64_t M, int64_t d);
int emcid_cov_factor_fold_f64(const void* src_ws, double lam_ratio, const double* Yp, int64_t ldy, int64_t M, int64_t capacity,
                              const float* C, double lam, double edit_weight, int fill_base, void* dst_ws, int64_t n_layers,
                              int64_t d, int64_t layer_index, double* base, void* workspace, int64_t workspace_bytes,
                              int* info_dev, void* stream);

int emcid_session_refold_update_f64(void* cov_ws, int64_t n_layers, int64_t d, int64_t layer_index, const double* Yp, int64_t ldy,
                                    int64_t M, int64_t capacity, double* archive, int64_t lda, int64_t n_archived,
                                    const int32_t* rel_idx_dev, int64_t n_rel, double* base, void* stream);
int emcid_cov_factor_refactor_f64(void* cov_ws, int64_t workspace_bytes, int64_t n_layers, int64_t d, int* info_dev, void* stream);

int emcid_score_rows_f32(const float* a, int64_t lda, const float* b, int64_t ldb, const float* t, int64_t ldt, const float* gamma,
                         const float* beta, float eps, int64_t rows, int64_t cols, double* out, void* stream);
int emcid_score_chains_f64(const double* node, int64_t U, const int32_t* anc, int64_t ld_anc, const int32_t* depth,
                           const int64_t* end_node, int64_t B, double* out, void* stream);
int emcid_score_chains_pair_f64(const double* node1, int64_t U1, const int32_t* anc1, int64_t ld_anc1, const int32_t* depth1,
                                const int64_t* end1, const double* node2, int64_t U2, const int32_t* anc2, int64_t ld_anc2,
                                const int32_t* depth2, const int64_t* end2, int64_t B, double* out, void* stream);
int emcid_score_chains_pair_grid_f64(const double* node1, int64_t G1, int64_t U1, const int32_t* anc1, int64_t ld_anc1,
                                     const int32_t* depth1, const int64_t* end1, const double* node2, int64_t G2, int64_t U2,
                                     const int32_t* anc2, int64_t ld_anc2, const int32_t* depth2, const int64_t* end2, int64_t B,
                                     const int32_t* combo, int64_t C, double* out, void* stream);
int emcid_score_pooled_f32(const float* a, int64_t lda, const float* b, int64_t ldb, const float* gamma, const float* beta, float eps,
                           const float* P, int64_t ldp, int64_t rows, int64_t cols, int64_t proj, double* out, void* stream);

int64_t emcid_edit_lu_workspace_bytes(int64_t N, int64_t d, int64_t h);
int emcid_edit_layer_lu_f64(const float* K, const float* Zc, const float* zs_t, const float* C,
                            int64_t N, int64_t d, int64_t h, double lam, double edit_weight, int layers_left,
                            const float* W0, float* W, double* adjk_out, double* Rt_out, float* dW_out,
                            void* workspace, int64_t workspace_bytes, int* info_dev, void* stream);
int emcid_lu_solve_f64(double* A, int64_t lda, int64_t n, double* B, int64_t ldb, int64_t nrhs, int* piv_dev,
                       int* info_dev, void* stream);

int emcid_edit_dual_cols_stage1_f64(const float* K, const float* Zc, const float* zs_t, int64_t N, int64_t d, int64_t h,
                                    double edit_weight, int layers_left, double lam_ratio, const void* cov_factor_ws, int64_t n_layers,
                                    int64_t layer_index, const int* tiles_host, int n_tiles, void* workspace,
                                    int64_t workspace_bytes, void* stream);
double* emcid_edit_dual_s(void* workspace, int64_t N, int64_t d, int64_t h);
double* emcid_edit_dual_u(void* workspace, int64_t N, int64_t d, int64_t h);
int emcid_edit_dual_cols_stage2_f64(int64_t N, int64_t d, int64_t h, const void* cov_factor_ws, int64_t n_layers,
                                    int64_t layer_index, const int* tiles_host, int n_tiles, void* workspace,
                                    int64_t workspace_bytes, int* info_dev, void* stream);
int emcid_apply_update2d_f32(const double* U, int64_t ldu, const float* W0, float* W, float* dW, int64_t h, int64_t d,
                             void* stream);


int emcid_assemble_spd_f64(const float* C, int64_t ldc, const double* Kt64, int64_t Np, int64_t d, int64_t ldk,
                           double lam, float cw, double* A, int64_t lda, void* stream);
int64_t emcid_inverse_workspace_doubles(int64_t dp);
int emcid_debug_leaf_stamps(const double* A, double* L, double* inv, int* info_dev, long long* stamps_dev, void* stream);
int emcid_cholesky_f64(double* A, double* L, int64_t dp, int64_t lda, double* invdiag, int* info_dev, void* stream);
int emcid_cholesky_solve_f64(const double* L, int64_t dp, int64_t lda, const double* invdiag,
                             double* Bt, double* Yt, int64_t Np, int64_t ldb, void* stream);
int64_t emcid_full_inverse_scratch_doubles(int64_t dp, int64_t lda);
int emcid_full_inverse_f64(const double* L, int64_t dp, int64_t lda, const double* invdiag, double* X, double* scratch,
                           int64_t scratch_doubles, void* stream);
int emcid_delta_w_f64(const double* Rt, int64_t ldr, const double* Xt, int64_t ldx, int64_t Np, int64_t h, int64_t d,
                      const float* W0, float* W, int64_t ldw, float* dW, double* U, void* stream);

int emcid_dgemm_f64(int ta, int tb, int64_t M, int64_t N, int64_t K, double alpha,
                    const double* A, int64_t lda, const double* B, int64_t ldb,
                    double beta, double* C, int64_t ldc, void* stream);
int emcid_dgemm_ex_f64(int ta, int tb, int64_t M, int64_t N, int64_t K, double alpha,
                       const double* A, int64_t lda, const double* B, int64_t ldb,
                       double beta, double* C, int64_t ldc, int flags, int cfg, int ksplit, void* stream);

int64_t emcid_streamk_workspace_bytes(int wgs);
int emcid_dgemm_streamk_f64(int tb, int64_t M, int64_t N, int64_t K, double alpha, const double* A, int64_t lda,
                            const double* B, int64_t ldb, double* C, int64_t ldc, int flags, int wgs, double diag_add,
                            void* workspace, int64_t workspace_bytes, void* stream);

int emcid_debug_streamk_stamps(long long* stamps_dev);
int emcid_debug_step_stamps(long long* stamps_dev);

int emcid_dgemm_batched_f64(int ta, int tb, int64_t M, int64_t N, int64_t K, double alpha,
                            const double* A, int64_t lda, int64_t sA, const double* B, int64_t ldb, int64_t sB,
                            double beta, double* C, int64_t ldc, int64_t sC, int64_t batch, void* stream);

int emcid_axpy_f32(float* W, const float* dW, int64_t n, void* stream);

#ifdef __cplusplus
}
#endif
#endif
```

Before: 110,900.

## Fuse edit key prep, residual transpose, and query-row gathers into single kernels

Merges the three gather launches in the layer head into one kernel that copies plane rows, hs rows and scales together. In the edit tail, a new key-prep kernel computes the segment mean, fp16 split planes, scale and the padded f64 Kt matrix in one pass. A separate kernel writes the residual directly in transposed f64 layout, so stage 2 can skip its transpose. This removes several launches and intermediate round trips to global memory, in exchange for more specialised entry points and a second code path that has to stay consistent with the old stage-1 prep.

```diff
diff --git a/emcid_amd/csrc/clip_layers.hip b/emcid_amd/csrc/clip_layers.hip
--- a/emcid_amd/csrc/clip_layers.hip
+++ b/emcid_amd/csrc/clip_layers.hip
@@ -4,20 +4,22 @@
 
 namespace emcid {
 
-__global__ __launch_bounds__(256) void gather_rows16_kernel(const unsigned char* __restrict__ src, int64_t src_stride,
-                                                             const int* __restrict__ idx, unsigned char* __restrict__ dst,
-                                                             int64_t dst_stride, int row_bytes) {
+__global__ __launch_bounds__(256) void gather_query_rows_kernel(const unsigned char* __restrict__ planes, const float* __restrict__ scale,
+                                                                 const unsigned char* __restrict__ hs, const int* __restrict__ idx,
+                                                                 unsigned char* __restrict__ planes_out, float* __restrict__ scale_out,
+                                                                 unsigned char* __restrict__ hs_out, int row_bytes) {
     typedef unsigned int v4u __attribute__((ext_vector_type(4)));
-    const int64_t r = blockIdx.x;
-    const v4u* s = reinterpret_cast<const v4u*>(src + (int64_t)idx[r] * src_stride);
-    v4u* d = reinterpret_cast<v4u*>(dst + r * dst_stride);
-    for (int i = threadIdx.x; i < row_bytes / 16; i += 256) d[i] = s[i];
-}
-
-__global__ __launch_bounds__(256) void gather_f32_kernel(const float* __restrict__ src, const int* __restrict__ idx,
-                                                          float* __restrict__ dst, int n) {
-    const int i = blockIdx.x * 256 + threadIdx.x;
-    if (i < n) dst[i] = src[idx[i]];
+    const int64_t r = blockIdx.x, src = idx[r];
+    const v4u* ps = reinterpret_cast<const v4u*>(planes + src * row_bytes);
+    const v4u* hsrc = reinterpret_cast<const v4u*>(hs + src * row_bytes);
+    v4u* pd = reinterpret_cast<v4u*>(planes_out + r * row_bytes);
+    v4u* hd = reinterpret_cast<v4u*>(hs_out + r * row_bytes);
+    for (int i = threadIdx.x; i < row_bytes / 16; i += 256) {
+        const v4u a = ps[i], b = hsrc[i];
+        pd[i] = a;
+        hd[i] = b;
+    }
+    if (threadIdx.x == 0) scale_out[r] = scale[src];
 }
 
 __device__ __forceinline__ unsigned long long fp_mix(unsigned long long x) {
@@ -177,6 +179,18 @@
 
 int64_t emcid_clip_workspace_bytes(int64_t rows, int64_t h, int64_t d) { return clip_ws_bytes(rows, h, d); }
 
+int emcid_gather_query_rows(const void* x_planes, const float* x_inv_scale, const float* hs, const int* rows_sel, int64_t n_sel,
+                            int64_t h, void* planes_out, float* scale_out, float* hs_out, void* stream) {
+    EMCID_CHECK_ARG(x_planes && x_inv_scale && hs && rows_sel && planes_out && scale_out && hs_out && n_sel > 0 && n_sel < (1LL << 31));
+    EMCID_CHECK_ARG(h > 0 && h % 4 == 0 && h < (1 << 24) && aligned16(x_planes) && aligned16(hs) && aligned16(planes_out) && aligned16(hs_out));
+    hipStream_t st = (hipStream_t)stream;
+    ScopedProf sp(KC_MISC, st);
+    hipLaunchKernelGGL(gather_query_rows_kernel, dim3((unsigned)n_sel), dim3(256), 0, st, (const unsigned char*)x_planes, x_inv_scale,
+                       (const unsigned char*)hs, rows_sel, (unsigned char*)planes_out, scale_out, (unsigned char*)hs_out, (int)(4 * h));
+    EMCID_CHECK_LAUNCH();
+    return EMCID_OK;
+}
+
 int emcid_clip_layer_head_sp16(const emcid_clip_layer_sp16* L, int64_t rows, int64_t h, int64_t d, int64_t heads, float attn_scale,
                                const int* anc, int64_t anc_ld, const int* depth, const int* rows_sel, int64_t n_sel,
                                const float* hs, const void* x_planes, const float* x_inv_scale, float* mid, void* f_planes,
@@ -185,7 +199,6 @@
     EMCID_CHECK_ARG(mid && f_planes && f_scale && n_sel > 0 && n_sel <= rows && (rows_sel != nullptr || n_sel == rows) && h % 32 == 0 && d % 32 == 0);
     ClipWs w;
     if (!clip_ws_carve(workspace, workspace_bytes, rows, h, d, w)) return fail(EMCID_ERR_BAD_ARG, __func__, "workspace too small or misaligned");
-    hipStream_t st = (hipStream_t)stream;
     const int64_t D = h / heads;
     const float* q;
     int64_t ldq;
@@ -198,16 +211,7 @@
         EMCID_TRY(emcid_linear_sp16_f32(x_planes, h, x_inv_scale, (const uint32_t*)L->qkv_planes + h * h, h, L->qkv_inv_scale + h,
                                         L->qkv_bias ? L->qkv_bias + h : nullptr, nullptr, 0, w.qkv + h, 3 * h, nullptr, 0, nullptr,
                                         rows, 2 * h, h, 0, -1, stream));
-        {
-            ScopedProf sp(KC_MISC, st);
-            hipLaunchKernelGGL(gather_rows16_kernel, dim3((unsigned)n_sel), dim3(256), 0, st, (const unsigned char*)x_planes, 4 * h,
-                               rows_sel, (unsigned char*)w.xq_p, 4 * h, (int)(4 * h));
-            hipLaunchKernelGGL(gather_f32_kernel, dim3((unsigned)((n_sel + 255) / 256)), dim3(256), 0, st, x_inv_scale, rows_sel,
-                               w.xq_s, (int)n_sel);
-            hipLaunchKernelGGL(gather_rows16_kernel, dim3((unsigned)n_sel), dim3(256), 0, st, (const unsigned char*)hs, 4 * h,
-                               rows_sel, (unsigned char*)w.hs_q, 4 * h, (int)(4 * h));
-            EMCID_CHECK_LAUNCH();
-        }
+        EMCID_TRY(emcid_gather_query_rows(x_planes, x_inv_scale, hs, rows_sel, n_sel, h, w.xq_p, w.xq_s, w.hs_q, stream));
         EMCID_TRY(emcid_linear_sp16_f32(w.xq_p, h, w.xq_s, L->qkv_planes, h, L->qkv_inv_scale, L->qkv_bias, nullptr, 0, w.mid, h,
                                         nullptr, 0, nullptr, n_sel, h, h, 0, -1, stream));
         q = w.mid, ldq = h, res = w.hs_q;
@@ -248,19 +252,25 @@
                                     float* x_inv_scale, void* stream) {
     EMCID_CHECK_ARG(L && n_rows > 0 && h % 32 == 0 && d % 32 == 0 && f_f32 && lookup && seg && B > 0 && N > 0 && zs_t);
     EMCID_CHECK_ARG(cov_factor_ws && W0 && W && K_out && Zc_out && dual_ws && info_dev && (hs_out == nullptr || (f_planes && f_inv_scale && mid)));
-    EMCID_TRY(emcid_gather_mean_f32(f_f32, B, n_rows, d, 0, d, lookup, seg, N, K_out, d, stream));
     EMCID_CHECK_ARG((k_planes == nullptr) == (k_inv_scale == nullptr));
     if (k_planes != nullptr) {
-        EMCID_TRY(emcid_split_rows_f16(K_out, d, N, d, k_planes, d, k_inv_scale, nullptr, stream));
+        EMCID_TRY(emcid_edit_key_prep_f64(f_f32, n_rows, lookup, seg, B, N, d, h, edit_weight, lam_ratio, K_out, k_planes, k_inv_scale,
+                                          dual_ws, dual_ws_bytes, stream));
         EMCID_TRY(emcid_linear_sp16_f32(k_planes, d, k_inv_scale, L->fc2_planes, d, L->fc2_inv_scale, L->fc2_bias, nullptr, 0, Zc_out, h,
                                         nullptr, 0, nullptr, N, h, d, 0, -1, stream));
+        EMCID_TRY(emcid_edit_residual_t_f64(Zc_out, zs_t, N, d, h, edit_weight, layers_left, lam_ratio, dual_ws, dual_ws_bytes, stream));
+        EMCID_TRY(emcid_edit_dual_apply_stage1_prepared_f64(N, d, h, cov_factor_ws, n_layers, layer_index, 0, N, use_inverse, dual_ws,
+                                                            dual_ws_bytes, stream));
+        EMCID_TRY(emcid_edit_dual_apply_stage2_rt_f64(N, d, h, cov_factor_ws, n_layers, layer_index, use_inverse, 0, 1, W0, W, dW,
+                                                      dual_ws, dual_ws_bytes, info_dev, stream));
     } else {
+        EMCID_TRY(emcid_gather_mean_f32(f_f32, B, n_rows, d, 0, d, lookup, seg, N, K_out, d, stream));
         EMCID_TRY(emcid_linear_ws_f32(K_out, d, W, d, L->fc2_bias, nullptr, 0, Zc_out, h, N, h, d, 0, -1, linear_ws, linear_ws_bytes, stream));
-    }
-    EMCID_TRY(emcid_edit_dual_apply_stage1_f64(K_out, Zc_out, zs_t, N, d, h, edit_weight, layers_left, lam_ratio, cov_factor_ws,
-                                               n_layers, layer_index, 0, N, use_inverse, dual_ws, dual_ws_bytes, stream));
-    EMCID_TRY(emcid_edit_dual_apply_stage2_f64(N, d, h, cov_factor_ws, n_layers, layer_index, use_inverse, 0, W0, W, dW, dual_ws,
-                                               dual_ws_bytes, info_dev, stream));
+        EMCID_TRY(emcid_edit_dual_apply_stage1_f64(K_out, Zc_out, zs_t, N, d, h, edit_weight, layers_left, lam_ratio, cov_factor_ws,
+                                                   n_layers, layer_index, 0, N, use_inverse, dual_ws, dual_ws_bytes, stream));
+        EMCID_TRY(emcid_edit_dual_apply_stage2_f64(N, d, h, cov_factor_ws, n_layers, layer_index, use_inverse, 0, W0, W, dW, dual_ws,
+                                                   dual_ws_bytes, info_dev, stream));
+    }
     if (hs_out != nullptr) {
         EMCID_TRY(emcid_split_rows_f16(W, d, h, d, const_cast<void*>(L->fc2_planes), d, const_cast<float*>(L->fc2_inv_scale), nullptr,
                                        stream));
diff --git a/emcid_amd/csrc/edit_solve.hip b/emcid_amd/csrc/edit_solve.hip
--- a/emcid_amd/csrc/edit_solve.hip
+++ b/emcid_amd/csrc/edit_solve.hip
@@ -1,4 +1,5 @@
 #include "spd_solve.h"
+#include "sp16.h"
 
 namespace emcid {
 
@@ -30,6 +31,129 @@
     ScopedProf sp(KC_PREP, st);
     hipLaunchKernelGGL(prep_kr_kernel, dim3((unsigned)Np), dim3(256), 0, st, K, Zc, zs_t, (int)N, (int)d, (int)h, sqrt(edit_weight / 0.5),
                        (double)layers_left, Kt, (int)Np, (int)dp, R, (int)hp, gain);
+}
+
+constexpr int KP_REG = 2;
+typedef float kp_v4f __attribute__((ext_vector_type(4)));
+typedef unsigned int kp_v4u __attribute__((ext_vector_type(4)));
+typedef _Float16 kp_v8h __attribute__((ext_vector_type(8)));
+
+__device__ __forceinline__ void key_prep_mean8(const float* __restrict__ f, int64_t ldf, int64_t n_rows,
+                                               const int64_t* __restrict__ idx, int64_t p0, int64_t p1, int col, kp_v4f& a, kp_v4f& b) {
+    kp_v4f sa = {0.f, 0.f, 0.f, 0.f}, sb = {0.f, 0.f, 0.f, 0.f};
+    for (int64_t p = p0; p < p1; ++p) {
+        int64_t r = idx[p];
+        r = r < 0 ? 0 : (r >= n_rows ? n_rows - 1 : r);
+        const float* x = f + r * ldf + col;
+        sa += *reinterpret_cast<const kp_v4f*>(x);
+        sb += *reinterpret_cast<const kp_v4f*>(x + 4);
+    }
+    const float cnt = (float)(p1 - p0);
+#pragma unroll
+    for (int e = 0; e < 4; ++e) {
+        a[e] = (p1 > p0) ? sa[e] / cnt : 0.f;
+        b[e] = (p1 > p0) ? sb[e] / cnt : 0.f;
+    }
+}
+
+__device__ __forceinline__ void key_prep_emit8(const kp_v4f& a, const kp_v4f& b, float sc, double s, double g, uint32_t* __restrict__ p,
+                                               double* __restrict__ kt) {
+    kp_v8h hi, lo;
+#pragma unroll
+    for (int e = 0; e < 8; ++e) {
+        const float x = e < 4 ? a[e] : b[e - 4];
+        const float t = x * sc;
+        hi[e] = (_Float16)t;
+        lo[e] = (_Float16)(t - (float)hi[e]);
+    }
+    *reinterpret_cast<kp_v4u*>(p) = *reinterpret_cast<kp_v4u*>(&hi);
+    *reinterpret_cast<kp_v4u*>(p + 4) = *reinterpret_cast<kp_v4u*>(&lo);
+#pragma unroll
+    for (int e = 0; e < 8; e += 2) {
+        double2 v;
+        v.x = (double)(e < 4 ? a[e] : b[e - 4]) * s * g;
+        v.y = (double)(e < 4 ? a[e + 1] : b[e - 3]) * s * g;
+        *reinterpret_cast<double2*>(kt + e) = v;
+    }
+}
+
+__global__ __launch_bounds__(256) void key_prep_kernel(const float* __restrict__ f, int64_t ldf, int64_t n_rows,
+                                                        const int64_t* __restrict__ idx, const int64_t* __restrict__ seg, int N,
+                                                        int d, int dp, double s, double g, float* __restrict__ K_out,
+                                                        uint32_t* __restrict__ P, float* __restrict__ inv_scale,
+                                                        double* __restrict__ Kt64) {
+    __shared__ float wmax[4];
+    const int n = blockIdx.x, tid = threadIdx.x;
+    double* kt = Kt64 + (int64_t)n * dp;
+    if (n >= N) {
+        const double2 z = {0.0, 0.0};
+        for (int j = tid; j < dp / 2; j += 256) reinterpret_cast<double2*>(kt)[j] = z;
+        return;
+    }
+    const int64_t p0 = seg[n], p1 = seg[n + 1];
+    const int ng = d / 8;
+    float* k = K_out + (int64_t)n * d;
+    kp_v4f a[KP_REG], b[KP_REG];
+    float amax = 0.f;
+#pragma unroll
+    for (int u = 0; u < KP_REG; ++u) {
+        const int gi = tid + 256 * u;
+        a[u] = b[u] = (kp_v4f){0.f, 0.f, 0.f, 0.f};
+        if (gi < ng) {
+            key_prep_mean8(f, ldf, n_rows, idx, p0, p1, 8 * gi, a[u], b[u]);
+            *reinterpret_cast<kp_v4f*>(k + 8 * gi) = a[u];
+            *reinterpret_cast<kp_v4f*>(k + 8 * gi + 4) = b[u];
+#pragma unroll
+            for (int e = 0; e < 4; ++e) amax = fmaxf(amax, fmaxf(fabsf(a[u][e]), fabsf(b[u][e])));
+        }
+    }
+    for (int gi = tid + 256 * KP_REG; gi < ng; gi += 256) {
+        kp_v4f xa, xb;
+        key_prep_mean8(f, ldf, n_rows, idx, p0, p1, 8 * gi, xa, xb);
+        *reinterpret_cast<kp_v4f*>(k + 8 * gi) = xa;
+        *reinterpret_cast<kp_v4f*>(k + 8 * gi + 4) = xb;
+#pragma unroll
+        for (int e = 0; e < 4; ++e) amax = fmaxf(amax, fmaxf(fabsf(xa[e]), fabsf(xb[e])));
+    }
+#pragma unroll
+    for (int o = 32; o > 0; o >>= 1) amax = fmaxf(amax, __shfl_xor(amax, o, 64));
+    if ((tid & 63) == 0) wmax[tid >> 6] = amax;
+    __syncthreads();
+    amax = fmaxf(fmaxf(wmax[0], wmax[1]), fmaxf(wmax[2], wmax[3]));
+    float sc, inv;
+    sp_scale_of(amax, sc, inv);
+    if (tid == 0) inv_scale[n] = inv;
+    uint32_t* p = P + (int64_t)n * d;
+#pragma unroll
+    for (int u = 0; u < KP_REG; ++u) {
+        const int gi = tid + 256 * u;
+        if (gi < ng) key_prep_emit8(a[u], b[u], sc, s, g, p + 8 * gi, kt + 8 * gi);
+    }
+    for (int gi = tid + 256 * KP_REG; gi < ng; gi += 256) {
+        const kp_v4f xa = *reinterpret_cast<const kp_v4f*>(k + 8 * gi), xb = *reinterpret_cast<const kp_v4f*>(k + 8 * gi + 4);
+        key_prep_emit8(xa, xb, sc, s, g, p + 8 * gi, kt + 8 * gi);
+    }
+    for (int j = d + tid; j < dp; j += 256) kt[j] = 0.0;
+}
+
+__global__ __launch_bounds__(256) void residual_t_kernel(const float* __restrict__ Zc, const float* __restrict__ zs_t, int N, int h,
+                                                          double s, double layers_left, double g, double* __restrict__ RT, int Np,
+                                                          int hp) {
+    __shared__ double tile[32][33];
+    const int bx = blockIdx.x * 32, by = blockIdx.y * 32;
+    const int tx = threadIdx.x & 31, ty = threadIdx.x >> 5;
+    for (int r = ty; r < 32; r += 8) {
+        const int n = by + r, i = bx + tx;
+        double v = 0.0;
+        if (n < N && i < h) {
+            const float src = zs_t[(int64_t)n * h + i] - Zc[(int64_t)n * h + i];
+            v = ((double)src * s) / layers_left * g;
+        }
+        tile[r][tx] = v;
+    }
+    __syncthreads();
+    for (int r = ty; r < 32; r += 8)
+        if (bx + r < hp) RT[(int64_t)(bx + r) * Np + by + tx] = tile[tx][r];
 }
 
 __global__ __launch_bounds__(256) void axpy_f32_kernel(float* __restrict__ W, const float* __restrict__ dW, int64_t n) {
@@ -120,11 +244,12 @@
 };
 
 int solve_schur_rhs(const double* R, int64_t hp, int64_t h, int64_t Np, const double* LS, const double* invS, const double* XT,
-                    double* full_inv, double* RT, double* Y2, int64_t y2_doubles, hipStream_t st) {
+                    double* full_inv, double* RT, double* Y2, int64_t y2_doubles, hipStream_t st, bool rt_ready) {
     if (y2_doubles < hp * Np) return fail(EMCID_ERR_WORKSPACE, __func__, "RT / Y2 hold fewer than h rows of Np (h > d rounded up to 128)");
     const int form = schur_rhs_form(Np, XT != nullptr, full_inv != nullptr, y2_doubles);
-    hipLaunchKernelGGL(transpose_f64_kernel, dim3((unsigned)((hp + 31) / 32), (unsigned)(Np / 32)), dim3(256), 0, st, R, hp, RT, Np,
-                       (int)Np, (int)hp);
+    if (!rt_ready)
+        hipLaunchKernelGGL(transpose_f64_kernel, dim3((unsigned)((hp + 31) / 32), (unsigned)(Np / 32)), dim3(256), 0, st, R, hp, RT,
+                           Np, (int)Np, (int)hp);
     if (form == EMCID_SCHUR_XROW) {
         ScopedProf sp(KC_TRSM_DIAG, st);
         GemmShape f{RT, Np, XT, Np, (int)h, (int)Np, (int)Np, 0};
@@ -445,20 +570,12 @@
     return EMCID_OK;
 }
 
-int emcid_edit_dual_apply_stage1_f64(const float* K, const float* Zc, const float* zs_t, int64_t N, int64_t d, int64_t h,
-                                     double edit_weight, int layers_left, double lam_ratio, const void* cov_factor_ws, int64_t n_layers,
-                                     int64_t layer_index, int64_t n_lo, int64_t n_hi, int use_inverse, void* workspace,
-                                     int64_t workspace_bytes, void* stream) {
-    EMCID_CHECK_DUAL_STAGE1_ARGS();
-    DualWorkspace ws(N, d, h);
-    EMCID_CHECK_WORKSPACE(workspace_bytes, ws.total * (int64_t)sizeof(double), "");
-    hipStream_t st = (hipStream_t)stream;
-    double* base = (double*)workspace;
-    double *Kt = base + ws.off_K, *Bs = base + ws.off_P, *Yt = base + ws.off_Y, *R = base + ws.off_R;
+static int apply_stage1_rows(const DualWorkspace& ws, int64_t N, int64_t d, const void* cov_factor_ws, int64_t n_layers, int64_t layer_index,
+                             int64_t n_lo, int64_t n_hi, int use_inverse, double* base, hipStream_t st) {
+    double *Kt = base + ws.off_K, *Bs = base + ws.off_P, *Yt = base + ws.off_Y;
     const int64_t dp = ws.dp;
     const CovFactorLayout cov(n_layers, d);
     const double *Lb = cov.L(cov_factor_ws, layer_index), *Ib = cov.I(cov_factor_ws, layer_index);
-    launch_prep_kr(K, Zc, zs_t, N, d, h, edit_weight, layers_left, 1.0 / sqrt(lam_ratio), Kt, ws.Np, dp, R, ws.hp, st);
     const int64_t rows = n_hi - n_lo;
     if (use_inverse) {
         const int64_t gemm_rows = (n_lo == 0 && n_hi == N) ? ws.Np : rows;
@@ -466,16 +583,39 @@
                               base + ws.off_SK);
         if (gemm_rows != ws.Np && ws.Np > N)
             hipLaunchKernelGGL(zero_f64_kernel, dim3(256), dim3(256), 0, st, Yt + N * dp, (ws.Np - N) * dp);
-        EMCID_CHECK_LAUNCH();
-        return EMCID_OK;
+        return check_launch("emcid_edit_dual_apply_stage1_f64");
     }
     if (ws.Np > N) hipLaunchKernelGGL(zero_f64_kernel, dim3(256), dim3(256), 0, st, Yt + N * dp, (ws.Np - N) * dp);
     if (hipMemcpyAsync(Bs + n_lo * dp, Kt + n_lo * dp, rows * dp * sizeof(double), hipMemcpyDeviceToDevice, st) != hipSuccess)
-        return fail(EMCID_ERR_HIP, __func__, "hipMemcpyAsync");
+        return fail(EMCID_ERR_HIP, "emcid_edit_dual_apply_stage1_f64", "hipMemcpyAsync");
     return with_graph(make_key(GRAPH_APPLY_STAGE1,{Lb, Ib, Bs + n_lo * dp, Yt + n_lo * dp}, {dp, rows}), st, [&](hipStream_t q) {
         trsm_forward(Lb, dp, dp, OB, Ib, Bs + n_lo * dp, dp, Yt + n_lo * dp, dp, (int)rows, q);
         return check_launch("emcid_edit_dual_apply_stage1_f64");
     });
+}
+
+int emcid_edit_dual_apply_stage1_f64(const float* K, const float* Zc, const float* zs_t, int64_t N, int64_t d, int64_t h,
+                                     double edit_weight, int layers_left, double lam_ratio, const void* cov_factor_ws, int64_t n_layers,
+                                     int64_t layer_index, int64_t n_lo, int64_t n_hi, int use_inverse, void* workspace,
+                                     int64_t workspace_bytes, void* stream) {
+    EMCID_CHECK_DUAL_STAGE1_ARGS();
+    DualWorkspace ws(N, d, h);
+    EMCID_CHECK_WORKSPACE(workspace_bytes, ws.total * (int64_t)sizeof(double), "");
+    double* base = (double*)workspace;
+    launch_prep_kr(K, Zc, zs_t, N, d, h, edit_weight, layers_left, 1.0 / sqrt(lam_ratio), base + ws.off_K, ws.Np, ws.dp,
+                   base + ws.off_R, ws.hp, (hipStream_t)stream);
+    return apply_stage1_rows(ws, N, d, cov_factor_ws, n_layers, layer_index, n_lo, n_hi, use_inverse, base, (hipStream_t)stream);
+}
+
+int emcid_edit_dual_apply_stage1_prepared_f64(int64_t N, int64_t d, int64_t h, const void* cov_factor_ws, int64_t n_layers,
+                                              int64_t layer_index, int64_t n_lo, int64_t n_hi, int use_inverse, void* workspace,
+                                              int64_t workspace_bytes, void* stream) {
+    EMCID_CHECK_ARG(N > 0 && d > 0 && h > 0 && cov_factor_ws && workspace);
+    EMCID_CHECK_ARG(0 <= layer_index && layer_index < n_layers && 0 <= n_lo && n_lo < n_hi && n_hi <= N);
+    DualWorkspace ws(N, d, h);
+    EMCID_CHECK_WORKSPACE(workspace_bytes, ws.total * (int64_t)sizeof(double), "");
+    return apply_stage1_rows(ws, N, d, cov_factor_ws, n_layers, layer_index, n_lo, n_hi, use_inverse, (double*)workspace,
+                             (hipStream_t)stream);
 }
 
 double* emcid_edit_dual_yt(void* workspace, int64_t N, int64_t d, int64_t h) { return dual_block(workspace, N, d, h, &DualWorkspace::off_Y); }
@@ -493,14 +633,15 @@
     return EMCID_OK;
 }
 
-int emcid_edit_dual_apply_stage2_f64(int64_t N, int64_t d, int64_t h, const void* cov_factor_ws, int64_t n_layers,
-                                     int64_t layer_index, int use_inverse, int assembled, const float* W0, float* W,
-                                     float* dW_out, void* workspace, int64_t workspace_bytes, int* info_dev, void* stream) {
-    EMCID_CHECK_ARG(N > 0 && d > 0 && h > 0 && workspace && info_dev && cov_factor_ws && ((W == nullptr) || (W0 != nullptr)));
-    EMCID_CHECK_ARG(0 <= layer_index && layer_index < n_layers && (W || dW_out));
-    DualWorkspace ws(N, d, h);
-    EMCID_CHECK_WORKSPACE(workspace_bytes, ws.total * (int64_t)sizeof(double), "");
-    hipStream_t st = (hipStream_t)stream;
+#define EMCID_CHECK_APPLY_STAGE2_ARGS()                                                                                            \
+    EMCID_CHECK_ARG(N > 0 && d > 0 && h > 0 && workspace && info_dev && cov_factor_ws && ((W == nullptr) || (W0 != nullptr)));     \
+    EMCID_CHECK_ARG(0 <= layer_index && layer_index < n_layers && (W || dW_out));                                                  \
+    EMCID_CHECK_WORKSPACE(workspace_bytes, DualWorkspace(N, d, h).total * (int64_t)sizeof(double), "")
+
+static int apply_stage2(int64_t N, int64_t d, int64_t h, const void* cov_factor_ws, int64_t n_layers, int64_t layer_index,
+                        int use_inverse, int assembled, bool rt_ready, const float* W0, float* W, float* dW_out, void* workspace,
+                        int* info_dev, hipStream_t st) {
+    DualWorkspace ws(N, d, h);
     double* base = (double*)workspace;
     double *Yt = base + ws.off_Y, *R = base + ws.off_R, *S = base + ws.off_S, *LS = base + ws.off_LS, *invS = base + ws.off_invS;
     double *RT = base + ws.off_PT, *Y2 = base + ws.off_Y2, *V = base + ws.off_V, *U = base + ws.off_U;
@@ -522,7 +663,8 @@
     double *XT = base + ws.off_XT, *TT = base + ws.off_TT;
     EMCID_TRY(with_graph(make_key(GRAPH_APPLY_STAGE2, {Yt, R, S, LS, RT, V, U, info_dev},
                                   {dp, Np, N, hp, (int64_t)(uintptr_t)Lb,
-                                   use_inverse + 2 * (assembled != 0) + 4 * (int)shadow + 8 * h + ((int64_t)p_first << 31) + ((int64_t)xrow << 30) + (d << 32)}),
+                                   use_inverse + 2 * (assembled != 0) + 4 * (int)shadow + 8 * h + ((int64_t)p_first << 31) + ((int64_t)xrow << 30) +
+                                       ((int64_t)rt_ready << 29) + (d << 32)}),
                          st,
                          [&](hipStream_t q) {
         if (!assembled) {
@@ -533,7 +675,7 @@
         job.wgs = (int)((Np + SH_BM - 1) / SH_BM) * (int)(((dp + SH_BN - 1) / SH_BN + 1) / 2);
         const XrowJob xj{XT, Np, TT};
         EMCID_TRY(cholesky_impl(S, LS, Np, Np, invS, info_dev, q, shadow ? &job : nullptr, xrow ? &xj : nullptr));
-        EMCID_TRY(solve_schur_rhs(R, hp, h, Np, LS, invS, xrow ? XT : nullptr, S, RT, Y2, ws.y2_doubles(), q));
+        EMCID_TRY(solve_schur_rhs(R, hp, h, Np, LS, invS, xrow ? XT : nullptr, S, RT, Y2, ws.y2_doubles(), q, rt_ready));
         if (!shadow && !p_first) {
             ScopedProf sp(KC_DELTA_W, q);
             GemmShape g{RT, Np, Yt, dp, (int)h, (int)dp, (int)Np, 0};
@@ -552,6 +694,54 @@
     if (use_inverse)
         apply_inverse_backward(X, dp, V, (int)h, (int)dp, U, dp, st, base + ws.off_SK);
     hipLaunchKernelGGL(apply_u2d_kernel, dim3((unsigned)h), dim3(256), 0, st, U, dp, W0, W, dW_out, (int)d);
+    return check_launch("emcid_edit_dual_apply_stage2_f64");
+}
+
+int emcid_edit_dual_apply_stage2_f64(int64_t N, int64_t d, int64_t h, const void* cov_factor_ws, int64_t n_layers,
+                                     int64_t layer_index, int use_inverse, int assembled, const float* W0, float* W,
+                                     float* dW_out, void* workspace, int64_t workspace_bytes, int* info_dev, void* stream) {
+    EMCID_CHECK_APPLY_STAGE2_ARGS();
+    return apply_stage2(N, d, h, cov_factor_ws, n_layers, layer_index, use_inverse, assembled, false, W0, W, dW_out, workspace,
+                        info_dev, (hipStream_t)stream);
+}
+
+int emcid_edit_dual_apply_stage2_rt_f64(int64_t N, int64_t d, int64_t h, const void* cov_factor_ws, int64_t n_layers,
+                                        int64_t layer_index, int use_inverse, int assembled, int rt_ready, const float* W0, float* W,
+                                        float* dW_out, void* workspace, int64_t workspace_bytes, int* info_dev, void* stream) {
+    EMCID_CHECK_APPLY_STAGE2_ARGS();
+    return apply_stage2(N, d, h, cov_factor_ws, n_layers, layer_index, use_inverse, assembled, rt_ready != 0, W0, W, dW_out,
+                        workspace, info_dev, (hipStream_t)stream);
+}
+
+int emcid_edit_key_prep_f64(const float* f_f32, int64_t n_rows, const int64_t* lookup, const int64_t* seg, int64_t B, int64_t N,
+                            int64_t d, int64_t h, double edit_weight, double lam_ratio, float* K_out, void* k_planes,
+                            float* k_inv_scale, void* workspace, int64_t workspace_bytes, void* stream) {
+    EMCID_CHECK_ARG(f_f32 && lookup && seg && K_out && k_planes && k_inv_scale && workspace && n_rows > 0 && B > 0 && N > 0);
+    EMCID_CHECK_ARG(d > 0 && h > 0 && d % 8 == 0 && d <= 32768 && N < (1 << 24) && lam_ratio > 0.0 && lam_ratio < 1e300);
+    EMCID_CHECK_ARG(aligned16(f_f32) && aligned16(K_out) && aligned16(k_planes) && aligned16(workspace));
+    DualWorkspace ws(N, d, h);
+    EMCID_CHECK_WORKSPACE(workspace_bytes, ws.total * (int64_t)sizeof(double), "");
+    hipStream_t st = (hipStream_t)stream;
+    ScopedProf sp(KC_PREP, st);
+    hipLaunchKernelGGL(key_prep_kernel, dim3((unsigned)ws.Np), dim3(256), 0, st, f_f32, d, n_rows, lookup, seg, (int)N, (int)d,
+                       (int)ws.dp, sqrt(edit_weight / 0.5), 1.0 / sqrt(lam_ratio), K_out, (uint32_t*)k_planes, k_inv_scale,
+                       (double*)workspace + ws.off_K);
+    EMCID_CHECK_LAUNCH();
+    return EMCID_OK;
+}
+
+int emcid_edit_residual_t_f64(const float* Zc, const float* zs_t, int64_t N, int64_t d, int64_t h, double edit_weight,
+                              int layers_left, double lam_ratio, void* workspace, int64_t workspace_bytes, void* stream) {
+    EMCID_CHECK_ARG(Zc && zs_t && workspace && N > 0 && d > 0 && h > 0 && layers_left > 0 && N < (1 << 24) && h <= 32768);
+    EMCID_CHECK_ARG(lam_ratio > 0.0 && lam_ratio < 1e300 && aligned16(workspace));
+    DualWorkspace ws(N, d, h);
+    EMCID_CHECK_WORKSPACE(workspace_bytes, ws.total * (int64_t)sizeof(double), "");
+    if (ws.y2_doubles() < ws.hp * ws.Np) return fail(EMCID_ERR_WORKSPACE, __func__, "RT holds fewer than h rows of Np (h > d rounded up to 128)");
+    hipStream_t st = (hipStream_t)stream;
+    ScopedProf sp(KC_PREP, st);
+    hipLaunchKernelGGL(residual_t_kernel, dim3((unsigned)((ws.hp + 31) / 32), (unsigned)(ws.Np / 32)), dim3(256), 0, st, Zc, zs_t,
+                       (int)N, (int)h, sqrt(edit_weight / 0.5), (double)layers_left, 1.0 / sqrt(lam_ratio),
+                       (double*)workspace + ws.off_PT, (int)ws.Np, (int)ws.hp);
     EMCID_CHECK_LAUNCH();
     return EMCID_OK;
 }
diff --git a/emcid_amd/csrc/spd_solve.h b/emcid_amd/csrc/spd_solve.h
--- a/emcid_amd/csrc/spd_solve.h
+++ b/emcid_amd/csrc/spd_solve.h
@@ -117,7 +117,7 @@
 }
 
 int solve_schur_rhs(const double* R, int64_t hp, int64_t h, int64_t Np, const double* LS, const double* invS, const double* XT,
-                    double* full_inv, double* RT, double* Y2, int64_t y2_doubles, hipStream_t st);
+                    double* full_inv, double* RT, double* Y2, int64_t y2_doubles, hipStream_t st, bool rt_ready = false);
 
 
 static __global__ __launch_bounds__(256) void copy2d_f64_kernel(const double* __restrict__ src, int64_t lds_, double* __restrict__ dst,
diff --git a/emcid_amd/hip.py b/emcid_amd/hip.py
--- a/emcid_amd/hip.py
+++ b/emcid_amd/hip.py
@@ -37,6 +37,8 @@
     "emcid_tree_attention_sp16", "emcid_tree_attention_sp16_supported", "emcid_clip_workspace_bytes",
     "emcid_clip_layer_head_sp16", "emcid_clip_layer_tail_sp16", "emcid_clip_layers_sp16", "emcid_clip_edit_layer_tail_sp16",
     "emcid_edit_dual_block", "emcid_edit_dual_schur_form", "emcid_full_inverse_scratch_doubles", "emcid_full_inverse_f64",
+    "emcid_edit_key_prep_f64", "emcid_edit_dual_apply_stage1_prepared_f64", "emcid_edit_residual_t_f64",
+    "emcid_edit_dual_apply_stage2_rt_f64", "emcid_gather_query_rows",
 ]
 DUAL_BLOCKS = ["K", "P", "Y", "R", "S", "LS", "INVS", "PT", "Y2", "V", "U", "SK", "XT", "TT", "SK_COUNTERS"]
 SCHUR_FORMS = ["xrow", "full_inverse", "substitution"]
@@ -96,6 +98,11 @@
         "emcid_edit_dual_yt": (p, [p, i64, i64, i64]),
         "emcid_edit_dual_apply_stage2_f64": (i32, [i64, i64, i64, p, i64, i64, i32, i32, p, p, p, p, i64, p, p]),
         "emcid_edit_dual_apply_assemble_f64": (i32, [i64, i64, i64, p, i64, p]),
+        "emcid_edit_key_prep_f64": (i32, [p, i64, p, p, i64, i64, i64, i64, f64, f64, p, p, p, p, i64, p]),
+        "emcid_edit_dual_apply_stage1_prepared_f64": (i32, [i64, i64, i64, p, i64, i64, i64, i64, i32, p, i64, p]),
+        "emcid_edit_residual_t_f64": (i32, [p, p, i64, i64, i64, f64, i32, f64, p, i64, p]),
+        "emcid_edit_dual_apply_stage2_rt_f64": (i32, [i64, i64, i64, p, i64, i64, i32, i32, i32, p, p, p, p, i64, p, p]),
+        "emcid_gather_query_rows": (i32, [p, p, p, p, i64, i64, p, p, p, p]),
         "emcid_edit_dual_preserve_workspace_bytes": (i64, [i64, i64, i64, i64]),
         "emcid_edit_layer_dual_preserve_f64": (i32, [p, p, p, i64, i64, i64, f64, i32, f64, p, i64, i64, p, i64, p, i64, p, i64, i64,
                                                      p, p, p, p, p, i64, p, p]),
@@ -948,6 +955,18 @@
     return {"K": K, "Zc": Zc, "dW": dW, "hs": hs, "x": x}
 
 
+def gather_query_rows(x: "SplitRows", hs: torch.Tensor, rows_sel: torch.Tensor):
+    n, h = rows_sel.numel(), hs.shape[1]
+    assert x.planes.shape == hs.shape and x.planes.is_contiguous() and hs.is_contiguous() and x.inv_scale.is_contiguous()
+    dev = hs.device
+    out = SplitRows(torch.empty(n, h, dtype=torch.int32, device=dev), torch.empty(n, dtype=torch.float32, device=dev))
+    hs_q = torch.empty(n, h, dtype=torch.float32, device=dev)
+    _check(load().emcid_gather_query_rows(_ptr(x.planes), _ptr(x.inv_scale, torch.float32, "scale"), _ptr(hs, torch.float32, "hs"),
+                                          _ptr(rows_sel, torch.int32, "rows"), n, h, _ptr(out.planes), _ptr(out.inv_scale),
+                                          _ptr(hs_q), _stream(hs)), "emcid_gather_query_rows")
+    return out, hs_q
+
+
 
 class CovFactors:
 
@@ -1192,6 +1211,52 @@
                                                 _ptr(ws.buf), ws.nbytes, _ptr(ws.info, torch.int32), _stream(K)),
            "emcid_edit_dual_apply_stage2_f64")
     return {"dW": dW, "ws": ws}
+
+
+def edit_key_prep(f_f32: torch.Tensor, lookup: torch.Tensor, seg: torch.Tensor, h: int, edit_weight: float, lam_ratio: float,
+                  ws: DualWorkspace):
+    n_rows, d = f_f32.shape
+    N = seg.numel() - 1
+    assert f_f32.is_contiguous() and ws.key == (N, d, h)
+    K = torch.empty(N, d, dtype=torch.float32, device=f_f32.device)
+    kp = SplitRows(torch.empty(N, d, dtype=torch.int32, device=f_f32.device), torch.empty(N, dtype=torch.float32, device=f_f32.device))
+    _check(load().emcid_edit_key_prep_f64(_ptr(f_f32, torch.float32, "f_f32"), n_rows, _ptr(lookup, torch.int64, "lookup"),
+                                          _ptr(seg, torch.int64, "seg"), lookup.numel(), N, d, h, float(edit_weight), float(lam_ratio),
+                                          _ptr(K), _ptr(kp.planes), _ptr(kp.inv_scale), _ptr(ws.buf), ws.nbytes, _stream(f_f32)),
+           "emcid_edit_key_prep_f64")
+    return K, kp
+
+
+def edit_residual_t(Zc: torch.Tensor, zs_t: torch.Tensor, d: int, edit_weight: float, layers_left: int, lam_ratio: float,
+                    ws: DualWorkspace):
+    N, h = Zc.shape
+    assert Zc.is_contiguous() and zs_t.is_contiguous() and zs_t.shape == (N, h) and ws.key == (N, d, h)
+    _check(load().emcid_edit_residual_t_f64(_ptr(Zc, torch.float32, "Zc"), _ptr(zs_t, torch.float32, "zs_t"), N, d, h,
+                                            float(edit_weight), int(layers_left), float(lam_ratio), _ptr(ws.buf), ws.nbytes,
+                                            _stream(Zc)), "emcid_edit_residual_t_f64")
+
+
+def dual_apply_stage1_prepared(factors: CovFactors, layer_index: int, ws: DualWorkspace, use_inverse: Optional[bool] = None):
+    if use_inverse is None:
+        use_inverse = layer_index in factors.have_inverse
+    N, d, h = ws.key
+    _check(load().emcid_edit_dual_apply_stage1_prepared_f64(N, d, h, _ptr(factors.buf), factors.n_layers, int(layer_index), 0, N,
+                                                            int(bool(use_inverse)), _ptr(ws.buf), ws.nbytes, _stream(ws.buf)),
+           "emcid_edit_dual_apply_stage1_prepared_f64")
+
+
+def dual_apply_stage2(factors: CovFactors, layer_index: int, W0, W, ws: DualWorkspace, rt_ready: bool, want_dw: bool = True,
+                      use_inverse: Optional[bool] = None):
+    if use_inverse is None:
+        use_inverse = layer_index in factors.have_inverse
+    N, d, h = ws.key
+    dW = torch.empty(h, d, dtype=torch.float32, device=W.device) if want_dw else None
+    _check(load().emcid_edit_dual_apply_stage2_rt_f64(N, d, h, _ptr(factors.buf), factors.n_layers, int(layer_index),
+                                                      int(bool(use_inverse)), 0, int(bool(rt_ready)),
+                                                      _ptr(W0, torch.float32, "W0"), _ptr(W, torch.float32, "W"), _ptr(dW),
+                                                      _ptr(ws.buf), ws.nbytes, _ptr(ws.info, torch.int32), _stream(W)),
+           "emcid_edit_dual_apply_stage2_rt_f64")
+    return dW
 
 
 def check_preserved_state(sd, n_layers: int, d: int, capacity: int) -> int:
diff --git a/include/emcid_hip.h b/include/emcid_hip.h
--- a/include/emcid_hip.h
+++ b/include/emcid_hip.h
@@ -97,6 +97,9 @@
                                const int* anc, int64_t anc_ld, const int* depth, const int* rows_sel, int64_t n_sel,
                                const float* hs, const void* x_planes, const float* x_inv_scale, float* mid, void* f_planes,
                                float* f_scale, float* f_f32, void* workspace, int64_t workspace_bytes, void* stream);
+
+int emcid_gather_query_rows(const void* x_planes, const float* x_inv_scale, const float* hs, const int* rows_sel, int64_t n_sel,
+                            int64_t h, void* planes_out, float* scale_out, float* hs_out, void* stream);
 
 int emcid_clip_layer_tail_sp16(const emcid_clip_layer_sp16* L, int64_t n, int64_t h, int64_t d, const void* f_planes,
                                const float* f_inv_scale, const float* mid, float* hs_out, const float* next_ln_gamma,
@@ -170,6 +173,17 @@
 int emcid_edit_dual_apply_stage2_f64(int64_t N, int64_t d, int64_t h, const void* cov_factor_ws, int64_t n_layers,
                                      int64_t layer_index, int use_inverse, int assembled, const float* W0, float* W,
                                      float* dW_out, void* workspace, int64_t workspace_bytes, int* info_dev, void* stream);
+int emcid_edit_key_prep_f64(const float* f_f32, int64_t n_rows, const int64_t* lookup, const int64_t* seg, int64_t B, int64_t N,
+                            int64_t d, int64_t h, double edit_weight, double lam_ratio, float* K_out, void* k_planes,
+                            float* k_inv_scale, void* workspace, int64_t workspace_bytes, void* stream);
+int emcid_edit_dual_apply_stage1_prepared_f64(int64_t N, int64_t d, int64_t h, const void* cov_factor_ws, int64_t n_layers,
+                                              int64_t layer_index, int64_t n_lo, int64_t n_hi, int use_inverse, void* workspace,
+                                              int64_t workspace_bytes, void* stream);
+int emcid_edit_residual_t_f64(const float* Zc, const float* zs_t, int64_t N, int64_t d, int64_t h, double edit_weight,
+                              int layers_left, double lam_ratio, void* workspace, int64_t workspace_bytes, void* stream);
+int emcid_edit_dual_apply_stage2_rt_f64(int64_t N, int64_t d, int64_t h, const void* cov_factor_ws, int64_t n_layers,
+                                        int64_t layer_index, int use_inverse, int assembled, int rt_ready, const float* W0, float* W,
+                                        float* dW_out, void* workspace, int64_t workspace_bytes, int* info_dev, void* stream);
 int emcid_edit_dual_apply_assemble_f64(int64_t N, int64_t d, int64_t h, void* workspace, int64_t workspace_bytes, void* stream);
 
 int64_t emcid_edit_dual_preserve_workspace_bytes(int64_t N, int64_t d, int64_t h, int64_t capacity);
```

Result: slower. 108,000 (-2.6%).
